# BIH-CEI/napkon-string-matching

Measured on AMD Instinct MI355X. Metric: pair-comparisons/sec (whole node), N x M all-pairs, higher is better.
Workload: dtype u64; 1 GPU; C3: 200000x200000 strings/GPU (len U[16,64], 37 symbols), fuzzy_match RAW, threshold 0.8; score_func=fuzzy_match, mode=RAW, hits_per_rank=2000, hits_all_ranks=2000, exact_prune=True, hit_ordering=second stream, overlapped with the next step's grid kernel (two hit buffers)

## Files before the change

### include/nsm_hip.h

```cpp
#ifndef NSM_HIP_H
#define NSM_HIP_H

#include <stdint.h>

#ifdef __cplusplus
extern "C" {
#endif

#define NSM_ABI_VERSION 5

#define NSM_E_BADARG 10001
#define NSM_E_UNSUPPORTED 10002

#define NSM_LEVELS_ID_LIMIT (1 << 26)

typedef struct nsm_hit {
  double score;
  int32_t i;
  int32_t j;
} nsm_hit;

typedef struct nsm_set_table {
  const int32_t* ids;
  const int32_t* cnt;
  const uint64_t* sig;
  const uint64_t* sig2;
  const int32_t* orig;
  const int32_t* size_start;
  const int32_t* nlev;
  const uint8_t* plen;
  const uint64_t* cat;
  const uint32_t* filt;
  const int32_t* seg;
  const int32_t* seg_start;
  int32_t n;
  int32_t width;
  int32_t max_levels;
  int32_t vocab;
  const uint64_t* post;
  const int32_t* post_start;
  uint64_t post_sq[5];
  int32_t post_row_bits;
  int32_t post_format;
} nsm_set_table;

typedef struct nsm_str_table {
  const uint8_t* codes;
  const int32_t* len;
  const int32_t* orig;
  const int32_t* len_start;
  const uint8_t* hist;
  int32_t n;
  int32_t stride;
  int32_t alphabet;
  const uint8_t* hist16;
} nsm_str_table;

typedef struct nsm_level_items {
  const int32_t* first;
  const int32_t* nlev;
  const int32_t* orig;
  const uint64_t* cat;
  const int32_t* seg;
  const int32_t* seg_start;
  int32_t n;
} nsm_level_items;

#define NSM_CAT_NONE 0
#define NSM_CAT_INTERSECT 1
#define NSM_CAT_INTERSECT_OR_BOTH_EMPTY 2

#define NSM_FLAG_PRUNE 1u
#define NSM_FLAG_INDEX 4u
#define NSM_FLAG_NO_INDEX 8u
#define NSM_FLAG_TILE_INDEX 64u
#define NSM_FLAG_PARK 16u
#define NSM_FLAG_SPLIT 128u
#define NSM_FLAG_TILE 256u
#define NSM_FLAG_PROBE 512u
#define NSM_FLAG_ONE_STAGE 1024u
#define NSM_FLAG_PACK 2048u
#define NSM_FLAG_NO_PACK 4096u
#define NSM_FLAG_WAVE_WIDE 2u

int nsm_abi_version(void);
const char* nsm_last_error(void);

int nsm_jaccard_raw_grid(const nsm_set_table* left, const nsm_set_table* right, double threshold,
                         uint32_t flags, nsm_hit* hits , uint64_t capacity,
                         unsigned long long* hit_count , void* stream);

int nsm_indel_raw_top_k(const nsm_str_table* left, const nsm_str_table* right, double threshold, int32_t k,
                        uint32_t flags, nsm_hit* out ,
                        unsigned long long* out_count , uint64_t* stats ,
                        void* stream);
int nsm_jaccard_raw_top_k(const nsm_set_table* left, const nsm_set_table* right, double threshold, int32_t k,
                          uint32_t flags, nsm_hit* out, unsigned long long* out_count, uint64_t* stats, void* stream);

int nsm_indel_raw_top_k_grouped(const nsm_str_table* left, const nsm_str_table* right,
                                const int32_t* right_group ,
                                double threshold, int32_t k, uint32_t flags,
                                nsm_hit* out , unsigned long long* out_count ,
                                uint64_t* stats , void* stream);
int nsm_jaccard_raw_top_k_grouped(const nsm_set_table* left, const nsm_set_table* right, const int32_t* right_group,
                                  double threshold, int32_t k, uint32_t flags,
                                  nsm_hit* out, unsigned long long* out_count, uint64_t* stats, void* stream);

int nsm_jaccard_levels_grid(const nsm_set_table* left, const nsm_set_table* right, double threshold,
                            int32_t category_mode, uint32_t flags, nsm_hit* hits, uint64_t capacity,
                            unsigned long long* hit_count, void* stream);

int nsm_indel_raw_grid(const nsm_str_table* left, const nsm_str_table* right, double threshold,
                       uint32_t flags, nsm_hit* hits, uint64_t capacity,
                       unsigned long long* hit_count, void* stream);

uint64_t nsm_indel_levels_workspace_bytes(const nsm_level_items* left, const nsm_str_table* left_strings,
                                          const nsm_level_items* right, const nsm_str_table* right_strings,
                                          double threshold, uint32_t flags, double expected_survivors);
int nsm_indel_levels_grid(const nsm_level_items* left, const nsm_str_table* left_strings,
                          const nsm_level_items* right, const nsm_str_table* right_strings,
                          double threshold, int32_t category_mode, uint32_t flags, nsm_hit* hits,
                          uint64_t capacity, unsigned long long* hit_count, void* workspace,
                          uint64_t workspace_bytes, double expected_survivors, void* stream);

int nsm_indel_levels_top_k(const nsm_level_items* left, const nsm_str_table* left_strings,
                           const nsm_level_items* right, const nsm_str_table* right_strings,
                           double threshold, int32_t k, int32_t category_mode, uint32_t flags,
                           const int32_t* banned_start , const int32_t* banned_j ,
                           nsm_hit* out , unsigned long long* out_count ,
                           uint64_t* stats , void* stream);
int nsm_jaccard_levels_top_k(const nsm_set_table* left, const nsm_set_table* right,
                             double threshold, int32_t k, int32_t category_mode, uint32_t flags,
                             const int32_t* banned_start, const int32_t* banned_j,
                             nsm_hit* out, unsigned long long* out_count, uint64_t* stats, void* stream);

int nsm_indel_raw_profile(const nsm_str_table* left, const nsm_str_table* right, const double* thresholds ,
                          int32_t n_thresholds, uint32_t flags, uint64_t* pairs ,
                          double* left_best ,
                          double* right_best , uint64_t* stats ,
                          void* stream);
int nsm_jaccard_raw_profile(const nsm_set_table* left, const nsm_set_table* right, const double* thresholds,
                            int32_t n_thresholds, uint32_t flags, uint64_t* pairs, double* left_best, double* right_best,
                            uint64_t* stats, void* stream);
int nsm_indel_levels_profile(const nsm_level_items* left, const nsm_str_table* left_strings,
                             const nsm_level_items* right, const nsm_str_table* right_strings,
                             const double* thresholds, int32_t n_thresholds, int32_t category_mode, uint32_t flags,
                             const int32_t* banned_start, const int32_t* banned_j, uint64_t* pairs, double* left_best,
                             double* right_best, uint64_t* stats, void* stream);
int nsm_jaccard_levels_profile(const nsm_set_table* left, const nsm_set_table* right, const double* thresholds,
                               int32_t n_thresholds, int32_t category_mode, uint32_t flags, const int32_t* banned_start,
                               const int32_t* banned_j, uint64_t* pairs, double* left_best, double* right_best,
                               uint64_t* stats, void* stream);

int nsm_indel_raw_floor_grid(const nsm_str_table* left, const nsm_str_table* right, double threshold,
                             const double* left_floor , const double* right_floor ,
                             uint32_t flags, nsm_hit* hits, uint64_t capacity,
                             unsigned long long* hit_count , uint64_t* stats ,
                             void* stream);
int nsm_jaccard_raw_floor_grid(const nsm_set_table* left, const nsm_set_table* right, double threshold,
                               const double* left_floor, const double* right_floor, uint32_t flags, nsm_hit* hits,
                               uint64_t capacity, unsigned long long* hit_count, uint64_t* stats, void* stream);
int nsm_indel_levels_floor_grid(const nsm_level_items* left, const nsm_str_table* left_strings,
                                const nsm_level_items* right, const nsm_str_table* right_strings, double threshold,
                                const double* left_floor, const double* right_floor, int32_t category_mode, uint32_t flags,
                                const int32_t* banned_start, const int32_t* banned_j, nsm_hit* hits, uint64_t capacity,
                                unsigned long long* hit_count, uint64_t* stats, void* stream);
int nsm_jaccard_levels_floor_grid(const nsm_set_table* left, const nsm_set_table* right, double threshold,
                                  const double* left_floor, const double* right_floor, int32_t category_mode, uint32_t flags,
                                  const int32_t* banned_start, const int32_t* banned_j, nsm_hit* hits, uint64_t capacity,
                                  unsigned long long* hit_count, uint64_t* stats, void* stream);

int nsm_indel_raw_pairs(const nsm_str_table* left, const nsm_str_table* right,
                        const int32_t* left_row , int32_t left_ids, const int32_t* right_row ,
                        int32_t right_ids, nsm_hit* pairs , uint64_t n_pairs, void* stream);
int nsm_jaccard_raw_pairs(const nsm_set_table* left, const nsm_set_table* right, const int32_t* left_row, int32_t left_ids,
                          const int32_t* right_row, int32_t right_ids, nsm_hit* pairs, uint64_t n_pairs, void* stream);
int nsm_indel_levels_pairs(const nsm_level_items* left, const nsm_str_table* left_strings,
                           const nsm_level_items* right, const nsm_str_table* right_strings,
                           const int32_t* left_row, int32_t left_ids, const int32_t* right_row, int32_t right_ids,
                           nsm_hit* pairs, uint64_t n_pairs, void* stream);
int nsm_jaccard_levels_pairs(const nsm_set_table* left, const nsm_set_table* right, const int32_t* left_row,
                             int32_t left_ids, const int32_t* right_row, int32_t right_ids, nsm_hit* pairs, uint64_t n_pairs,
                             void* stream);

int nsm_release(void* stream);
int nsm_release_all(void);

#define NSM_BUILD_PARTITION 1u
#define NSM_BUILD_VALIDATE 2u
#define NSM_BUILD_SORT 4u

int nsm_build_set_table(const int32_t* ids_in, int32_t n, int32_t width_in, int32_t side, const int32_t* nlev_in,
                        const uint8_t* plen_in, const uint64_t* cat_in, const int32_t* orig_in, int32_t category_mode,
                        uint32_t flags, nsm_set_table* out, void* stream);

int nsm_build_str_table(const uint8_t* codes_in, const int32_t* len_in, const int32_t* orig_in, int32_t n, uint32_t flags,
                        nsm_str_table* out, void* stream);

int nsm_build_level_items(const int32_t* first_in, const int32_t* nlev_in, const uint64_t* cat_in, const int32_t* orig_in,
                          int32_t n, int32_t category_mode, uint32_t flags, nsm_level_items* out, void* stream);

typedef struct nsm_any_strings {
  const uint16_t* codes;
  const int64_t* offset;
  int32_t n_rows;
  int32_t alphabet;
  int32_t max_len;
} nsm_any_strings;

typedef struct nsm_any_items {
  const int32_t* first;
  const int32_t* nlev;
  const int32_t* orig;
  const uint64_t* cat;
  int32_t n;
} nsm_any_items;

typedef struct nsm_any_sets {
  const int32_t* ids;
  const uint8_t* lv;
  const int64_t* offset;
  const int32_t* nlev;
  const int32_t* plen;
  const int32_t* orig;
  const uint64_t* cat;
  int32_t n;
  int32_t max_levels;
  int32_t max_ids;
  const int32_t* first;
} nsm_any_sets;

#define NSM_FLAG_RAW_SCORE 32u

int nsm_indel_any_grid(const nsm_any_items* left, const nsm_any_strings* left_strings, const nsm_any_items* right,
                       const nsm_any_strings* right_strings, double threshold, int32_t category_mode, uint32_t flags,
                       nsm_hit* hits, uint64_t capacity, unsigned long long* hit_count, void* stream);
int nsm_jaccard_any_grid(const nsm_any_sets* left, const nsm_any_sets* right, double threshold, int32_t category_mode,
                         uint32_t flags, nsm_hit* hits, uint64_t capacity, unsigned long long* hit_count, void* stream);

int nsm_sort_hits(nsm_hit* hits, nsm_hit* scratch, uint64_t capacity, const unsigned long long* hit_count,
                  uint64_t n_hint, uint32_t id_limit, void* stream);

#ifdef __cplusplus
}
#endif
#endif
```

### napkon-string-matching_amd/csrc/indel_raw.hip

```cpp
#include "nsm_common.hpp"
#include "indel_score.hpp"

#include <map>
#include <mutex>
#include <utility>

namespace nsm {

struct IndelRawParams {
  int32_t n_left;
  int32_t n_right;
  int32_t rows_per_chunk;
  int32_t pm_stride;
  int32_t zero_need;
  unsigned long long cap;
  uint8_t lcsmin[132];
};

static double indel_score_host(int la, int lb, int lcs) {
  if (la == 0 || lb == 0) return 0.0;
  const volatile double maximum = static_cast<double>(la + lb);
  const volatile double dist = static_cast<double>(la + lb - 2 * lcs);
  const volatile double q = dist / maximum;
  const volatile double norm_sim = 1.0 - q;
  const volatile double pct = norm_sim * 100.0;
  return pct / 100.0;
}

template <typename T>
__device__ __forceinline__ T lds_load(uint32_t addr) {
  return *reinterpret_cast<const __attribute__((address_space(3))) T*>(addr);
}

__device__ __forceinline__ unsigned long long add64(unsigned long long a, unsigned long long b) {
  unsigned long long d;
  asm("v_lshl_add_u64 %0, %1, 0, %2" : "=v"(d) : "v"(a), "v"(b));
  return d;
}

__device__ __forceinline__ void raw_build_masks(unsigned long long* pm, int pm_stride, const uint8_t* __restrict__ lcodes, int i,
                                                int la, bool wide, int lane) {
  for (int c = lane; c < pm_stride; c += kWave) pm[c] = 0ull;
  __builtin_amdgcn_fence(__ATOMIC_RELEASE, "wavefront");
  __builtin_amdgcn_wave_barrier();
  if (lane < la) {
    const unsigned c = lcodes[static_cast<size_t>(i) * 64 + lane];
    atomicOr(&pm[c], wide ? (1ull << lane) : ((1ull << lane) | (1ull << (32 + lane))));
  }
  __builtin_amdgcn_fence(__ATOMIC_ACQ_REL, "wavefront");
  __builtin_amdgcn_wave_barrier();
}

#ifndef NSM_LCS_STOP_EVERY
#define NSM_LCS_STOP_EVERY 1
#endif
__device__ __forceinline__ int raw_lcs_units(uint32_t lcode, int la, uint32_t rcode, int lb, int need, int lane) {
  const bool swap = la < lb;
  const int lp = swap ? lb : la, lt = swap ? la : lb;
  const uint32_t pat = lane < lp ? (swap ? rcode : lcode) : 0x100u;
  const uint32_t text = lane < lt ? (swap ? lcode : rcode) : 0x200u;
  const int lim = lt - need + 64;
  unsigned long long v = ~0ull;
  if (lt > 0) {
#pragma unroll
    for (int w = 0; w < 16; ++w) {
#pragma unroll
      for (int b = 0; b < 4; ++b) {
        const uint32_t c = static_cast<uint32_t>(__builtin_amdgcn_readlane(static_cast<int>(text), 4 * w + b));
        const unsigned long long m = __ballot(pat == c);
        const unsigned long long u = v & m;
        v = (v + u) | (v & ~m);
      }
      if (4 * (w + 1) >= lt) break;
      if (NSM_LCS_STOP_EVERY > 0 && (w + 1) % (NSM_LCS_STOP_EVERY > 0 ? NSM_LCS_STOP_EVERY : 1) == 0 && __popcll(v) + 4 * (w + 1) > lim)
        break;
    }
  }
  return __popcll(~v);
}

__device__ __forceinline__ int raw_lcs_pair(const uint8_t* __restrict__ lcodes, int row, int la, const uint8_t* __restrict__ rcodes,
                                            int j, int lb, int need, int lane) {
  return raw_lcs_units(lcodes[static_cast<size_t>(row) * 64 + lane], la, rcodes[static_cast<size_t>(j) * 64 + lane], lb, need, lane);
}

#ifndef NSM_C3_OCC
#define NSM_C3_OCC
#endif
#ifndef NSM_C3_TILES
#define NSM_C3_TILES 2
#endif
template <bool PRUNE>
constexpr int c3_tiles() { return PRUNE ? NSM_C3_TILES : 1; }

template <bool PRUNE>
__global__ __launch_bounds__(kBlock) NSM_C3_OCC void indel_raw_kernel(
    const uint8_t* __restrict__ lcodes, const int32_t* __restrict__ llen, const int32_t* __restrict__ lstart,
    const int32_t* __restrict__ lorig, const uint32_t* __restrict__ lhist, const uint8_t* __restrict__ rcodes,
    const int32_t* __restrict__ rlen, const int32_t* __restrict__ rorig, const uint32_t* __restrict__ rhist,
    nsm_hit* __restrict__ hits, unsigned long long* __restrict__ count, const IndelRawParams p) {
  constexpr int T = c3_tiles<PRUNE>();
  extern __shared__ __attribute__((aligned(16))) unsigned long long s_mem[];
  uint8_t* s_lcsmin = reinterpret_cast<uint8_t*>(s_mem + kWavesPerBlock * p.pm_stride);
  for (int t = threadIdx.x; t < 132; t += kBlock) s_lcsmin[t] = p.lcsmin[t];
  __syncthreads();

  const int lane = threadIdx.x & (kWave - 1);
  const int wave = threadIdx.x >> 6;
  const int tile0 = (blockIdx.x * kWavesPerBlock + wave) * T;
  if (tile0 * kWave >= p.n_right) return;
  bool valid[T];
  int jc[T], lbj[T];
#pragma unroll
  for (int t = 0; t < T; ++t) {
    const int j = (tile0 + t) * kWave + lane;
    valid[t] = j < p.n_right;
    jc[t] = valid[t] ? j : p.n_right - 1;
    lbj[t] = valid[t] ? rlen[jc[t]] : 0;
  }

  unsigned long long* pm = s_mem + wave * p.pm_stride;
  const uint32_t pm_base = static_cast<uint32_t>(wave * p.pm_stride * 8);

  uint32_t taddr[PRUNE ? 1 : 32];
  auto build_taddr = [&](bool narrow) {
    if constexpr (!PRUNE) {
      const uint4* tp = reinterpret_cast<const uint4*>(rcodes + static_cast<size_t>(jc[0]) * 64);
      const uint32_t hsel = narrow ? 4u : 0u;
#pragma unroll
      for (int q = 0; q < 4; ++q) {
        const uint4 v = tp[q];
        const uint32_t w[4] = {v.x, v.y, v.z, v.w};
#pragma unroll
        for (int e = 0; e < 4; ++e) {
          const uint32_t c0 = w[e] & 0xffu, c1 = (w[e] >> 8) & 0xffu, c2 = (w[e] >> 16) & 0xffu, c3 = w[e] >> 24;
          const uint32_t a0 = pm_base + 8 * c0 + (((c0 >> 4) & 1u) ? hsel : 0u), a1 = pm_base + 8 * c1 + (((c1 >> 4) & 1u) ? hsel : 0u);
          const uint32_t a2 = pm_base + 8 * c2 + (((c2 >> 4) & 1u) ? hsel : 0u), a3 = pm_base + 8 * c3 + (((c3 >> 4) & 1u) ? hsel : 0u);
          taddr[8 * q + 2 * e + 0] = a0 | (a1 << 16);
          taddr[8 * q + 2 * e + 1] = a2 | (a3 << 16);
        }
      }
    }
  };
  int taddr_narrow = -1;
  const int npairs = (wave_first(lbj[0]) + 1) >> 1;
  uint32_t hr[T][8];
  if (PRUNE) {
#pragma unroll
    for (int t = 0; t < T; ++t) {
      const uint4* hp = reinterpret_cast<const uint4*>(rhist + static_cast<size_t>(jc[t]) * 8);
      const uint4 h0 = hp[0], h1 = hp[1];
      hr[t][0] = h0.x; hr[t][1] = h0.y; hr[t][2] = h0.z; hr[t][3] = h0.w;
      hr[t][4] = h1.x; hr[t][5] = h1.y; hr[t][6] = h1.z; hr[t][7] = h1.w;
    }
  }
  uint32_t lowmask = 0xffffu;
  asm volatile("" : "+v"(lowmask));

  const int i0 = blockIdx.y * p.rows_per_chunk;
  const int i1 = min(p.n_left, i0 + p.rows_per_chunk);

  auto build_masks = [&](int i, int la, bool wide) { raw_build_masks(pm, p.pm_stride, lcodes, i, la, wide, lane); };

  auto lcs_row = [&](int i, int la, bool wide) -> int {
    if (taddr_narrow != static_cast<int>(!wide)) {
      build_taddr(!wide);
      taddr_narrow = static_cast<int>(!wide);
    }
    build_masks(i, la, wide);
    const int nchars = 2 * npairs;
    if (!wide) {
      uint32_t v = ~0u;
#pragma unroll
      for (int g = 0; g < 8; ++g) {
        if (g * 8 < nchars) {
          uint32_t m[8];
#pragma unroll
          for (int q = 0; q < 4; ++q) {
            m[2 * q] = lds_load<uint32_t>(taddr[(4 * g + q) % (PRUNE ? 1 : 32)] & lowmask);
            m[2 * q + 1] = lds_load<uint32_t>(taddr[(4 * g + q) % (PRUNE ? 1 : 32)] >> 16);
          }
#pragma unroll
          for (int q = 0; q < 8; ++q) v = lcs_step32(v, m[q]);
        }
      }
      return 32 - __popc(v);
    }
    unsigned long long v = ~0ull;
#pragma unroll
    for (int g = 0; g < 8; ++g) {
      if (g * 8 < nchars) {
        unsigned long long m[8];
#pragma unroll
        for (int q = 0; q < 4; ++q) {
          m[2 * q] = lds_load<unsigned long long>(taddr[(4 * g + q) % (PRUNE ? 1 : 32)] & lowmask);
          m[2 * q + 1] = lds_load<unsigned long long>(taddr[(4 * g + q) % (PRUNE ? 1 : 32)] >> 16);
        }
#pragma unroll
        for (int q = 0; q < 8; ++q) v = lcs_step64(v, m[q]);
      }
    }
    return 64 - __popcll(v);
  };

  const int c_first = 64 - llen[i0];
  const int c_last = 64 - llen[i1 - 1];
  for (int c = c_first; c <= c_last; ++c) {
    const int a = max(i0, lstart[c]);
    const int b = min(i1, lstart[c + 1]);
    if (a >= b) continue;
    const int la = 64 - c;
    int need[T];
#pragma unroll
    for (int t = 0; t < T; ++t) {
      if (la == 0 || lbj[t] == 0) need[t] = p.zero_need;
      else need[t] = s_lcsmin[la + lbj[t]];
      if (!valid[t]) need[t] = kNever;
    }
    const bool wide = la > 32;
    if constexpr (PRUNE) {
      bool fits[T], some = false;
#pragma unroll
      for (int t = 0; t < T; ++t) {
        fits[t] = min(la, lbj[t]) >= need[t];
        some = some || fits[t];
      }
      if (!__any(some)) continue;
      auto score_row = [&](int i, uint32_t who) {
#pragma unroll
        for (int t = 0; t < T; ++t) {
          for (unsigned long long todo = __ballot((who >> t) & 1u); todo; todo &= todo - 1ull) {
            const int leader = __builtin_ctzll(todo);
            const int j_s = __builtin_amdgcn_readlane(jc[t], leader);
            const int lb_s = __builtin_amdgcn_readlane(lbj[t], leader);
            const int need_s = __builtin_amdgcn_readlane(need[t], leader);
            const int lcs = raw_lcs_pair(lcodes, i, la, rcodes, j_s, lb_s, need_s, lane);
            if (lcs >= need_s && lane == 0) emit_hit(hits, p.cap, count, indel_score(la, lb_s, lcs), lorig[i], rorig[j_s]);
          }
        }
      };
      int limit[T];
      uint32_t seed[T];
#pragma unroll
      for (int t = 0; t < T; ++t) {
        limit[t] = fits[t] ? la + lbj[t] - 2 * need[t] : -1;
        seed[t] = static_cast<uint32_t>(-(limit[t] + 1));
      }
      const uint32_t* __restrict__ hp = lhist + static_cast<size_t>(a) * 8;
      int i = a;
#ifndef NSM_C3_BATCH
#define NSM_C3_BATCH 4
#endif
      constexpr int BATCH = NSM_C3_BATCH;
      for (; i + BATCH <= b; i += BATCH, hp += 8 * BATCH) {
        uint32_t h[8 * BATCH];
#pragma unroll
        for (int q = 0; q < 8 * BATCH; ++q) h[q] = hp[q];
        int margin[T][BATCH];
        int any_pass = 0;
#pragma unroll
        for (int r = 0; r < BATCH; ++r) {
#pragma unroll
          for (int t = 0; t < T; ++t) {
            uint32_t l1 = seed[t];
#pragma unroll
            for (int q = 0; q < 8; ++q) l1 = __builtin_amdgcn_sad_u8(h[8 * r + q], hr[t][q], l1);
            margin[t][r] = static_cast<int>(l1);
            any_pass |= margin[t][r];
          }
        }
        if (__any(any_pass < 0)) {
          uint32_t cand[T];
#pragma unroll
          for (int t = 0; t < T; ++t) {
            cand[t] = 0;
#pragma unroll
            for (int r = 0; r < BATCH; ++r) cand[t] |= margin[t][r] < 0 ? (1u << r) : 0u;
          }
          for (int r = 0; r < BATCH; ++r) {
            uint32_t who = 0;
#pragma unroll
            for (int t = 0; t < T; ++t) who |= ((cand[t] >> r) & 1u) << t;
            if (__any(who != 0u)) score_row(i + r, who);
          }
        }
      }
      for (; i < b; ++i, hp += 8) {
        uint32_t who = 0;
#pragma unroll
        for (int t = 0; t < T; ++t) {
          uint32_t l1 = 0;
#pragma unroll
          for (int q = 0; q < 8; ++q) l1 = __builtin_amdgcn_sad_u8(hp[q], hr[t][q], l1);
          who |= (static_cast<int>(l1) <= limit[t] ? 1u : 0u) << t;
        }
        if (__any(who != 0u)) score_row(i, who);
      }
    } else {
      for (int i = a; i < b; ++i) {
        const int lcs = lcs_row(i, la, wide);
        const bool hit = lcs >= need[0];
        if (__any(hit)) {
          if (hit) emit_hit(hits, p.cap, count, indel_score(la, lbj[0], lcs), lorig[i], rorig[jc[0]]);
        }
      }
    }
  }
}

}
#include "indel_raw_coarse.hpp"
namespace nsm {

static int pick_rows_per_chunk(int n_left, int n_tiles) {
#ifndef NSM_C3_WANT_WAVES
#define NSM_C3_WANT_WAVES (16ll * 256 * 32)
#endif
  const long long want_waves = NSM_C3_WANT_WAVES;
  long long chunks = (want_waves + n_tiles - 1) / (n_tiles > 0 ? n_tiles : 1);
  if (chunks < 1) chunks = 1;
  long long rows = (n_left + chunks - 1) / chunks;
  if (rows < 64) rows = 64;
#ifndef NSM_C3_CHUNK_MAX
#define NSM_C3_CHUNK_MAX 4096
#endif
  if (rows > NSM_C3_CHUNK_MAX) rows = NSM_C3_CHUNK_MAX;
  return static_cast<int>(rows);
}

struct PackScratch {
  void* rows = nullptr;
  size_t bytes = 0;
};
static std::mutex g_pack_mu;
static std::map<std::pair<int, void*>, PackScratch> g_pack;

static void* pack_scratch(hipStream_t stream, size_t bytes) {
  int dev = 0;
  if (hipGetDevice(&dev) != hipSuccess) return nullptr;
  std::lock_guard<std::mutex> lock(g_pack_mu);
  PackScratch& w = g_pack[std::make_pair(dev, static_cast<void*>(stream))];
  if (w.bytes >= bytes && w.rows) return w.rows;
  if (w.rows) (void)hipFree(w.rows);
  w.rows = nullptr;
  w.bytes = 0;
  if (hipMalloc(&w.rows, bytes) != hipSuccess) {
    (void)hipGetLastError();
    w.rows = nullptr;
    return nullptr;
  }
  w.bytes = bytes;
  return w.rows;
}

void release_pack_scratch(int dev, void* stream, bool all) {
  std::lock_guard<std::mutex> lock(g_pack_mu);
  for (auto it = g_pack.begin(); it != g_pack.end();) {
    if (all || it->first == std::make_pair(dev, stream)) {
      if (it->second.rows) (void)hipFree(it->second.rows);
      it = g_pack.erase(it);
    } else {
      ++it;
    }
  }
}

int indel_raw_wide(const nsm_str_table* left, const nsm_str_table* right, double threshold, uint32_t flags,
                   nsm_hit* hits, uint64_t capacity, unsigned long long* hit_count, hipStream_t stream);

}

extern "C" int nsm_indel_raw_grid(const nsm_str_table* left, const nsm_str_table* right,
                                  double threshold, uint32_t flags, nsm_hit* hits, uint64_t capacity,
                                  unsigned long long* hit_count, void* stream) {
  using namespace nsm;
  if (!left || !right || !hit_count || (!hits && capacity)) {
    set_error("nsm_indel_raw_grid: null argument");
    return NSM_E_BADARG;
  }
  if (left->stride != right->stride || (left->stride != 64 && left->stride != 128 && left->stride != 256 && left->stride != 512)) {
    set_error("nsm_indel_raw_grid: stride %d/%d unsupported (both sides 64, 128, 256 or 512 code units)",
              left->stride, right->stride);
    return NSM_E_UNSUPPORTED;
  }
  if (left->alphabet != right->alphabet || left->alphabet < 1 || left->alphabet > 255) {
    set_error("nsm_indel_raw_grid: alphabets differ or exceed 255 (%d, %d)", left->alphabet,
              right->alphabet);
    return NSM_E_BADARG;
  }
  if (left->n < 0 || right->n < 0) {
    set_error("nsm_indel_raw_grid: negative row count");
    return NSM_E_BADARG;
  }
  if (left->n == 0 || right->n == 0) return 0;
  if (!left->codes || !left->len || !left->orig || !left->len_start || !right->codes || !right->len ||
      !right->orig) {
    set_error("nsm_indel_raw_grid: table has a null column");
    return NSM_E_BADARG;
  }

  if (left->stride != 64)
    return indel_raw_wide(left, right, threshold, flags, hits, capacity, hit_count, static_cast<hipStream_t>(stream));

  IndelRawParams p;
  p.n_left = left->n; p.n_right = right->n;
  p.cap = capacity;
  p.pm_stride = ((left->alphabet + 1) + 63) / 64 * 64;
  p.zero_need = (0.0 >= threshold) ? 0 : kNever;
  for (int s = 0; s < 132; ++s) {
    p.lcsmin[s] = kNever;
    if (s < 2 || s > 128) continue;
    for (int lcs = 0; 2 * lcs <= s; ++lcs) {
      if (indel_score_host(1, s - 1, lcs) >= threshold) {
        p.lcsmin[s] = static_cast<uint8_t>(lcs);
        break;
      }
    }
  }
  const bool prune = (flags & NSM_FLAG_PRUNE) && left->hist && right->hist;
  if (prune && left->hist16 && right->hist16 && !(flags & NSM_FLAG_ONE_STAGE)) {
    if ((reinterpret_cast<uintptr_t>(left->hist16) | reinterpret_cast<uintptr_t>(right->hist16)) & 15u) {
      set_error("nsm_indel_raw_grid: hist16 must be 16-byte aligned (rows are read as one 128-bit word)");
      return NSM_E_BADARG;
    }
    if ((reinterpret_cast<uintptr_t>(left->hist) | reinterpret_cast<uintptr_t>(right->hist)) & 15u) {
      set_error("nsm_indel_raw_grid: hist must be 16-byte aligned (rows are read as 128-bit words)");
      return NSM_E_BADARG;
    }
    const int n_tiles = (right->n + kC3cRights - 1) / kC3cRights;
    p.rows_per_chunk = (pick_rows_per_chunk(left->n, n_tiles) + kC3cBlock - 1) / kC3cBlock * kC3cBlock;
    dim3 grid((n_tiles + kWavesPerBlock - 1) / kWavesPerBlock, (left->n + p.rows_per_chunk - 1) / p.rows_per_chunk);
    if (grid.y > 65535) {
      p.rows_per_chunk = ((left->n + 65534) / 65535 + kC3cBlock - 1) / kC3cBlock * kC3cBlock;
      grid.y = (left->n + p.rows_per_chunk - 1) / p.rows_per_chunk;
    }
    if (p.rows_per_chunk > (1 << 15)) {
      set_error("nsm_indel_raw_grid: %d left rows per chunk", p.rows_per_chunk);
      return NSM_E_UNSUPPORTED;
    }
    hipStream_t hs = static_cast<hipStream_t>(stream);
    const uint32_t* lh32 = reinterpret_cast<const uint32_t*>(left->hist);
    const uint32_t* rh32 = reinterpret_cast<const uint32_t*>(right->hist);
#if NSM_C3C_FP4
    bool pack = !(flags & NSM_FLAG_NO_PACK) &&
                ((flags & NSM_FLAG_PACK) || c3c_pack_pays(static_cast<long long>(left->n) * static_cast<long long>(right->n)));
    if (pack) {
      hipStreamCaptureStatus capture = hipStreamCaptureStatusNone;
      if (hipStreamIsCapturing(hs, &capture) != hipSuccess) capture = hipStreamCaptureStatusNone;
      pack = capture == hipStreamCaptureStatusNone;
    }
    void* packed = pack ? pack_scratch(hs, static_cast<size_t>(left->n) * kC3cPackedRow) : nullptr;
    if (packed) {
      const long long units = 2ll * left->n;
      hipLaunchKernelGGL(c3c_pack_left_kernel, dim3(static_cast<unsigned>((units + kBlock - 1) / kBlock)), dim3(kBlock), 0, hs,
                         lh32, static_cast<c3c_v4i*>(packed), left->n);
      hipLaunchKernelGGL((indel_raw_coarse_kernel<NSM_C3C_NT, NSM_C3C_CAP, true>), grid, dim3(kBlock), c3c_lds_bytes(), hs,
                         left->codes, left->len, left->len_start, left->orig, lh32, right->codes, right->len, right->orig,
                         rh32, hits, hit_count, p, static_cast<const char*>(packed));
      return hip_status(hipGetLastError(), "indel_raw_coarse_kernel launch (packed)");
    }
#endif
    hipLaunchKernelGGL((indel_raw_coarse_kernel<NSM_C3C_NT, NSM_C3C_CAP, false>), grid, dim3(kBlock), c3c_lds_bytes(), hs,
                       left->codes, left->len, left->len_start, left->orig, lh32, right->codes, right->len, right->orig,
                       rh32, hits, hit_count, p, static_cast<const char*>(nullptr));
    return hip_status(hipGetLastError(), "indel_raw_coarse_kernel launch");
  }
  const int tiles_per_wave = prune ? c3_tiles<true>() : 1;
  const int n_tiles = ((right->n + kWave - 1) / kWave + tiles_per_wave - 1) / tiles_per_wave;
  p.rows_per_chunk = pick_rows_per_chunk(left->n, n_tiles);
  dim3 grid((n_tiles + kWavesPerBlock - 1) / kWavesPerBlock,
            (left->n + p.rows_per_chunk - 1) / p.rows_per_chunk);
  if (grid.y > 65535) {
    p.rows_per_chunk = (left->n + 65534) / 65535;
    grid.y = (left->n + p.rows_per_chunk - 1) / p.rows_per_chunk;
  }
  const size_t lds = static_cast<size_t>(kWavesPerBlock) * p.pm_stride * 8 + 136;
  hipStream_t s = static_cast<hipStream_t>(stream);
  const uint32_t* lh = reinterpret_cast<const uint32_t*>(left->hist);
  const uint32_t* rh = reinterpret_cast<const uint32_t*>(right->hist);
  if (prune)
    hipLaunchKernelGGL((indel_raw_kernel<true>), grid, dim3(kBlock), lds, s, left->codes, left->len,
                       left->len_start, left->orig, lh, right->codes, right->len, right->orig, rh, hits, hit_count, p);
  else
    hipLaunchKernelGGL((indel_raw_kernel<false>), grid, dim3(kBlock), lds, s, left->codes, left->len,
                       left->len_start, left->orig, lh, right->codes, right->len, right->orig, rh, hits, hit_count, p);
  return hip_status(hipGetLastError(), "indel_raw_kernel launch");
}
```

### napkon-string-matching_amd/csrc/indel_raw_coarse.hpp

```cpp
#pragma once

namespace nsm {

#ifndef NSM_C3C_CAP
#define NSM_C3C_CAP 3
#endif
#ifndef NSM_C3C_FP4
#define NSM_C3C_FP4 1
#endif
#ifndef NSM_C3C_FP4_PERM
#define NSM_C3C_FP4_PERM 1
#endif
#ifndef NSM_C3C_FP4_SPLIT
#define NSM_C3C_FP4_SPLIT 4
#endif
#ifndef NSM_C3C_NT
#define NSM_C3C_NT 4
#endif
#ifndef NSM_C3C_ORFOLD
#define NSM_C3C_ORFOLD (NSM_C3C_FP4 && NSM_C3C_NT % 2 == 0)
#endif
#ifndef NSM_C3C_PIPE
#define NSM_C3C_PIPE (NSM_C3C_NT % (NSM_C3C_ORFOLD ? 4 : 2) == 0)
#endif
#ifndef NSM_C3C_OR_SPLIT
#define NSM_C3C_OR_SPLIT 2
#endif
#ifndef NSM_C3C_LCS_PREFETCH
#define NSM_C3C_LCS_PREFETCH 1
#endif
#ifndef NSM_C3C_EARLY_OUT
#define NSM_C3C_EARLY_OUT 1
#endif
constexpr int kC3cBlock = 32;
constexpr int kC3cRights = NSM_C3C_NT * kC3cBlock;
constexpr int kC3cPipeExtra = NSM_C3C_PIPE ? (NSM_C3C_ORFOLD ? 2 : 1) : 0;
constexpr int kC3cStack = (NSM_C3C_NT + 2 + kC3cPipeExtra) * kWave;
constexpr int kC3cDrainAt = 2 * kWave;
static_assert(NSM_C3C_NT >= 1 && NSM_C3C_NT <= 4, "an entry keeps its tile in 2 bits");
static_assert(NSM_C3C_CAP >= 2 && NSM_C3C_CAP <= 8, "code slots per bucket");

static inline size_t c3c_lds_bytes() {
  return static_cast<size_t>(kWavesPerBlock) * (kC3cStack * 8 + static_cast<size_t>(kC3cRights) * (8 * 4 + 1)) + 136;
}

typedef int c3c_v4i __attribute__((ext_vector_type(4)));
typedef int c3c_v16i __attribute__((ext_vector_type(16)));
typedef int c3c_v8i __attribute__((ext_vector_type(8)));
typedef float c3c_v16f __attribute__((ext_vector_type(16)));

__device__ __forceinline__ uint32_t c3c_ge64(uint32_t w, int k) {
  return (w + static_cast<uint32_t>(0x40 - k) * 0x01010101u) & 0x40404040u;
}


__device__ __forceinline__ int c3c_fp4_scale(const uint4& f0, const uint4& f1) {
  const uint32_t ws[8] = {f0.x, f0.y, f0.z, f0.w, f1.x, f1.y, f1.z, f1.w};
  uint32_t any = 0u;
#pragma unroll
  for (int q = 0; q < 8; ++q) any |= ws[q];
  if ((any & 0xf0f0f0f0u) == 0u) return 0;
  uint32_t top = 0u;
#pragma unroll
  for (int q = 0; q < 8; ++q)
#pragma unroll
    for (int b = 0; b < 4; ++b) top = max(top, (ws[q] >> (8 * b)) & 0xffu);
  return top <= 27u ? 1 : top <= 51u ? 2 : 3;
}
__device__ __forceinline__ void c3c_fp4_right_k0(uint32_t fw, int& m1, int& m2) {
  const uint32_t sel = fw & 0x07070707u;
  const uint32_t big = ((fw >> 3) & 0x01010101u) * 0xffu;
  const uint32_t lo1 = __builtin_amdgcn_perm(0x11111111u, 0x11110100u, sel);
  const uint32_t lo2 = __builtin_amdgcn_perm(0x41312111u, 0x01000000u, sel), hi2 = __builtin_amdgcn_perm(0x71717171u, 0x61615151u, sel);
  m1 = static_cast<int>((big & 0x11111111u) | (~big & lo1));
  m2 = static_cast<int>((big & hi2) | (~big & lo2));
}
__device__ __forceinline__ void c3c_fp4_right_scaled(uint32_t fw, int k, int& m1, int& m2) {
  m1 = static_cast<int>((c3c_ge64(fw, 1) >> 6) | (c3c_ge64(fw, 2) >> 2));
  uint32_t w2 = c3c_ge64(fw, 3) >> 6;
  const uint32_t round_up = (1u << k) - 1u;
#pragma unroll
  for (int b = 0; b < 4; ++b) {
    const uint32_t r = (fw >> (8 * b)) & 0xffu;
    const uint32_t q = (max(r, 3u) - 3u + round_up) >> k;
    w2 |= (static_cast<uint32_t>(0x7777665543210ull >> (4u * q)) & 0xfu) << (8 * b + 4);
  }
  m2 = static_cast<int>(w2);
}
__device__ __forceinline__ void c3c_fp4_left(uint32_t w, int& m1, int& m2) {
#if NSM_C3C_FP4_PERM
  const uint32_t sel = (w + 0x3c3c3c3cu) & 0x43434343u;
  m1 = static_cast<int>(__builtin_amdgcn_perm(0u, 0x44440400u, sel) & 0x44444444u);
  m2 = static_cast<int>(__builtin_amdgcn_perm(0u, 0x04000000u, sel) & 0x44444444u);
#else
  m1 = static_cast<int>(((c3c_ge64(w, 1) >> 4)) | c3c_ge64(w, 2));
  m2 = static_cast<int>(((c3c_ge64(w, 3) >> 4)) | c3c_ge64(w, 4));
#endif
}
__device__ __forceinline__ c3c_v16f c3c_fp4_mfma1(const c3c_v4i& a, const c3c_v4i& b) {
  const c3c_v8i a8 = {a.x, a.y, a.z, a.w, 0, 0, 0, 0}, b8 = {b.x, b.y, b.z, b.w, 0, 0, 0, 0};
  const c3c_v16f zero = {0, 0, 0, 0, 0, 0, 0, 0, 0, 0, 0, 0, 0, 0, 0, 0};
  return __builtin_amdgcn_mfma_scale_f32_32x32x64_f8f6f4(a8, b8, zero, 4, 4, 0, 0, 0, 0);
}
__device__ __forceinline__ c3c_v16f c3c_fp4_mfma2(const c3c_v4i& a, const c3c_v4i& b, const c3c_v16f& acc, int scales, int t) {
  const c3c_v8i a8 = {a.x, a.y, a.z, a.w, 0, 0, 0, 0}, b8 = {b.x, b.y, b.z, b.w, 0, 0, 0, 0};
  switch (t) {
    case 0: return __builtin_amdgcn_mfma_scale_f32_32x32x64_f8f6f4(a8, b8, acc, 4, 4, 0, 0x7f7f7f7f, 0, scales);
    case 1: return __builtin_amdgcn_mfma_scale_f32_32x32x64_f8f6f4(a8, b8, acc, 4, 4, 0, 0x7f7f7f7f, 1, scales);
    case 2: return __builtin_amdgcn_mfma_scale_f32_32x32x64_f8f6f4(a8, b8, acc, 4, 4, 0, 0x7f7f7f7f, 2, scales);
    default: return __builtin_amdgcn_mfma_scale_f32_32x32x64_f8f6f4(a8, b8, acc, 4, 4, 0, 0x7f7f7f7f, 3, scales);
  }
}

constexpr int kC3cPackedRow = 64;
#ifndef NSM_C3C_PACK_MIN_PAIRS
#define NSM_C3C_PACK_MIN_PAIRS 10000000000ll
#endif
static inline bool c3c_pack_pays(long long pairs) { return pairs >= static_cast<long long>(NSM_C3C_PACK_MIN_PAIRS); }
struct c3c_packed_rows {
  c3c_v4i m1, m2;
};
template <bool PACKED>
struct c3c_rows {
  typedef uint4 type;
};
template <>
struct c3c_rows<true> {
  typedef c3c_packed_rows type;
};

__global__ __launch_bounds__(kBlock) void c3c_pack_left_kernel(const uint32_t* __restrict__ lhist, c3c_v4i* __restrict__ packed,
                                                               int n_left) {
  const int u = blockIdx.x * kBlock + threadIdx.x;
  if (u >= 2 * n_left) return;
  const uint4 w = reinterpret_cast<const uint4*>(lhist)[u];
  const uint32_t ws[4] = {w.x, w.y, w.z, w.w};
  c3c_v4i m1, m2;
#pragma unroll
  for (int q = 0; q < 4; ++q) {
    int a1, a2;
    c3c_fp4_left(ws[q], a1, a2);
    m1[q] = a1;
    m2[q] = a2;
  }
  packed[2 * static_cast<size_t>(u)] = m1;
  packed[2 * static_cast<size_t>(u) + 1] = m2;
}

#ifndef NSM_C3C_OCC
#define NSM_C3C_OCC __attribute__((amdgpu_waves_per_eu((NSM_C3C_ORFOLD && PACKED) ? 4 : 2)))
#endif
template <int NT, int CAP, bool PACKED>
__global__ __launch_bounds__(kBlock) NSM_C3C_OCC void indel_raw_coarse_kernel(
    const uint8_t* __restrict__ lcodes, const int32_t* __restrict__ llen, const int32_t* __restrict__ lstart,
    const int32_t* __restrict__ lorig, const uint32_t* __restrict__ lhist, const uint8_t* __restrict__ rcodes,
    const int32_t* __restrict__ rlen, const int32_t* __restrict__ rorig, const uint32_t* __restrict__ rhist,
    nsm_hit* __restrict__ hits, unsigned long long* __restrict__ count, const IndelRawParams p,
    const char* __restrict__ lpacked) {
  static_assert(!PACKED || NSM_C3C_FP4, "only the FP4 scan has packed left rows");
  constexpr int kRights = NT * kC3cBlock;
  static_assert(kC3cDrainAt >= kWave && kC3cDrainAt + (NT + kC3cPipeExtra) * kWave <= kC3cStack,
                "the drain is triggered above kC3cDrainAt entries and runs full passes");
  constexpr bool kOrFold = NSM_C3C_ORFOLD && PACKED;
  constexpr int kFlagHi = 1 << 17, kFlagLo = 1 << 8;
  static_assert(!kOrFold || (NSM_C3C_FP4 && NT % 2 == 0), "the OR fold puts tiles 2 p and 2 p + 1 of the FP4 scan on one accumulator");
  extern __shared__ __attribute__((aligned(16))) unsigned long long s_mem[];
  unsigned long long* s_stack = s_mem;
  uint32_t* s_rh = reinterpret_cast<uint32_t*>(s_stack + kWavesPerBlock * kC3cStack);
  uint8_t* s_rl = reinterpret_cast<uint8_t*>(s_rh + kWavesPerBlock * 8 * kRights);
  uint8_t* s_lcsmin = s_rl + kWavesPerBlock * kRights;
  for (int t = threadIdx.x; t < 132; t += kBlock) s_lcsmin[t] = p.lcsmin[t];
  __syncthreads();

  const int lane = threadIdx.x & (kWave - 1);
  const int wave = threadIdx.x >> 6;
  const int col = lane & (kC3cBlock - 1);
  const int half = lane >> 5;
  const int j0 = (blockIdx.x * kWavesPerBlock + wave) * kRights;
  if (j0 >= p.n_right) return;
  auto lane_again = [&]() -> int {
    int l = lane;
    asm volatile("" : "+v"(l));
    return l;
  };
#if NSM_C3C_EARLY_OUT
  if (p.zero_need != 0) {
    const int ie = blockIdx.y * p.rows_per_chunk;
    const int la_hi = llen[ie], la_lo = llen[min(p.n_left, ie + p.rows_per_chunk) - 1];
    bool fits = false;
#pragma unroll
    for (int k = 0; k < (kRights + kWave - 1) / kWave; ++k) {
      const int j = j0 + k * kWave + lane;
      if (k * kWave + lane < kRights && j < p.n_right) {
        const int lb = rlen[j];
        const int la = min(max(lb, la_lo), la_hi);
        const int nd = (la == 0 || lb == 0) ? p.zero_need : static_cast<int>(s_lcsmin[la + lb]);
        fits = fits || min(la, lb) >= nd;
      }
    }
    if (!__any(fits)) return;
  }
#endif
  unsigned long long* stack = s_stack + wave * kC3cStack;
  uint32_t* rh_lds = s_rh + wave * 8 * kRights;
  uint8_t* rl_lds = s_rl + wave * kRights;

#pragma unroll
  for (int k = 0; k < (kRights + kWave - 1) / kWave; ++k) {
    const int rl = k * kWave + lane;
    if (rl < kRights) {
      const int j = j0 + rl;
      const int jcl = j < p.n_right ? j : p.n_right - 1;
      const uint4* fp = reinterpret_cast<const uint4*>(rhist + static_cast<size_t>(jcl) * 8);
      const uint4 f0 = fp[0], f1 = fp[1];
      uint32_t* dst = rh_lds + rl;
      dst[0 * kRights] = f0.x; dst[1 * kRights] = f0.y; dst[2 * kRights] = f0.z; dst[3 * kRights] = f0.w;
      dst[4 * kRights] = f1.x; dst[5 * kRights] = f1.y; dst[6 * kRights] = f1.z; dst[7 * kRights] = f1.w;
      rl_lds[rl] = static_cast<uint8_t>(j < p.n_right ? rlen[jcl] : 0);
    }
  }
  bool valid[NT];
#if NSM_C3C_FP4
  c3c_v4i bfrag[NT][2];
  uint32_t bscales = 0u;
  auto scale_base = [](int t) -> uint32_t { return (kOrFold && t % 2 == 0) ? 0x7fu + 9u : 0x7fu; };
  uint32_t bscales1 = 0u;
  if constexpr (kOrFold) {
#pragma unroll
    for (int t = 0; t < NT; ++t) bscales1 |= scale_base(t) << (8 * t);
    asm volatile("" : "+v"(bscales1));
  }
  auto code_tile = [&](int t, const uint4& f, int k) __attribute__((always_inline)) {
    const uint32_t ws[4] = {f.x, f.y, f.z, f.w};
    if (k == 0) {
#pragma unroll
      for (int q = 0; q < 4; ++q) {
        int m1, m2;
        c3c_fp4_right_k0(ws[q], m1, m2);
        bfrag[t][0][q] = m1;
        bfrag[t][1][q] = m2;
      }
    } else {
#pragma unroll
      for (int q = 0; q < 4; ++q) {
        int m1, m2;
        c3c_fp4_right_scaled(ws[q], k, m1, m2);
        bfrag[t][0][q] = m1;
        bfrag[t][1][q] = m2;
      }
    }
  };
#pragma unroll
  for (int t = 0; t < NT; ++t) {
    const int j = j0 + t * kC3cBlock + col;
    valid[t] = j < p.n_right;
    const int jcl = valid[t] ? j : p.n_right - 1;
    const uint4* fp = reinterpret_cast<const uint4*>(rhist + static_cast<size_t>(jcl) * 8);
    const uint4 f0 = fp[0], f1 = fp[1];
    const int k = c3c_fp4_scale(f0, f1);
    bscales |= (scale_base(t) + static_cast<uint32_t>(k)) << (8 * t);
    uint4 f = half ? f1 : f0;
    if (!valid[t]) f = make_uint4(0u, 0u, 0u, 0u);
    code_tile(t, f, k);
  }
  auto make_bfrag = [&]() __attribute__((always_inline)) {
    const int l = lane_again();
    const uint32_t* rp0 = rh_lds + (4 * (l >> 5)) * kRights + (l & (kC3cBlock - 1));
#pragma unroll
    for (int t = 0; t < NT; ++t) {
      const uint32_t* rp = rp0 + t * kC3cBlock;
      const int k = static_cast<int>(((bscales >> (8 * t)) & 0xffu) - scale_base(t));
      uint4 f = make_uint4(rp[0], rp[kRights], rp[2 * kRights], rp[3 * kRights]);
      if (!valid[t]) f = make_uint4(0u, 0u, 0u, 0u);
      code_tile(t, f, k);
    }
  };
  __builtin_amdgcn_fence(__ATOMIC_ACQ_REL, "wavefront");
  __builtin_amdgcn_wave_barrier();
#else
  c3c_v4i bfrag[NT][CAP];
  auto code_b = [&](int t, int q, uint32_t fw) {
    const uint32_t full = c3c_ge64(fw, CAP);
#pragma unroll
    for (int s = 0; s < CAP - 1; ++s)
      bfrag[t][s][q] = static_cast<int>((c3c_ge64(fw, s + 1) ^ full) >> 6);
    bfrag[t][CAP - 1][q] = static_cast<int>(full);
  };
#pragma unroll
  for (int t = 0; t < NT; ++t) {
    const int j = j0 + t * kC3cBlock + col;
    valid[t] = j < p.n_right;
    const int jcl = valid[t] ? j : p.n_right - 1;
    uint4 f = reinterpret_cast<const uint4*>(rhist + static_cast<size_t>(jcl) * 8)[half];
    if (!valid[t]) f = make_uint4(0u, 0u, 0u, 0u);
    code_b(t, 0, f.x); code_b(t, 1, f.y); code_b(t, 2, f.z); code_b(t, 3, f.w);
  }
  auto make_bfrag = [&]() {
#pragma unroll
    for (int t = 0; t < NT; ++t) {
      const uint32_t* rp = rh_lds + (4 * half) * kRights + t * kC3cBlock + col;
#pragma unroll
      for (int q = 0; q < 4; ++q) code_b(t, q, valid[t] ? rp[q * kRights] : 0u);
    }
  };
  __builtin_amdgcn_fence(__ATOMIC_ACQ_REL, "wavefront");
  __builtin_amdgcn_wave_barrier();
#endif
  const int i0 = blockIdx.y * p.rows_per_chunk;
  const int i1 = min(p.n_left, i0 + p.rows_per_chunk);
  int q_cnt = 0;

  auto need_of = [&](int la, int lb) -> int { return (la == 0 || lb == 0) ? p.zero_need : static_cast<int>(s_lcsmin[la + lb]); };

  const char* chunk = reinterpret_cast<const char*>(lhist + static_cast<size_t>(i0) * 8);
  const char* pchunk = PACKED ? lpacked + static_cast<size_t>(i0) * kC3cPackedRow : nullptr;

  auto drain_pass = [&]() __attribute__((always_inline)) {
    __builtin_amdgcn_fence(__ATOMIC_ACQ_REL, "wavefront");
    __builtin_amdgcn_wave_barrier();
    const int n = min(q_cnt, kWave);
    const int base = q_cnt - n;
    q_cnt = base;
#ifdef NSM_C3C_X_NODRAIN
    return;
#endif
    const int m = lane & 3;
    uint32_t mask = 0;
#pragma nounroll
    for (int s = (n - 1) >> 4; s >= 0; --s) {
      const int e = 16 * s + (lane >> 2);
      const bool active = e < n;
      const unsigned long long ent = stack[base + (active ? e : 0)];
      const int n_rows = active ? static_cast<int>(static_cast<uint32_t>(ent)) : 0;
      const uint32_t ehi = static_cast<uint32_t>(ent >> 32);
      const uint32_t ib_rel = active ? ehi >> 15 : 0u;
      const int r0 = 4 * static_cast<int>((ehi >> 5) & 1u) + m;
      const uint32_t last_r = static_cast<uint32_t>(max(n_rows, 1) - 1);
      uint4 w0[4], w1[4];
#pragma unroll
      for (int g = 0; g < 4; ++g) {
        const uint4* lp = reinterpret_cast<const uint4*>(chunk + (ib_rel + min(static_cast<uint32_t>(r0 + 8 * g), last_r)) * 32u);
        w0[g] = lp[0];
        w1[g] = lp[1];
      }
      const int la = static_cast<int>((ehi >> 8) & 127u);
      const int tl = static_cast<int>((ehi >> 6) & 3u) * kC3cBlock + static_cast<int>(ehi & 31u);
      const int lb = rl_lds[tl];
      uint32_t rq[8];
      {
        const uint32_t* rp = rh_lds + tl;
#pragma unroll
        for (int q = 0; q < 8; ++q) rq[q] = rp[q * kRights];
      }
      const int nd = need_of(la, lb);
      const int budget = (active && min(la, lb) >= nd) ? la + lb - 2 * nd : -1;
      const uint32_t sad0 = ~static_cast<uint32_t>(budget);
#pragma unroll
      for (int g = 3; g >= 0; --g) {
        uint32_t l1 = sad0;
        l1 = __builtin_amdgcn_sad_u8(w0[g].x, rq[0], l1);
        l1 = __builtin_amdgcn_sad_u8(w0[g].y, rq[1], l1);
        l1 = __builtin_amdgcn_sad_u8(w0[g].z, rq[2], l1);
        l1 = __builtin_amdgcn_sad_u8(w0[g].w, rq[3], l1);
        l1 = __builtin_amdgcn_sad_u8(w1[g].x, rq[4], l1);
        l1 = __builtin_amdgcn_sad_u8(w1[g].y, rq[5], l1);
        l1 = __builtin_amdgcn_sad_u8(w1[g].z, rq[6], l1);
        l1 = __builtin_amdgcn_sad_u8(w1[g].w, rq[7], l1);
        if (r0 + 8 * g >= n_rows) l1 = 0u;
        mask = __builtin_amdgcn_alignbit(mask, l1, 31);
      }
    }
#ifdef NSM_C3C_X_NOLCS
    mask = 0u;
#endif
#ifdef NSM_C3C_X_FINEONLY
    mask = p.n_left < 0 ? mask : 0u;
#endif
    unsigned long long todo = __ballot(mask != 0u);
    uint32_t cur = 0u;
    int leader = 0, row_s = 0, j_n = 0, la_n = 0, lb_n = 0;
    auto next_pair = [&]() -> bool {
      if (cur == 0u) {
        if (todo == 0ull) return false;
        leader = __builtin_ctzll(todo);
        todo &= todo - 1ull;
        cur = static_cast<uint32_t>(__builtin_amdgcn_readlane(static_cast<int>(mask), leader));
      }
      const int pos = 31 - __builtin_clz(cur);
      cur &= ~(1u << pos);
      const uint32_t ehi = static_cast<uint32_t>(
          __builtin_amdgcn_readfirstlane(static_cast<int>(stack[base + 16 * (pos >> 2) + (leader >> 2)] >> 32)));
      const int tl = static_cast<int>((ehi >> 6) & 3u) * kC3cBlock + static_cast<int>(ehi & 31u);
      row_s = i0 + static_cast<int>(ehi >> 15) + 8 * (pos & 3) + 4 * static_cast<int>((ehi >> 5) & 1u) + (leader & 3);
      j_n = j0 + tl;
      la_n = static_cast<int>((ehi >> 8) & 127u);
      lb_n = __builtin_amdgcn_readfirstlane(static_cast<int>(rl_lds[tl]));
      return true;
    };
    auto row_units = [&](uint32_t& lc, uint32_t& rc) {
      lc = lcodes[static_cast<size_t>(row_s) * 64 + lane];
      rc = rcodes[static_cast<size_t>(j_n) * 64 + lane];
    };
    uint32_t lc_next = 0, rc_next = 0;
    bool have = next_pair();
    if (NSM_C3C_LCS_PREFETCH && have) row_units(lc_next, rc_next);
    while (have) {
      const int row_c = row_s, j_s = j_n, la_s = la_n, lb_s = lb_n;
      const int need_s = need_of(la_s, lb_s);
      uint32_t lc = lc_next, rc = rc_next;
      if (!NSM_C3C_LCS_PREFETCH) row_units(lc, rc);
      have = next_pair();
      if (NSM_C3C_LCS_PREFETCH && have) row_units(lc_next, rc_next);
      const int lcs = raw_lcs_units(lc, la_s, rc, lb_s, need_s, lane);
#ifdef NSM_C3C_X_COUNTLCS
      if (lane == 0)
#else
      if (lcs >= need_s && lane == 0)
#endif
        emit_hit(hits, p.cap, count, indel_score(la_s, lb_s, lcs), lorig[row_c], rorig[j_s]);
    }
  };
  auto drain_full = [&]() __attribute__((always_inline)) {
    while (q_cnt >= kWave) drain_pass();
    make_bfrag();
  };

  const int c_first = 64 - llen[i0];
  const int c_last = 64 - llen[i1 - 1];
  const uint32_t lane_off = static_cast<uint32_t>(col * 32 + half * 16);
  for (int c = c_first; c <= c_last; ++c) {
    const int a = max(i0, lstart[c]);
    const int b = min(i1, lstart[c + 1]);
    if (a >= b) continue;
    const int la = 64 - c;
    int need2[2] = {static_cast<int>(kNever), static_cast<int>(kNever)};
    int nm1[NT];
    bool some = false;
    const int l_c = lane_again();
#pragma unroll
    for (int t = 0; t < NT; ++t) {
      const int lb = rl_lds[t * kC3cBlock + (l_c & (kC3cBlock - 1))];
      const int nd = valid[t] ? need_of(la, lb) : static_cast<int>(kNever);
      const bool fits = min(la, lb) >= nd;
      some = some || fits;
#if NSM_C3C_FP4
      if constexpr (kOrFold)
        need2[t & 1] = min(need2[t & 1], fits ? nd : static_cast<int>(kNever));
      else
        nm1[t] = __float_as_int(static_cast<float>(fits ? nd : static_cast<int>(kNever)) - 0.5f);
#else
      nm1[t] = 64 * (fits ? nd : static_cast<int>(kNever)) - 1;
#endif
    }
    if (!__any(some)) continue;
    c3c_v16f bias;
    const float bias1 = __int_as_float(0x4b000000 | ((256 - need2[0]) << 9) | (256 - need2[1]));
    auto make_bias = [&]() {
#pragma unroll
      for (int k = 0; k < 16; ++k) {
        float x;
        asm volatile("v_mov_b32 %0, %1" : "=v"(x) : "v"(bias1));
        bias[k] = x;
      }
    };

    typedef typename c3c_rows<PACKED>::type rows_t;
    const uint32_t last_off = static_cast<uint32_t>(b - 1 - i0) * (PACKED ? 64u : 32u) + static_cast<uint32_t>((l_c >> 5) * (PACKED ? 32 : 16));
    auto load_rows = [&](int i) -> rows_t {
      if constexpr (PACKED) {
        const uint32_t off = min(static_cast<uint32_t>(i - i0) * 64u + 2u * lane_off, last_off);
        const c3c_v4i* pp = reinterpret_cast<const c3c_v4i*>(pchunk + off);
        return c3c_packed_rows{pp[0], pp[1]};
      } else {
        const uint32_t off = min(static_cast<uint32_t>(i - i0) * 32u + lane_off, last_off);
        return *reinterpret_cast<const uint4*>(chunk + off);
      }
    };
#if NSM_C3C_FP4
    typedef c3c_v16f acc_t;
    c3c_v4i afrag[2];
    auto make_afrag = [&](const rows_t& w) {
      if constexpr (!PACKED) {
        const uint32_t ws[4] = {w.x, w.y, w.z, w.w};
#pragma unroll
        for (int q = 0; q < 4; ++q) {
          int m1, m2;
          c3c_fp4_left(ws[q], m1, m2);
          afrag[0][q] = m1;
          afrag[1][q] = m2;
        }
      }
    };
    constexpr int NU = kOrFold ? NT / 2 : NT;
    auto chain = [&](int u, const rows_t& w) -> acc_t {
      if constexpr (kOrFold) {
        acc_t acc = c3c_fp4_mfma2(w.m1, bfrag[2 * u][0], bias, static_cast<int>(bscales1), 2 * u);
        acc = c3c_fp4_mfma2(w.m2, bfrag[2 * u][1], acc, static_cast<int>(bscales), 2 * u);
        acc = c3c_fp4_mfma2(w.m1, bfrag[2 * u + 1][0], acc, static_cast<int>(bscales1), 2 * u + 1);
        return c3c_fp4_mfma2(w.m2, bfrag[2 * u + 1][1], acc, static_cast<int>(bscales), 2 * u + 1);
      } else if constexpr (PACKED) {
        return c3c_fp4_mfma2(w.m2, bfrag[u][1], c3c_fp4_mfma1(w.m1, bfrag[u][0]), static_cast<int>(bscales), u);
      } else {
        return c3c_fp4_mfma2(afrag[1], bfrag[u][1], c3c_fp4_mfma1(afrag[0], bfrag[u][0]), static_cast<int>(bscales), u);
      }
    };
    auto fold = [&](const acc_t& acc) -> int {
      const c3c_v16i bits = __builtin_bit_cast(c3c_v16i, acc);
      if constexpr (kOrFold) {
        int top = bits[0] | bits[1] | bits[2];
#pragma unroll
        for (int k = 3; k < 15; k += 2) top = top | bits[k] | bits[k + 1];
        return (top | bits[15]) & (kFlagHi | kFlagLo);
      } else {
        int top = max(max(bits[0], bits[1]), bits[2]);
#pragma unroll
        for (int k = 3; k < 15; k += 2) top = max(max(top, bits[k]), bits[k + 1]);
        return max(top, bits[15]);
      }
    };
#else
    typedef c3c_v16i acc_t;
    constexpr int NU = NT;
    c3c_v4i afrag[CAP - 1];
    auto make_afrag = [&](const uint4& w) {
#pragma unroll
      for (int s = 0; s < CAP - 1; ++s) {
        afrag[s].x = static_cast<int>(c3c_ge64(w.x, s + 1)); afrag[s].y = static_cast<int>(c3c_ge64(w.y, s + 1));
        afrag[s].z = static_cast<int>(c3c_ge64(w.z, s + 1)); afrag[s].w = static_cast<int>(c3c_ge64(w.w, s + 1));
      }
    };
    auto chain = [&](int t, const uint4& w) -> c3c_v16i {
      c3c_v16i acc = {0, 0, 0, 0, 0, 0, 0, 0, 0, 0, 0, 0, 0, 0, 0, 0};
#pragma unroll
      for (int s = 0; s < CAP - 1; ++s) acc = __builtin_amdgcn_mfma_i32_32x32x32_i8(afrag[s], bfrag[t][s], acc, 0, 0, 0);
      const c3c_v4i last = {static_cast<int>(w.x), static_cast<int>(w.y), static_cast<int>(w.z), static_cast<int>(w.w)};
      return __builtin_amdgcn_mfma_i32_32x32x32_i8(last, bfrag[t][CAP - 1], acc, 0, 0, 0);
    };
    auto fold = [&](const c3c_v16i& acc) -> int {
      int top = max(max(acc[0], acc[1]), acc[2]);
#pragma unroll
      for (int k = 3; k < 15; k += 2) top = max(max(top, acc[k]), acc[k + 1]);
      return max(top, acc[15]);
    };
#endif
    auto push = [&](bool ps, unsigned long long m, int t, int i) {
      if (m == 0ull) return;
#ifdef NSM_C3C_X_COUNTPUSH
      if (lane == 0) atomicAdd(count, static_cast<unsigned long long>(__popcll(m)));
#endif
      if (ps) {
        const int slot = __builtin_amdgcn_mbcnt_hi(static_cast<uint32_t>(m >> 32), __builtin_amdgcn_mbcnt_lo(static_cast<uint32_t>(m), static_cast<uint32_t>(q_cnt)));
        const uint32_t hi = (static_cast<uint32_t>(i - i0) << 15) | (static_cast<uint32_t>(la) << 8) | (static_cast<uint32_t>(t) << 6);
        uint32_t el = static_cast<uint32_t>(lane);
        asm volatile("" : "+v"(el));
        const uint32_t n_rows = static_cast<uint32_t>(min(kC3cBlock, b - i));
        stack[slot] = (static_cast<unsigned long long>(hi | el) << 32) | n_rows;
      }
      q_cnt += __popcll(m);
    };
    auto finish = [&](int top, int u, int i) {
      if constexpr (kOrFold) {
        if (__ballot(top != 0) == 0ull) return;
        const bool hi = (top & kFlagHi) != 0 && valid[2 * u], lo = (top & kFlagLo) != 0 && valid[2 * u + 1];
        push(hi, __ballot(hi), 2 * u, i);
        push(lo, __ballot(lo), 2 * u + 1, i);
      } else {
        const bool ps = top > nm1[u];
        push(ps, __ballot(ps), u, i);
      }
    };
#if NSM_C3C_PIPE
    static_assert(NU % 2 == 0, "unit 0 of the next block takes the accumulator of unit NU: NU must be even (or NSM_C3C_PIPE=0)");
    acc_t acc[2];
    auto block = [&](int i, rows_t& wc, rows_t& wn) __attribute__((always_inline)) -> bool {
      const bool more = i + kC3cBlock < b;
      bool flush = false;
#pragma unroll
      for (int t = 0; t < NU; ++t) {
        if (t + 1 < NU) {
          acc[(t + 1) & 1] = chain(t + 1, wc);
        } else {
          flush = q_cnt > kC3cDrainAt;
          if (kOrFold || (more && !flush)) {
            make_afrag(wn);
            if constexpr (PACKED) asm volatile("" : "+v"(wn.m1), "+v"(wn.m2));
            if (i + 2 * kC3cBlock < b) wc = load_rows(i + 2 * kC3cBlock);
            acc[0] = chain(0, wn);
          }
        }
        const int top = fold(acc[t & 1]);
#if NSM_C3C_FP4
        if constexpr (kOrFold) {
          __builtin_amdgcn_sched_group_barrier(0x008, 1, 0);
          __builtin_amdgcn_sched_group_barrier(0x002, NSM_C3C_OR_SPLIT, 0);
          __builtin_amdgcn_sched_group_barrier(0x008, 1, 0);
          __builtin_amdgcn_sched_group_barrier(0x002, NSM_C3C_OR_SPLIT, 0);
          __builtin_amdgcn_sched_group_barrier(0x008, 1, 0);
          __builtin_amdgcn_sched_group_barrier(0x002, NSM_C3C_OR_SPLIT, 0);
          __builtin_amdgcn_sched_group_barrier(0x008, 1, 0);
          __builtin_amdgcn_sched_group_barrier(0x002, 8 - 3 * NSM_C3C_OR_SPLIT, 0);
        } else {
          __builtin_amdgcn_sched_group_barrier(0x008, 1, 0);
          __builtin_amdgcn_sched_group_barrier(0x002, NSM_C3C_FP4_SPLIT, 0);
          __builtin_amdgcn_sched_group_barrier(0x008, 1, 0);
          __builtin_amdgcn_sched_group_barrier(0x002, 8 - NSM_C3C_FP4_SPLIT, 0);
        }
        if (t + 1 < NU || kOrFold || (more && !flush)) asm volatile("" : "+v"(acc[(t + 1) & 1]));
#else
        __builtin_amdgcn_sched_group_barrier(0x008, 1, 0);
        __builtin_amdgcn_sched_group_barrier(0x002, 4, 0);
        __builtin_amdgcn_sched_group_barrier(0x008, 1, 0);
        __builtin_amdgcn_sched_group_barrier(0x002, 4, 0);
        __builtin_amdgcn_sched_group_barrier(0x008, 1, 0);
#endif
        finish(top, t, i);
      }
      return flush;
    };
    for (int i = a; i < b;) {
      if (q_cnt > kC3cDrainAt)
        drain_full();
      if constexpr (kOrFold) make_bias();
      rows_t w0 = load_rows(i);
      make_afrag(w0);
      rows_t w1;
      if constexpr (PACKED) {
        w1 = load_rows(i + kC3cBlock);
      } else {
        w1 = w0;
        if (i + kC3cBlock < b) w1 = load_rows(i + kC3cBlock);
      }
      acc[0] = chain(0, w0);
      for (;;) {
        const bool f0 = block(i, w0, w1);
        if ((i += kC3cBlock) >= b || f0) break;
        const bool f1 = block(i, w1, w0);
        if ((i += kC3cBlock) >= b || f1) break;
      }
    }
#else
    if constexpr (kOrFold) make_bias();
    rows_t w_next = load_rows(a);
    for (int i = a; i < b; i += kC3cBlock) {
      const rows_t w = w_next;
      if (i + kC3cBlock < b) w_next = load_rows(i + kC3cBlock);
      if (q_cnt > kC3cDrainAt)
        drain_full();
      make_afrag(w);
#pragma unroll
      for (int t = 0; t < NU; ++t) {
        const acc_t acc = chain(t, w);
        finish(fold(acc), t, i);
      }
    }
#endif
  }
  while (q_cnt > 0) drain_pass();
}

}
```

### napkon-string-matching_amd/napkon_string_matching_amd/_lib.py

```python
import ctypes
import os
from pathlib import Path

_HERE = Path(__file__).resolve().parent
LIB_PATH = Path(os.environ.get("NSM_HIP_LIBRARY", _HERE.parent / "csrc" / "libnsm_hip.so"))

ABI_VERSION = 5
FLAG_PRUNE = 1
FLAG_WAVE_WIDE = 2
FLAG_INDEX, FLAG_NO_INDEX = 4, 8
FLAG_TILE_INDEX = 64
FLAG_RAW_SCORE = 32
FLAG_ONE_STAGE = 1024
FLAG_PACK, FLAG_NO_PACK = 2048, 4096
FLAG_SPLIT, FLAG_TILE, FLAG_PROBE = 128, 256, 512
FLAG_PARK = 16
BUILD_PARTITION, BUILD_VALIDATE, BUILD_SORT = 1, 2, 4
ASSIGN_ROUNDS_ONLY, ASSIGN_STREAM_ONLY = 1, 2
GROUP_CONTINUE = 1
SPAN_NO_COMPACT = 1
CAT_NONE, CAT_INTERSECT, CAT_INTERSECT_OR_BOTH_EMPTY = 0, 1, 2

c_i32p = ctypes.c_void_p
c_u64 = ctypes.c_uint64


class NsmHit(ctypes.Structure):
    _fields_ = [("score", ctypes.c_double), ("i", ctypes.c_int32), ("j", ctypes.c_int32)]


class NsmHitList(ctypes.Structure):
    _fields_ = [("hits", ctypes.c_void_p), ("n", ctypes.c_uint64), ("left_base", ctypes.c_int32), ("left_ids", ctypes.c_int32),
                ("right_base", ctypes.c_int32), ("right_ids", ctypes.c_int32)]


class NsmSetTable(ctypes.Structure):
    _fields_ = [
        ("ids", ctypes.c_void_p),
        ("cnt", ctypes.c_void_p),
        ("sig", ctypes.c_void_p),
        ("sig2", ctypes.c_void_p),
        ("orig", ctypes.c_void_p),
        ("size_start", ctypes.c_void_p),
        ("nlev", ctypes.c_void_p),
        ("plen", ctypes.c_void_p),
        ("cat", ctypes.c_void_p),
        ("filt", ctypes.c_void_p),
        ("seg", ctypes.c_void_p),
        ("seg_start", ctypes.c_void_p),
        ("n", ctypes.c_int32),
        ("width", ctypes.c_int32),
        ("max_levels", ctypes.c_int32),
        ("vocab", ctypes.c_int32),
        ("post", ctypes.c_void_p),
        ("post_start", ctypes.c_void_p),
        ("post_sq", ctypes.c_uint64 * 5),
        ("post_row_bits", ctypes.c_int32),
        ("post_format", ctypes.c_int32),
    ]


class NsmStrTable(ctypes.Structure):
    _fields_ = [
        ("codes", ctypes.c_void_p),
        ("len", ctypes.c_void_p),
        ("orig", ctypes.c_void_p),
        ("len_start", ctypes.c_void_p),
        ("hist", ctypes.c_void_p),
        ("n", ctypes.c_int32),
        ("stride", ctypes.c_int32),
        ("alphabet", ctypes.c_int32),
        ("hist16", ctypes.c_void_p),
    ]


class NsmAnyStrings(ctypes.Structure):
    _fields_ = [("codes", ctypes.c_void_p), ("offset", ctypes.c_void_p), ("n_rows", ctypes.c_int32),
                ("alphabet", ctypes.c_int32), ("max_len", ctypes.c_int32)]


class NsmAnyItems(ctypes.Structure):
    _fields_ = [("first", ctypes.c_void_p), ("nlev", ctypes.c_void_p), ("orig", ctypes.c_void_p), ("cat", ctypes.c_void_p),
                ("n", ctypes.c_int32)]


class NsmAnySets(ctypes.Structure):
    _fields_ = [("ids", ctypes.c_void_p), ("lv", ctypes.c_void_p), ("offset", ctypes.c_void_p), ("nlev", ctypes.c_void_p),
                ("plen", ctypes.c_void_p), ("orig", ctypes.c_void_p), ("cat", ctypes.c_void_p), ("n", ctypes.c_int32),
                ("max_levels", ctypes.c_int32), ("max_ids", ctypes.c_int32), ("first", ctypes.c_void_p)]


class NsmLevelItems(ctypes.Structure):
    _fields_ = [
        ("first", ctypes.c_void_p),
        ("nlev", ctypes.c_void_p),
        ("orig", ctypes.c_void_p),
        ("cat", ctypes.c_void_p),
        ("seg", ctypes.c_void_p),
        ("seg_start", ctypes.c_void_p),
        ("n", ctypes.c_int32),
    ]


EXPORTS = (
    "nsm_abi_version",
    "nsm_last_error",
    "nsm_jaccard_raw_grid",
    "nsm_jaccard_levels_grid",
    "nsm_indel_raw_grid",
    "nsm_indel_levels_grid",
    "nsm_indel_levels_workspace_bytes",
    "nsm_release",
    "nsm_release_all",
    "nsm_sort_hits",
    "nsm_build_set_table",
    "nsm_build_str_table",
    "nsm_build_level_items",
    "nsm_indel_any_grid",
    "nsm_jaccard_any_grid",
    "nsm_indel_raw_top_k",
    "nsm_jaccard_raw_top_k",
    "nsm_indel_levels_top_k",
    "nsm_jaccard_levels_top_k",
    "nsm_indel_raw_top_k_grouped",
    "nsm_jaccard_raw_top_k_grouped",
    "nsm_indel_raw_profile",
    "nsm_jaccard_raw_profile",
    "nsm_indel_levels_profile",
    "nsm_jaccard_levels_profile",
    "nsm_indel_raw_pairs",
    "nsm_jaccard_raw_pairs",
    "nsm_indel_levels_pairs",
    "nsm_jaccard_levels_pairs",
    "nsm_indel_raw_floor_grid",
    "nsm_jaccard_raw_floor_grid",
    "nsm_indel_levels_floor_grid",
    "nsm_jaccard_levels_floor_grid",
)

ASSIGN_EXPORTS = ("nsm_assign_hits",)
GROUP_EXPORTS = ("nsm_group_hits",)

SPAN_EXPORTS = ("nsm_span_hits",)

_lib = None


class NsmLibraryError(RuntimeError):
    pass


def load() -> ctypes.CDLL:
    global _lib
    if _lib is not None:
        return _lib
    if not LIB_PATH.exists():
        raise NsmLibraryError(
            f"{LIB_PATH} is missing: build it with `python -c 'import __graft_entry__ as g; g.build()'` "
            "(hipcc --offload-arch=gfx950).  There is no CPU fallback for the match loop."
        )
    lib = ctypes.CDLL(str(LIB_PATH))
    lib.nsm_abi_version.restype = ctypes.c_int
    lib.nsm_last_error.restype = ctypes.c_char_p
    if lib.nsm_abi_version() != ABI_VERSION:
        raise NsmLibraryError(f"{LIB_PATH}: ABI {lib.nsm_abi_version()} != expected {ABI_VERSION}")
    P = ctypes.POINTER
    grid_tail = [ctypes.c_void_p, c_u64, ctypes.c_void_p, ctypes.c_void_p]
    lib.nsm_jaccard_raw_grid.argtypes = [P(NsmSetTable), P(NsmSetTable), ctypes.c_double, ctypes.c_uint32] + grid_tail
    lib.nsm_jaccard_levels_grid.argtypes = [
        P(NsmSetTable), P(NsmSetTable), ctypes.c_double, ctypes.c_int32, ctypes.c_uint32] + grid_tail
    lib.nsm_indel_raw_grid.argtypes = [P(NsmStrTable), P(NsmStrTable), ctypes.c_double, ctypes.c_uint32] + grid_tail
    lib.nsm_indel_levels_grid.argtypes = [
        P(NsmLevelItems), P(NsmStrTable), P(NsmLevelItems), P(NsmStrTable),
        ctypes.c_double, ctypes.c_int32, ctypes.c_uint32, ctypes.c_void_p, c_u64, ctypes.c_void_p, ctypes.c_void_p, c_u64,
        ctypes.c_double, ctypes.c_void_p]
    lib.nsm_indel_levels_workspace_bytes.argtypes = [
        P(NsmLevelItems), P(NsmStrTable), P(NsmLevelItems), P(NsmStrTable), ctypes.c_double, ctypes.c_uint32, ctypes.c_double]
    lib.nsm_release.argtypes = [ctypes.c_void_p]
    lib.nsm_release_all.argtypes = []
    lib.nsm_indel_any_grid.argtypes = [
        P(NsmAnyItems), P(NsmAnyStrings), P(NsmAnyItems), P(NsmAnyStrings), ctypes.c_double, ctypes.c_int32,
        ctypes.c_uint32] + grid_tail
    lib.nsm_jaccard_any_grid.argtypes = [P(NsmAnySets), P(NsmAnySets), ctypes.c_double, ctypes.c_int32, ctypes.c_uint32] + grid_tail
    top_k_tail = [ctypes.c_double, ctypes.c_int32, ctypes.c_uint32, ctypes.c_void_p, ctypes.c_void_p, ctypes.c_void_p,
                  ctypes.c_void_p]
    lib.nsm_indel_raw_top_k.argtypes = [P(NsmStrTable), P(NsmStrTable)] + top_k_tail
    lib.nsm_jaccard_raw_top_k.argtypes = [P(NsmSetTable), P(NsmSetTable)] + top_k_tail
    lib.nsm_indel_raw_top_k_grouped.argtypes = [P(NsmStrTable), P(NsmStrTable), ctypes.c_void_p] + top_k_tail
    lib.nsm_jaccard_raw_top_k_grouped.argtypes = [P(NsmSetTable), P(NsmSetTable), ctypes.c_void_p] + top_k_tail
    levels_top_k_tail = [ctypes.c_double, ctypes.c_int32, ctypes.c_int32, ctypes.c_uint32, ctypes.c_void_p, ctypes.c_void_p,
                         ctypes.c_void_p, ctypes.c_void_p, ctypes.c_void_p, ctypes.c_void_p]
    lib.nsm_indel_levels_top_k.argtypes = [P(NsmLevelItems), P(NsmStrTable), P(NsmLevelItems), P(NsmStrTable)] + levels_top_k_tail
    lib.nsm_jaccard_levels_top_k.argtypes = [P(NsmSetTable), P(NsmSetTable)] + levels_top_k_tail
    profile_tail = [ctypes.c_void_p, ctypes.c_int32, ctypes.c_uint32, ctypes.c_void_p, ctypes.c_void_p, ctypes.c_void_p,
                    ctypes.c_void_p, ctypes.c_void_p]
    lib.nsm_indel_raw_profile.argtypes = [P(NsmStrTable), P(NsmStrTable)] + profile_tail
    lib.nsm_jaccard_raw_profile.argtypes = [P(NsmSetTable), P(NsmSetTable)] + profile_tail
    levels_profile_tail = [ctypes.c_void_p, ctypes.c_int32, ctypes.c_int32, ctypes.c_uint32, ctypes.c_void_p, ctypes.c_void_p,
                           ctypes.c_void_p, ctypes.c_void_p, ctypes.c_void_p, ctypes.c_void_p, ctypes.c_void_p]
    lib.nsm_indel_levels_profile.argtypes = [P(NsmLevelItems), P(NsmStrTable), P(NsmLevelItems), P(NsmStrTable)] + levels_profile_tail
    lib.nsm_jaccard_levels_profile.argtypes = [P(NsmSetTable), P(NsmSetTable)] + levels_profile_tail
    pairs_tail = [ctypes.c_void_p, ctypes.c_int32, ctypes.c_void_p, ctypes.c_int32, ctypes.c_void_p, c_u64, ctypes.c_void_p]
    lib.nsm_indel_raw_pairs.argtypes = [P(NsmStrTable), P(NsmStrTable)] + pairs_tail
    lib.nsm_jaccard_raw_pairs.argtypes = [P(NsmSetTable), P(NsmSetTable)] + pairs_tail
    lib.nsm_indel_levels_pairs.argtypes = [P(NsmLevelItems), P(NsmStrTable), P(NsmLevelItems), P(NsmStrTable)] + pairs_tail
    lib.nsm_jaccard_levels_pairs.argtypes = [P(NsmSetTable), P(NsmSetTable)] + pairs_tail
    floor_tail = [ctypes.c_double, ctypes.c_void_p, ctypes.c_void_p, ctypes.c_uint32, ctypes.c_void_p, c_u64, ctypes.c_void_p,
                  ctypes.c_void_p, ctypes.c_void_p]
    lib.nsm_indel_raw_floor_grid.argtypes = [P(NsmStrTable), P(NsmStrTable)] + floor_tail
    lib.nsm_jaccard_raw_floor_grid.argtypes = [P(NsmSetTable), P(NsmSetTable)] + floor_tail
    levels_floor_tail = [ctypes.c_double, ctypes.c_void_p, ctypes.c_void_p, ctypes.c_int32, ctypes.c_uint32, ctypes.c_void_p,
                         ctypes.c_void_p, ctypes.c_void_p, c_u64, ctypes.c_void_p, ctypes.c_void_p, ctypes.c_void_p]
    lib.nsm_indel_levels_floor_grid.argtypes = [P(NsmLevelItems), P(NsmStrTable), P(NsmLevelItems), P(NsmStrTable)] + levels_floor_tail
    lib.nsm_jaccard_levels_floor_grid.argtypes = [P(NsmSetTable), P(NsmSetTable)] + levels_floor_tail
    lib.nsm_sort_hits.argtypes = [ctypes.c_void_p, ctypes.c_void_p, c_u64, ctypes.c_void_p, c_u64, ctypes.c_uint32,
                                  ctypes.c_void_p]
    vp, i32, u32 = ctypes.c_void_p, ctypes.c_int32, ctypes.c_uint32
    lib.nsm_build_set_table.argtypes = [vp, i32, i32, i32, vp, vp, vp, vp, i32, u32, P(NsmSetTable), vp]
    lib.nsm_build_str_table.argtypes = [vp, vp, vp, i32, u32, P(NsmStrTable), vp]
    lib.nsm_build_level_items.argtypes = [vp, vp, vp, vp, i32, i32, u32, P(NsmLevelItems), vp]
    for name in EXPORTS:
        fn = getattr(lib, name)
        if name not in ("nsm_last_error", "nsm_indel_levels_workspace_bytes"):
            fn.restype = ctypes.c_int
    lib.nsm_indel_levels_workspace_bytes.restype = c_u64
    lib.nsm_last_error.restype = ctypes.c_char_p
    assign_args = {"nsm_assign_hits": [vp, c_u64, i32, i32, u32, vp, vp, vp, vp]}
    group_args = {"nsm_group_hits": [P(NsmHitList), i32, i32, ctypes.c_double, u32, vp, vp, vp]}
    span_args = {"nsm_span_hits": [P(NsmHitList), i32, i32, ctypes.c_double, u32, vp, vp, vp, vp, vp]}
    for names, args in ((ASSIGN_EXPORTS, assign_args), (GROUP_EXPORTS, group_args), (SPAN_EXPORTS, span_args)):
        for name in names:
            try:
                fn = getattr(lib, name)
            except AttributeError:
                continue
            fn.argtypes, fn.restype = args[name], ctypes.c_int
    _lib = lib
    return lib


def entry(name: str):
    try:
        return getattr(load(), name)
    except AttributeError:
        raise NsmLibraryError(f"{LIB_PATH} has no {name}: rebuild it (python -c 'import __graft_entry__ as g; g.build()')") from None


def check(status: int, what: str) -> None:
    if status != 0:
        msg = load().nsm_last_error().decode("utf-8", "replace")
        if status == 10002:
            raise NotImplementedError(f"{what}: {msg}")
        raise NsmLibraryError(f"{what} failed with status {status}: {msg}")
```

### napkon-string-matching_amd/napkon_string_matching_amd/grid.py

```python
from __future__ import annotations

from dataclasses import dataclass
from typing import Callable, Optional

import numpy as np
import torch

from . import _lib
from .tables import LevelItems, SetTable, StrTable

HIT_BYTES = 16
DEFAULT_CAPACITY = 1 << 20


@dataclass
class Hits:

    score: np.ndarray
    i: np.ndarray
    j: np.ndarray

    def __len__(self) -> int:
        return int(self.score.shape[0])

    def as_tuples(self):
        return list(zip(self.score.tolist(), self.i.tolist(), self.j.tolist()))


def _require_gpu(device) -> torch.device:
    dev = torch.device(device)
    if dev.type != "cuda" or not torch.cuda.is_available():
        raise _lib.NsmLibraryError(
            "the match loop only runs on an MI355X (HIP device); there is no CPU fallback"
        )
    return dev


class HitBuffer:

    def __init__(self, capacity: int, device) -> None:
        self.capacity = int(capacity)
        rows = max(1, self.capacity)
        self.storage = torch.zeros((rows + 1, 2), dtype=torch.float64, device=device)
        self.records = self.storage[:rows]
        self.count = self.storage[rows:].view(torch.int64).view(-1)[:1]
        self.scratch: Optional[torch.Tensor] = None

    def reset(self) -> None:
        self.count.zero_()

    def views(self, n: int):
        score = self.records[:n, 0]
        ij = self.records.view(torch.int32).view(-1, 4)[:n, 2:4]
        return score, ij[:, 0], ij[:, 1]


SMALL_SORT_MAX = 8192


def sort_hits_device(buf: HitBuffer, n: int, id_limit: int = 0) -> Hits:
    if n == 0:
        return Hits(np.zeros(0, np.float64), np.zeros(0, np.int32), np.zeros(0, np.int32))
    lib = _lib.load()
    scratch_ptr = 0
    if n > SMALL_SORT_MAX:
        if buf.scratch is None or buf.scratch.shape[0] < n:
            buf.scratch = torch.empty((n, 2), dtype=torch.float64, device=buf.records.device)
        scratch_ptr = buf.scratch.data_ptr()
    stream = torch.cuda.current_stream(buf.records.device).cuda_stream
    _lib.check(
        lib.nsm_sort_hits(buf.records.data_ptr(), scratch_ptr, buf.capacity, buf.count.data_ptr(), n,
                          max(0, min(int(id_limit), 0x7FFFFFFF)), stream),
        "nsm_sort_hits",
    )
    host = buf.records[:n].cpu().numpy()
    ij = host.view(np.int32).reshape(n, 4)
    return Hits(host[:, 0].copy(), ij[:, 2].copy(), ij[:, 3].copy())


class PendingHits:

    def __init__(self, buf: HitBuffer, n: int, id_limit: int) -> None:
        self.buf, self.n, self.id_limit = buf, int(n), int(id_limit)

    def finish(self) -> Hits:
        return sort_hits_device(self.buf, self.n, self.id_limit)

    def storage(self, capacity: int) -> torch.Tensor:
        out = torch.zeros((int(capacity) + 1, 2), dtype=torch.float64, device=self.buf.records.device)
        out[: self.n] = self.buf.records[: self.n]
        out[int(capacity):].view(torch.int64).view(-1)[0] = self.n
        return out


def run_grid(launch: Callable[[HitBuffer, int], int], device, capacity: Optional[int], what: str,
             id_limit: int = 0, defer: bool = False):
    dev = _require_gpu(device)
    buf = HitBuffer(capacity or DEFAULT_CAPACITY, dev)
    stream = torch.cuda.current_stream(dev).cuda_stream
    for _attempt in range(2):
        buf.reset()
        _lib.check(launch(buf, stream), what)
        n = int(buf.count.item())
        if n <= buf.capacity:
            return PendingHits(buf, n, id_limit) if defer else sort_hits_device(buf, n, id_limit)
        buf = HitBuffer(n, dev)
    raise _lib.NsmLibraryError(f"{what}: hit count changed between two identical launches")


def jaccard_raw_grid(
    left: SetTable, right: SetTable, threshold: float, prune: bool = True, capacity: Optional[int] = None,
    index: Optional[bool] = None, defer: bool = False,
) -> Hits:
    if left.side != "left" or right.side != "right":
        raise ValueError("tables must be encoded with side='left' and side='right' (distinct padding)")
    if left.has_empty and right.has_empty:
        raise ZeroDivisionError("division by zero")
    lib = _lib.load()
    ls, rs = left.struct(), right.struct()
    flags = (_lib.FLAG_PRUNE if prune else 0) | (0 if index is None else (_lib.FLAG_INDEX if index else _lib.FLAG_NO_INDEX))
    if index == "tile":
        flags |= _lib.FLAG_TILE_INDEX

    def launch(buf: HitBuffer, stream: int) -> int:
        return lib.nsm_jaccard_raw_grid(
            ls, rs, float(threshold), flags, buf.records.data_ptr(), buf.capacity, buf.count.data_ptr(), stream
        )

    id_limit = max(left.id_limit, right.id_limit) if left.id_limit and right.id_limit else 0
    return run_grid(launch, left.ids.device, capacity, "nsm_jaccard_raw_grid", id_limit=id_limit, defer=defer)


def indel_raw_grid(
    left: StrTable, right: StrTable, threshold: float, prune: bool = True, capacity: Optional[int] = None,
    two_stage: bool = True, pack: Optional[bool] = None, defer: bool = False,
) -> Hits:
    lib = _lib.load()
    ls, rs = left.struct(), right.struct()
    flags = ((_lib.FLAG_PRUNE if prune else 0) | (0 if two_stage else _lib.FLAG_ONE_STAGE)
             | (0 if pack is None else (_lib.FLAG_PACK if pack else _lib.FLAG_NO_PACK)))

    def launch(buf: HitBuffer, stream: int) -> int:
        return lib.nsm_indel_raw_grid(
            ls, rs, float(threshold), flags, buf.records.data_ptr(), buf.capacity, buf.count.data_ptr(), stream
        )

    return run_grid(launch, left.codes.device, capacity, "nsm_indel_raw_grid", defer=defer)


TOP_K_MAX = 4096


def check_k(k) -> int:
    if isinstance(k, bool) or not isinstance(k, (int, np.integer)) or int(k) < 1:
        raise ValueError(f"k must be an int >= 1, got {k!r}")
    return int(k)


def select_top_k(hits: Hits, k: int, groups=None) -> Hits:
    if len(hits) == 0:
        return hits
    by_row = np.lexsort((hits.j, -hits.score, hits.i))
    if groups is not None:
        g = np.asarray(groups)[hits.j]
        by_group = np.lexsort((hits.j, -hits.score, g, hits.i))
        gi, gg = hits.i[by_group], g[by_group]
        reps = by_group[np.r_[True, (gi[1:] != gi[:-1]) | (gg[1:] != gg[:-1])]]
        by_row = reps[np.lexsort((hits.j[reps], -hits.score[reps], hits.i[reps]))]
    i_sorted = hits.i[by_row]
    start = np.r_[0, np.flatnonzero(i_sorted[1:] != i_sorted[:-1]) + 1]
    rank = np.arange(len(by_row)) - np.repeat(start, np.diff(np.r_[start, len(by_row)]))
    keep = by_row[rank < k]
    order = keep[np.lexsort((hits.j[keep], hits.i[keep], -hits.score[keep]))]
    return Hits(hits.score[order], hits.i[order], hits.j[order])


def _device_groups(groups, n_right: int, orig: torch.Tensor, device, what: str) -> torch.Tensor:
    if isinstance(groups, torch.Tensor):
        if groups.dim() != 1 or groups.dtype != torch.int32:
            raise ValueError(f"{what}: groups must be a one-dimensional int32 tensor")
        n = int(groups.shape[0])
    else:
        groups = np.ascontiguousarray(groups)
        if groups.ndim != 1 or not np.issubdtype(groups.dtype, np.integer):
            raise ValueError(f"{what}: groups must be a one-dimensional integer array")
        n = int(groups.shape[0])
    if n != n_right:
        raise ValueError(f"{what}: {n} group ids for {n_right} right items")
    dev = _require_gpu(device)
    if not isinstance(groups, torch.Tensor):
        if groups.size and (groups.min() < -(1 << 31) or groups.max() >= (1 << 31)):
            raise ValueError(f"{what}: group ids must fit int32")
        groups = torch.from_numpy(groups.astype(np.int32))
    groups = groups.to(dev).contiguous()
    if n_right and int(orig.max().item()) >= n:
        raise ValueError(f"{what}: the right table reports ids up to {int(orig.max().item())}, beyond the {n} group ids")
    return groups


def _top_k(launch: Callable, n_left: int, n_right: int, k: int, device, what: str, stats: Optional[list] = None,
           id_limit: int = 0) -> Hits:
    dev = _require_gpu(device)
    k_eff = min(k, max(n_right, 1))
    if k_eff > TOP_K_MAX:
        raise NotImplementedError(f"{what}: k = {k_eff} (after clamping to the right side's {n_right} rows) exceeds the "
                                  f"supported {TOP_K_MAX}")
    buf = HitBuffer(max(1, n_left * k_eff), dev)
    st = torch.zeros(4, dtype=torch.int64, device=dev)
    buf.reset()
    if n_left and n_right:
        _lib.check(launch(buf.records, buf.count, st, k_eff, torch.cuda.current_stream(dev).cuda_stream), what)
    n = int(buf.count.item())
    if stats is not None:
        stats[:] = [int(v) for v in st.tolist()]
    return sort_hits_device(buf, n, id_limit)


def _raw_top_k(entry: str, left, right, device, k: int, threshold: float, prune: bool, stats: Optional[list], groups,
               id_limit: int = 0) -> Hits:
    what = entry if groups is None else entry + "_grouped"
    gcol = None if groups is None else _device_groups(groups, right.n, right.orig, device, what)
    fn = getattr(_lib.load(), what)
    ls, rs = left.struct(), right.struct()
    flags = _lib.FLAG_PRUNE if prune else 0
    group_arg = () if gcol is None else (gcol.data_ptr(),)
    return _top_k(lambda out, cnt, st, kk, stream: fn(
        ls, rs, *group_arg, float(threshold), kk, flags, out.data_ptr(), cnt.data_ptr(), st.data_ptr(), stream),
        left.n, right.n, k, device, what, stats, id_limit)


def indel_raw_top_k(left: StrTable, right: StrTable, k: int, threshold: float, prune: bool = True,
                    stats: Optional[list] = None, groups=None) -> Hits:
    k = check_k(k)
    return _raw_top_k("nsm_indel_raw_top_k", left, right, left.codes.device, k, threshold, prune, stats, groups)


def jaccard_raw_top_k(left: SetTable, right: SetTable, k: int, threshold: float, prune: bool = True,
                      stats: Optional[list] = None, groups=None) -> Hits:
    k = check_k(k)
    if left.side != "left" or right.side != "right":
        raise ValueError("tables must be encoded with side='left' and side='right' (distinct padding)")
    if groups is not None and len(groups) != right.n:
        raise ValueError(f"nsm_jaccard_raw_top_k_grouped: {len(groups)} group ids for {right.n} right items")
    if left.has_empty and right.has_empty:
        raise ZeroDivisionError("division by zero")
    id_limit = max(left.id_limit, right.id_limit) if left.id_limit and right.id_limit else 0
    return _raw_top_k("nsm_jaccard_raw_top_k", left, right, left.ids.device, k, threshold, prune, stats, groups, id_limit)


def banned_csr(banned, n_ids: int, device):
    if banned is None:
        return None, None
    bi = np.asarray(banned[0], dtype=np.int64).reshape(-1)
    bj = np.asarray(banned[1], dtype=np.int64).reshape(-1)
    if bi.shape != bj.shape:
        raise ValueError("banned: the left and right id arrays differ in length")
    if len(bi) == 0:
        return None, None
    if int(bi.min()) < 0 or int(bj.min()) < 0:
        raise ValueError("banned: caller ids must be >= 0")
    n = max(int(n_ids), int(bi.max()) + 1)
    order = np.lexsort((bj, bi))
    start = np.zeros(n + 1, dtype=np.int32)
    start[1:] = np.cumsum(np.bincount(bi, minlength=n))
    to_dev = lambda a: torch.from_numpy(np.ascontiguousarray(a, dtype=np.int32)).to(device)
    return to_dev(start), to_dev(bj[order])


def _left_id_limit(orig: torch.Tensor, n: int) -> int:
    if not n:
        return 0
    lo, hi = torch.stack(torch.aminmax(orig[:n])).tolist()
    return 0 if lo < 0 else int(hi) + 1


def _id_count(orig: torch.Tensor, n: int, what: str) -> int:
    ids = _left_id_limit(orig, n)
    if n and not ids:
        raise ValueError(f"{what}: caller ids must be >= 0")
    return ids


def _levels_top_k(entry: str, tables: tuple, left, right, device, k: int, threshold: float, category_mode: int, prune: bool,
                  banned, stats: Optional[list]) -> Hits:
    fn = getattr(_lib.load(), entry)
    if left.category_mode is not None:
        category_mode = left.category_mode
    structs = [t.struct() for t in tables]
    flags = _lib.FLAG_PRUNE if prune else 0
    bs, bj = banned_csr(banned, _id_count(left.orig, left.n, "banned") if banned is not None else 0, device)
    ptr = lambda t: 0 if t is None else t.data_ptr()
    return _top_k(lambda out, cnt, st, kk, stream: fn(
        *structs, float(threshold), kk, int(category_mode), flags, ptr(bs), ptr(bj), out.data_ptr(), cnt.data_ptr(),
        st.data_ptr(), stream), left.n, right.n, k, device, entry, stats)


def indel_levels_top_k(left: LevelItems, left_strings: StrTable, right: LevelItems, right_strings: StrTable, k: int,
                       threshold: float, category_mode: int = _lib.CAT_NONE, prune: bool = True, banned=None,
                       stats: Optional[list] = None) -> Hits:
    k = check_k(k)
    return _levels_top_k("nsm_indel_levels_top_k", (left, left_strings, right, right_strings), left, right, left.first.device,
                         k, threshold, category_mode, prune, banned, stats)


def jaccard_levels_top_k(left: SetTable, right: SetTable, k: int, threshold: float, category_mode: int = _lib.CAT_NONE,
                         prune: bool = True, banned=None, stats: Optional[list] = None) -> Hits:
    k = check_k(k)
    if left.nlev is None or right.nlev is None:
        raise ValueError("levels top-k needs tables built with SetTable.from_levels")
    if left.side != "left" or right.side != "right":
        raise ValueError("tables must be encoded with side='left' and side='right' (distinct padding)")
    return _levels_top_k("nsm_jaccard_levels_top_k", (left, right), left, right, left.ids.device, k, threshold,
                         category_mode, prune, banned, stats)


PROFILE_MAX_THRESHOLDS = 64


def check_thresholds(thresholds) -> np.ndarray:
    t = np.array(list(thresholds), dtype=np.float64).reshape(-1)
    if not 1 <= len(t) <= PROFILE_MAX_THRESHOLDS:
        raise ValueError(f"a profile takes 1 .. {PROFILE_MAX_THRESHOLDS} thresholds, got {len(t)}")
    if np.isnan(t).any():
        raise ValueError("thresholds must not be NaN")
    if (np.diff(t) <= 0).any():
        raise ValueError("thresholds must be strictly ascending")
    return t


@dataclass
class ThresholdProfile:

    thresholds: np.ndarray
    pairs: np.ndarray
    left_best: np.ndarray
    right_best: np.ndarray

    def matched_left(self) -> np.ndarray:
        return (self.left_best[None, :] >= self.thresholds[:, None]).sum(axis=1).astype(np.int64)

    def matched_right(self) -> np.ndarray:
        return (self.right_best[None, :] >= self.thresholds[:, None]).sum(axis=1).astype(np.int64)


def profile_of_hits(hits: Hits, thresholds, n_left: int, n_right: int) -> ThresholdProfile:
    t = check_thresholds(thresholds)
    keep = hits.score >= t[0]
    score, i, j = hits.score[keep], hits.i[keep], hits.j[keep]
    pairs = (len(score) - np.searchsorted(np.sort(score), t, side="left")).astype(np.uint64)
    left_best, right_best = np.full(int(n_left), -1.0), np.full(int(n_right), -1.0)
    np.maximum.at(left_best, i, score)
    np.maximum.at(right_best, j, score)
    return ThresholdProfile(t, pairs, left_best, right_best)


def merge_profiles(parts, thresholds, n_left: int, n_right: int) -> ThresholdProfile:
    t = check_thresholds(thresholds)
    out = ThresholdProfile(t, np.zeros(len(t), np.uint64), np.full(int(n_left), -1.0), np.full(int(n_right), -1.0))
    for prof, li, ri in parts:
        if not np.array_equal(prof.thresholds, t):
            raise ValueError("profiles of different ladders cannot be merged")
        out.pairs += prof.pairs
        np.maximum.at(out.left_best, np.asarray(li, dtype=np.int64), prof.left_best)
        np.maximum.at(out.right_best, np.asarray(ri, dtype=np.int64), prof.right_best)
    return out


def _profile(launch: Callable, t: np.ndarray, left_orig: torch.Tensor, n_left: int, right_orig: torch.Tensor, n_right: int,
             device, what: str, stats: Optional[list]) -> ThresholdProfile:
    import ctypes

    dev = _require_gpu(device)
    ids_l, ids_r = _id_count(left_orig, n_left, what), _id_count(right_orig, n_right, what)
    pairs = torch.zeros(len(t), dtype=torch.int64, device=dev)
    left_best = torch.full((max(1, ids_l),), -1.0, dtype=torch.float64, device=dev)
    right_best = torch.full((max(1, ids_r),), -1.0, dtype=torch.float64, device=dev)
    st = torch.zeros(4, dtype=torch.int64, device=dev)
    ladder = (ctypes.c_double * len(t))(*t.tolist())
    _lib.check(launch(ladder, len(t), pairs.data_ptr(), left_best.data_ptr(), right_best.data_ptr(), st.data_ptr(),
                      torch.cuda.current_stream(dev).cuda_stream), what)
    if stats is not None:
        stats[:] = [int(v) for v in st.tolist()]
    return ThresholdProfile(t, pairs.cpu().numpy().view(np.uint64), left_best[:ids_l].cpu().numpy(),
                            right_best[:ids_r].cpu().numpy())


def indel_raw_profile(left: StrTable, right: StrTable, thresholds, prune: bool = True,
                      stats: Optional[list] = None) -> ThresholdProfile:
    t = check_thresholds(thresholds)
    lib = _lib.load()
    ls, rs = left.struct(), right.struct()
    flags = _lib.FLAG_PRUNE if prune else 0
    return _profile(lambda lad, n, pairs, lb, rb, st, stream: lib.nsm_indel_raw_profile(ls, rs, lad, n, flags, pairs, lb, rb, st, stream),
                    t, left.orig, left.n, right.orig, right.n, left.codes.device, "nsm_indel_raw_profile", stats)


def jaccard_raw_profile(left: SetTable, right: SetTable, thresholds, prune: bool = True,
                        stats: Optional[list] = None) -> ThresholdProfile:
    t = check_thresholds(thresholds)
    if left.side != "left" or right.side != "right":
        raise ValueError("tables must be encoded with side='left' and side='right' (distinct padding)")
    if left.has_empty and right.has_empty:
        raise ZeroDivisionError("division by zero")
    lib = _lib.load()
    ls, rs = left.struct(), right.struct()
    flags = _lib.FLAG_PRUNE if prune else 0
    return _profile(lambda lad, n, pairs, lb, rb, st, stream: lib.nsm_jaccard_raw_profile(ls, rs, lad, n, flags, pairs, lb, rb, st, stream),
                    t, left.orig, left.n, right.orig, right.n, left.ids.device, "nsm_jaccard_raw_profile", stats)


def _levels_profile(entry: str, tables: tuple, left, right, device, t: np.ndarray, category_mode: int, prune: bool, banned,
                    stats: Optional[list]) -> ThresholdProfile:
    fn = getattr(_lib.load(), entry)
    if left.category_mode is not None:
        category_mode = left.category_mode
    structs = [tab.struct() for tab in tables]
    flags = _lib.FLAG_PRUNE if prune else 0
    bs, bj = banned_csr(banned, _id_count(left.orig, left.n, "banned") if banned is not None else 0, device)
    ptr = lambda x: 0 if x is None else x.data_ptr()
    return _profile(lambda lad, n, pairs, lb, rb, st, stream: fn(*structs, lad, n, int(category_mode), flags, ptr(bs), ptr(bj),
                                                                 pairs, lb, rb, st, stream),
                    t, left.orig, left.n, right.orig, right.n, device, entry, stats)


def indel_levels_profile(left: LevelItems, left_strings: StrTable, right: LevelItems, right_strings: StrTable, thresholds,
                         category_mode: int = _lib.CAT_NONE, prune: bool = True, banned=None,
                         stats: Optional[list] = None) -> ThresholdProfile:
    t = check_thresholds(thresholds)
    return _levels_profile("nsm_indel_levels_profile", (left, left_strings, right, right_strings), left, right,
                           left.first.device, t, category_mode, prune, banned, stats)


def jaccard_levels_profile(left: SetTable, right: SetTable, thresholds, category_mode: int = _lib.CAT_NONE, prune: bool = True,
                           banned=None, stats: Optional[list] = None) -> ThresholdProfile:
    t = check_thresholds(thresholds)
    if left.nlev is None or right.nlev is None:
        raise ValueError("levels profile needs tables built with SetTable.from_levels")
    if left.side != "left" or right.side != "right":
        raise ValueError("tables must be encoded with side='left' and side='right' (distinct padding)")
    return _levels_profile("nsm_jaccard_levels_profile", (left, right), left, right, left.ids.device, t, category_mode, prune,
                           banned, stats)


def check_margin(margin) -> float:
    if isinstance(margin, bool) or not isinstance(margin, (int, float, np.integer, np.floating)):
        raise ValueError(f"margin must be a finite number >= 0, got {margin!r}")
    m = float(margin)
    if not np.isfinite(m) or m < 0.0:
        raise ValueError(f"margin must be a finite number >= 0, got {margin!r}")
    return m


def _best_scores(hits: Hits, n_left: Optional[int], n_right: Optional[int]):
    nl = max(int(n_left or 0), int(hits.i.max()) + 1 if len(hits) else 0)
    nr = max(int(n_right or 0), int(hits.j.max()) + 1 if len(hits) else 0)
    lb, rb = np.full(nl, -np.inf), np.full(nr, -np.inf)
    np.maximum.at(lb, hits.i, hits.score)
    np.maximum.at(rb, hits.j, hits.score)
    return lb, rb


def _canonical(score: np.ndarray, i: np.ndarray, j: np.ndarray) -> Hits:
    order = np.lexsort((j, i, -score))
    return Hits(score[order], i[order], j[order])


def filter_by_floors(hits: Hits, left_floor=None, right_floor=None) -> Hits:
    keep = np.ones(len(hits), dtype=bool)
    if left_floor is not None:
        keep &= hits.score >= np.asarray(left_floor, dtype=np.float64)[hits.i]
    if right_floor is not None:
        keep &= hits.score >= np.asarray(right_floor, dtype=np.float64)[hits.j]
    return _canonical(hits.score[keep], hits.i[keep], hits.j[keep])


def best_of_hits(hits: Hits, margin: float = 0.0, mutual: bool = False, n_left: Optional[int] = None,
                 n_right: Optional[int] = None) -> Hits:
    m = check_margin(margin)
    lb, rb = _best_scores(hits, n_left, n_right)
    return filter_by_floors(hits, lb - m, rb - m if mutual else None)


def _floor_column(floor, ids: int, device, what: str) -> Optional[torch.Tensor]:
    if floor is None:
        return None
    if isinstance(floor, torch.Tensor):
        if floor.dim() != 1 or floor.dtype != torch.float64:
            raise ValueError(f"{what}: floors must be a one-dimensional float64 tensor")
        col = floor.to(device).contiguous()
    else:
        arr = np.ascontiguousarray(floor, dtype=np.float64)
        if arr.ndim != 1:
            raise ValueError(f"{what}: floors must be a one-dimensional float64 array")
        col = torch.from_numpy(arr).to(device)
    if int(col.shape[0]) < ids:
        raise ValueError(f"{what}: {int(col.shape[0])} floors for caller ids up to {ids - 1}")
    return col


def _floor_grid(entry: str, structs: list, middle: tuple, left, right, device, threshold: float, left_floor, right_floor,
                stats: Optional[list], capacity: Optional[int]) -> Hits:
    dev = _require_gpu(device)
    fn = getattr(_lib.load(), entry)
    ids_l, ids_r = _left_id_limit(left.orig, left.n), _left_id_limit(right.orig, right.n)
    if left_floor is not None:
        _id_count(left.orig, left.n, entry + ": left_floor")
    if right_floor is not None:
        _id_count(right.orig, right.n, entry + ": right_floor")
    lf = _floor_column(left_floor, ids_l, dev, entry + ": left_floor")
    rf = _floor_column(right_floor, ids_r, dev, entry + ": right_floor")
    st = torch.zeros(4, dtype=torch.int64, device=dev)
    ptr = lambda t: 0 if t is None or t.numel() == 0 else t.data_ptr()

    def launch(buf: HitBuffer, stream: int) -> int:
        st.zero_()
        return fn(*structs, float(threshold), ptr(lf), ptr(rf), *middle, buf.records.data_ptr(), buf.capacity,
                  buf.count.data_ptr(), st.data_ptr(), stream)

    hits = run_grid(launch, dev, capacity, entry, id_limit=max(ids_l, ids_r) if ids_l and ids_r else 0)
    if stats is not None:
        stats[:] = [int(v) for v in st.tolist()]
    return hits


def indel_raw_floor_grid(left: StrTable, right: StrTable, threshold: float, left_floor=None, right_floor=None,
                         prune: bool = True, stats: Optional[list] = None, capacity: Optional[int] = None) -> Hits:
    flags = _lib.FLAG_PRUNE if prune else 0
    return _floor_grid("nsm_indel_raw_floor_grid", [left.struct(), right.struct()], (flags,), left, right, left.codes.device,
                       threshold, left_floor, right_floor, stats, capacity)


def jaccard_raw_floor_grid(left: SetTable, right: SetTable, threshold: float, left_floor=None, right_floor=None,
                           prune: bool = True, stats: Optional[list] = None, capacity: Optional[int] = None) -> Hits:
    if left.side != "left" or right.side != "right":
        raise ValueError("tables must be encoded with side='left' and side='right' (distinct padding)")
    if left.has_empty and right.has_empty:
        raise ZeroDivisionError("division by zero")
    flags = _lib.FLAG_PRUNE if prune else 0
    return _floor_grid("nsm_jaccard_raw_floor_grid", [left.struct(), right.struct()], (flags,), left, right, left.ids.device,
                       threshold, left_floor, right_floor, stats, capacity)


def _levels_floor_grid(entry: str, tables: tuple, left, right, device, threshold: float, left_floor, right_floor,
                       category_mode: int, prune: bool, banned, stats: Optional[list], capacity: Optional[int]) -> Hits:
    if left.category_mode is not None:
        category_mode = left.category_mode
    bs, bj = banned_csr(banned, _id_count(left.orig, left.n, "banned") if banned is not None else 0, device)
    ptr = lambda t: 0 if t is None else t.data_ptr()
    middle = (int(category_mode), _lib.FLAG_PRUNE if prune else 0, ptr(bs), ptr(bj))
    return _floor_grid(entry, [t.struct() for t in tables], middle, left, right, device, threshold, left_floor, right_floor,
                       stats, capacity)


def indel_levels_floor_grid(left: LevelItems, left_strings: StrTable, right: LevelItems, right_strings: StrTable,
                            threshold: float, left_floor=None, right_floor=None, category_mode: int = _lib.CAT_NONE,
                            prune: bool = True, banned=None, stats: Optional[list] = None,
                            capacity: Optional[int] = None) -> Hits:
    return _levels_floor_grid("nsm_indel_levels_floor_grid", (left, left_strings, right, right_strings), left, right,
                              left.first.device, threshold, left_floor, right_floor, category_mode, prune, banned, stats, capacity)


def jaccard_levels_floor_grid(left: SetTable, right: SetTable, threshold: float, left_floor=None, right_floor=None,
                              category_mode: int = _lib.CAT_NONE, prune: bool = True, banned=None,
                              stats: Optional[list] = None, capacity: Optional[int] = None) -> Hits:
    if left.nlev is None or right.nlev is None:
        raise ValueError("levels floor grid needs tables built with SetTable.from_levels")
    if left.side != "left" or right.side != "right":
        raise ValueError("tables must be encoded with side='left' and side='right' (distinct padding)")
    return _levels_floor_grid("nsm_jaccard_levels_floor_grid", (left, right), left, right, left.ids.device, threshold,
                              left_floor, right_floor, category_mode, prune, banned, stats, capacity)


def floors_of_profile(prof: ThresholdProfile, margin: float, mutual: bool):
    m = check_margin(margin)
    return prof.left_best - m, (prof.right_best - m if mutual else None)


def _best(profile: Callable, floor_grid: Callable, margin: float, threshold: float, mutual: bool, stats: Optional[list]) -> Hits:
    m = check_margin(margin)
    t = check_thresholds([threshold])
    st1, st2 = [], []
    lf, rf = floors_of_profile(profile(t, st1), m, mutual)
    hits = floor_grid(lf, rf, st2)
    if stats is not None:
        stats[:] = [st1, st2]
    return hits


def indel_raw_best(left: StrTable, right: StrTable, margin: float = 0.0, threshold: float = 0.0, mutual: bool = False,
                   prune: bool = True, stats: Optional[list] = None) -> Hits:
    return _best(lambda t, st: indel_raw_profile(left, right, t, prune=prune, stats=st),
                 lambda lf, rf, st: indel_raw_floor_grid(left, right, threshold, lf, rf, prune=prune, stats=st),
                 margin, threshold, mutual, stats)


def jaccard_raw_best(left: SetTable, right: SetTable, margin: float = 0.0, threshold: float = 0.0, mutual: bool = False,
                     prune: bool = True, stats: Optional[list] = None) -> Hits:
    return _best(lambda t, st: jaccard_raw_profile(left, right, t, prune=prune, stats=st),
                 lambda lf, rf, st: jaccard_raw_floor_grid(left, right, threshold, lf, rf, prune=prune, stats=st),
                 margin, threshold, mutual, stats)


def indel_levels_best(left: LevelItems, left_strings: StrTable, right: LevelItems, right_strings: StrTable,
                      margin: float = 0.0, threshold: float = 0.0, mutual: bool = False, category_mode: int = _lib.CAT_NONE,
                      prune: bool = True, banned=None, stats: Optional[list] = None) -> Hits:
    tabs = (left, left_strings, right, right_strings)
    return _best(lambda t, st: indel_levels_profile(*tabs, t, category_mode=category_mode, prune=prune, banned=banned, stats=st),
                 lambda lf, rf, st: indel_levels_floor_grid(*tabs, threshold, lf, rf, category_mode=category_mode, prune=prune,
                                                            banned=banned, stats=st),
                 margin, threshold, mutual, stats)


def jaccard_levels_best(left: SetTable, right: SetTable, margin: float = 0.0, threshold: float = 0.0, mutual: bool = False,
                        category_mode: int = _lib.CAT_NONE, prune: bool = True, banned=None,
                        stats: Optional[list] = None) -> Hits:
    return _best(lambda t, st: jaccard_levels_profile(left, right, t, category_mode=category_mode, prune=prune, banned=banned, stats=st),
                 lambda lf, rf, st: jaccard_levels_floor_grid(left, right, threshold, lf, rf, category_mode=category_mode,
                                                              prune=prune, banned=banned, stats=st),
                 margin, threshold, mutual, stats)


NO_SCORE = -1.0


def check_pair_ids(i, j):
    i, j = np.asarray(i), np.asarray(j)
    for name, a in (("i", i), ("j", j)):
        if a.ndim != 1 or not (np.issubdtype(a.dtype, np.integer) or a.size == 0):
            raise ValueError(f"pairs: {name} must be a one-dimensional integer array")
    if i.shape != j.shape:
        raise ValueError(f"pairs: {len(i)} left ids for {len(j)} right ids")
    return i.astype(np.int64), j.astype(np.int64)


def _pair_keys(i: np.ndarray, j: np.ndarray) -> np.ndarray:
    return (i.astype(np.int64) << 32) | (j.astype(np.int64) & 0xFFFFFFFF)


def lookup_pairs(hits, i, j) -> np.ndarray:
    i, j = check_pair_ids(i, j)
    if not isinstance(hits, Hits):
        rec = list(hits)
        hits = Hits(np.array([r[0] for r in rec], dtype=np.float64), np.array([r[1] for r in rec], dtype=np.int32),
                    np.array([r[2] for r in rec], dtype=np.int32))
    out = np.full(len(i), NO_SCORE, dtype=np.float64)
    if len(hits) == 0 or len(i) == 0:
        return out
    keys = _pair_keys(hits.i, hits.j)
    order = np.argsort(keys, kind="stable")
    keys = keys[order]
    int32 = lambda a: (a >= -(1 << 31)) & (a < (1 << 31))
    fits = int32(i) & int32(j)
    want = _pair_keys(np.where(fits, i, 0), np.where(fits, j, 0))
    at = np.minimum(np.searchsorted(keys, want), len(keys) - 1)
    found = fits & (keys[at] == want)
    out[found] = hits.score[order[at[found]]]
    return out


def _row_map(orig: torch.Tensor, n: int, device) -> torch.Tensor:
    ids = _id_count(orig, n, "pairs")
    rows = torch.full((max(1, ids),), -1, dtype=torch.int32, device=device)
    if n:
        rows[orig[:n].long()] = torch.arange(n, dtype=torch.int32, device=device)
    return rows[:ids] if ids else rows[:0]


def _pairs(entry: str, tables: tuple, left, right, device, i, j) -> np.ndarray:
    i, j = check_pair_ids(i, j)
    dev = _require_gpu(device)
    fn = getattr(_lib.load(), entry)
    n = len(i)
    if n == 0:
        return np.zeros(0, dtype=np.float64)
    fits = lambda a: np.where((a >= 0) & (a < (1 << 31)), a, -1).astype(np.int32)
    host = np.zeros((n, 2), dtype=np.float64)
    ij = host.view(np.int32).reshape(n, 4)
    ij[:, 2], ij[:, 3] = fits(i), fits(j)
    records = torch.from_numpy(host).to(dev)
    lmap, rmap = _row_map(left.orig, left.n, dev), _row_map(right.orig, right.n, dev)
    structs = [t.struct() for t in tables]
    ptr = lambda t: t.data_ptr() if t.numel() else 0
    _lib.check(fn(*structs, ptr(lmap), int(lmap.numel()), ptr(rmap), int(rmap.numel()), records.data_ptr(), n,
                  torch.cuda.current_stream(dev).cuda_stream), entry)
    return records[:, 0].cpu().numpy()


def indel_raw_pairs(left: StrTable, right: StrTable, i, j) -> np.ndarray:
    i, j = check_pair_ids(i, j)
    return _pairs("nsm_indel_raw_pairs", (left, right), left, right, left.codes.device, i, j)


def jaccard_raw_pairs(left: SetTable, right: SetTable, i, j) -> np.ndarray:
    i, j = check_pair_ids(i, j)
    if left.side != "left" or right.side != "right":
        raise ValueError("tables must be encoded with side='left' and side='right' (distinct padding)")
    return _pairs("nsm_jaccard_raw_pairs", (left, right), left, right, left.ids.device, i, j)


def indel_levels_pairs(left: LevelItems, left_strings: StrTable, right: LevelItems, right_strings: StrTable, i, j) -> np.ndarray:
    i, j = check_pair_ids(i, j)
    return _pairs("nsm_indel_levels_pairs", (left, left_strings, right, right_strings), left, right, left.first.device, i, j)


def jaccard_levels_pairs(left: SetTable, right: SetTable, i, j) -> np.ndarray:
    i, j = check_pair_ids(i, j)
    if left.nlev is None or right.nlev is None:
        raise ValueError("levels pairs need tables built with SetTable.from_levels")
    if left.side != "left" or right.side != "right":
        raise ValueError("tables must be encoded with side='left' and side='right' (distinct padding)")
    return _pairs("nsm_jaccard_levels_pairs", (left, right), left, right, left.ids.device, i, j)


def jaccard_levels_grid(
    left: SetTable, right: SetTable, threshold: float, category_mode: int = _lib.CAT_NONE, prune: bool = True,
    capacity: Optional[int] = None, index: Optional[bool] = None, defer: bool = False,
) -> Hits:
    if left.nlev is None or right.nlev is None:
        raise ValueError("levels grid needs tables built with SetTable.from_levels")
    lib = _lib.load()
    ls, rs = left.struct(), right.struct()
    flags = (_lib.FLAG_PRUNE if prune else 0) | (0 if index is None else (_lib.FLAG_INDEX if index else _lib.FLAG_NO_INDEX))
    if index == "tile":
        flags |= _lib.FLAG_TILE_INDEX
    if (left.seg is None) != (right.seg is None) or left.category_mode != right.category_mode:
        raise ValueError("both sides must be encoded alike: same category_mode and partition (tables.partition_allowed)")
    if left.category_mode is not None:
        category_mode = left.category_mode

    def launch(buf: HitBuffer, stream: int) -> int:
        return lib.nsm_jaccard_levels_grid(
            ls, rs, float(threshold), int(category_mode), flags, buf.records.data_ptr(), buf.capacity,
            buf.count.data_ptr(), stream,
        )

    return run_grid(launch, left.ids.device, capacity, "nsm_jaccard_levels_grid", defer=defer)


PROBE_MIN_PAIRS = 1 << 27
PROBE_LEFT_ROWS = 8192
SPLIT_MAX_SURVIVAL = 0.10


def _visited_pairs(left: LevelItems, right: LevelItems) -> float:
    if left.seg_start is None or right.seg_start is None:
        return float(left.n) * float(right.n)
    a = left.seg_start.cpu().numpy().astype(np.float64)
    b = right.seg_start.cpu().numpy().astype(np.float64)
    return float(((a[1:] - a[:-1]) * (b[1:] - b[:-1])).sum())


def probe_survival(left: LevelItems, left_strings: StrTable, right: LevelItems, right_strings: StrTable, threshold: float,
                   category_mode: int):
    lib = _lib.load()
    dev = left.first.device
    k = max(1, left.n // PROBE_LEFT_ROWS)
    idx = torch.arange(0, left.n, k, device=dev)
    seg = seg_start = None
    if left.seg is not None:
        seg = left.seg[idx].contiguous()
        seg_start = torch.zeros(65, dtype=torch.int32, device=dev)
        seg_start[1:] = torch.cumsum(torch.bincount(seg, minlength=64)[:64], 0).to(torch.int32)
    sample = LevelItems(first=left.first[idx].contiguous(), nlev=left.nlev[idx].contiguous(), orig=left.orig[idx].contiguous(),
                        cat=None if left.cat is None else left.cat[idx].contiguous(), n=int(idx.numel()), seg=seg,
                        seg_start=seg_start, category_mode=left.category_mode)
    flags = _lib.FLAG_PRUNE | _lib.FLAG_SPLIT | _lib.FLAG_PROBE
    si, ls, ri, rs = sample.struct(), left_strings.struct(), right.struct(), right_strings.struct()
    if int(lib.nsm_indel_levels_workspace_bytes(si, ls, ri, rs, float(threshold), flags, 0.0)) == 0:
        return None
    ws = torch.zeros(64 + 2 * (1 << 16), dtype=torch.int64, device=dev)
    count = torch.zeros(1, dtype=torch.int64, device=dev)
    stream = torch.cuda.current_stream(dev).cuda_stream
    _lib.check(lib.nsm_indel_levels_grid(si, ls, ri, rs, float(threshold), int(category_mode), flags, 0, 0, count.data_ptr(),
                                         ws.data_ptr(), ws.numel() * 8, 1.0, stream), "nsm_indel_levels_grid (probe)")
    survivors = float(ws[2:64].sum().item())
    visited_sample = _visited_pairs(sample, right)
    visited = _visited_pairs(left, right)
    if visited_sample <= 0:
        return 0.0, visited
    return survivors / visited_sample * visited, visited


def route_one_word(left: LevelItems, left_strings: StrTable, right: LevelItems, right_strings: StrTable, threshold: float,
                   category_mode: int):
    got = probe_survival(left, left_strings, right, right_strings, threshold, category_mode)
    if got is None:
        return 0, 0.0, None
    expected, visited = got
    rate = expected / visited if visited > 0 else 0.0
    if rate <= SPLIT_MAX_SURVIVAL:
        return _lib.FLAG_SPLIT, max(1.0, 1.25 * expected), {"survival_rate": rate, "path": "split", "pairs_visited": visited}
    return _lib.FLAG_TILE, 0.0, {"survival_rate": rate, "path": "tile", "pairs_visited": visited}


def indel_levels_grid(
    left: LevelItems, left_strings: StrTable, right: LevelItems, right_strings: StrTable, threshold: float,
    category_mode: int = _lib.CAT_NONE, prune: bool = True, capacity: Optional[int] = None, wave_wide: bool = False,
    park: bool = False, workspace: Optional[int] = None, return_overflow: Optional[list] = None, defer: bool = False,
    probe: Optional[bool] = None, route: Optional[list] = None,
) -> Hits:
    lib = _lib.load()
    li, ls, ri, rs = left.struct(), left_strings.struct(), right.struct(), right_strings.struct()
    flags = (_lib.FLAG_PRUNE if prune else 0) | (_lib.FLAG_WAVE_WIDE if wave_wide else 0) | (_lib.FLAG_PARK if park else 0)
    if (left.seg is None) != (right.seg is None) or left.category_mode != right.category_mode:
        raise ValueError("both sides must be encoded alike: same category_mode and partition (tables.partition_allowed)")
    if left.category_mode is not None:
        category_mode = left.category_mode

    dev = left.first.device
    expected = 0.0
    if probe is None:
        probe = (workspace is None and prune and not wave_wide and not park and left_strings.stride == 64 and threshold > 0 and
                 float(left.n) * float(right.n) >= PROBE_MIN_PAIRS)
    if probe:
        extra, expected, measured = route_one_word(left, left_strings, right, right_strings, threshold, category_mode)
        flags |= extra
        if route is not None and measured is not None:
            route.append(dict(measured, expected_survivors=expected))
    want = int(lib.nsm_indel_levels_workspace_bytes(li, ls, ri, rs, float(threshold), flags, float(expected))) if workspace is None \
        else int(workspace)
    ws = split_workspace(want, dev) if want > 0 else None

    def launch(buf: HitBuffer, stream: int) -> int:
        return lib.nsm_indel_levels_grid(
            li, ls, ri, rs, float(threshold), int(category_mode), flags, buf.records.data_ptr(), buf.capacity,
            buf.count.data_ptr(), ws.data_ptr() if ws is not None else 0, ws.numel() * 8 if ws is not None else 0, float(expected),
            stream,
        )

    hits = run_grid(launch, dev, capacity, "nsm_indel_levels_grid", defer=defer)
    if ws is not None and return_overflow is not None:
        return_overflow.append(int(ws[1].item()) & 0xFFFFFFFF)
    return hits


def split_workspace(nbytes: int, device) -> Optional[torch.Tensor]:
    words = int(nbytes) // 8
    try:
        free, _total = torch.cuda.mem_get_info(device)
        words = min(words, int(free * 0.5) // 8)
    except RuntimeError:
        pass
    if words < 128:
        return None
    try:
        return torch.empty(words, dtype=torch.int64, device=device)
    except torch.cuda.OutOfMemoryError:
        return None


ASSIGN_ROUTES = {None: 0, "rounds": _lib.ASSIGN_ROUNDS_ONLY, "stream": _lib.ASSIGN_STREAM_ONLY}


def assign_of_hits(hits: Hits) -> Hits:
    h = _canonical(np.asarray(hits.score, np.float64), np.asarray(hits.i, np.int32), np.asarray(hits.j, np.int32))
    left, right, keep = set(), set(), []
    for r, (a, b) in enumerate(zip(h.i.tolist(), h.j.tolist())):
        if a not in left and b not in right:
            left.add(a)
            right.add(b)
            keep.append(r)
    keep = np.asarray(keep, dtype=np.int64)
    return Hits(h.score[keep], h.i[keep], h.j[keep])


def _assign_flags(route) -> int:
    if route not in ASSIGN_ROUTES:
        raise ValueError(f"route must be None, 'rounds' or 'stream', got {route!r}")
    return ASSIGN_ROUTES[route]


def assign_hits_device(buf: HitBuffer, n: int, n_left: int, n_right: int, id_limit: int = 0, route=None,
                       stats: Optional[list] = None) -> Hits:
    flags = _assign_flags(route)
    if n == 0:
        if stats is not None:
            stats[:] = [0, 0, 0, 0]
        return Hits(np.zeros(0, np.float64), np.zeros(0, np.int32), np.zeros(0, np.int32))
    fn = _lib.entry("nsm_assign_hits")
    lib = _lib.load()
    dev = buf.records.device
    stream = torch.cuda.current_stream(dev).cuda_stream
    limit = max(0, min(int(id_limit), 0x7FFFFFFF))
    scratch_ptr = 0
    if n > SMALL_SORT_MAX:
        if buf.scratch is None or buf.scratch.shape[0] < n:
            buf.scratch = torch.empty((n, 2), dtype=torch.float64, device=dev)
        scratch_ptr = buf.scratch.data_ptr()
    _lib.check(lib.nsm_sort_hits(buf.records.data_ptr(), scratch_ptr, buf.capacity, buf.count.data_ptr(), n, limit, stream),
               "nsm_sort_hits")
    out = HitBuffer(max(1, min(n, int(n_left), int(n_right))), dev)
    st = torch.zeros(4, dtype=torch.int64, device=dev)
    _lib.check(fn(buf.records.data_ptr(), n, int(n_left), int(n_right), flags, out.records.data_ptr(), out.count.data_ptr(),
                  st.data_ptr(), stream), "nsm_assign_hits")
    if stats is not None:
        stats[:] = [int(v) for v in st.tolist()]
    return sort_hits_device(out, int(out.count.item()), limit)


def assign_hits(hits: Hits, n_left: Optional[int] = None, n_right: Optional[int] = None, device=None, route=None,
                stats: Optional[list] = None) -> Hits:
    _assign_flags(route)
    dev = _require_gpu("cuda" if device is None else device)
    if dev.index is None:
        dev = torch.device("cuda", torch.cuda.current_device())
    h = _canonical(np.asarray(hits.score, np.float64), np.asarray(hits.i, np.int32), np.asarray(hits.j, np.int32))
    n = len(h)
    nl = max(int(n_left or 0), int(h.i.max()) + 1 if n else 0)
    nr = max(int(n_right or 0), int(h.j.max()) + 1 if n else 0)
    if n and (int(h.i.min()) < 0 or int(h.j.min()) < 0):
        raise ValueError("assign_hits: ids must be >= 0")
    buf = HitBuffer(n, dev)
    if n:
        host = np.empty((n, 2), dtype=np.float64)
        host[:, 0] = h.score
        ij = host.view(np.int32).reshape(n, 4)
        ij[:, 2], ij[:, 3] = h.i, h.j
        buf.records[:n] = torch.from_numpy(host).to(dev)
        buf.count.fill_(n)
    return assign_hits_device(buf, n, nl, nr, max(nl, nr), route, stats)


def _assign_pending(pending: PendingHits, left, right, route, stats: Optional[list]) -> Hits:
    ids_l, ids_r = _id_count(left.orig, left.n, "assign"), _id_count(right.orig, right.n, "assign")
    return assign_hits_device(pending.buf, pending.n, ids_l, ids_r, max(ids_l, ids_r) if ids_l and ids_r else 0, route, stats)


def indel_raw_assign(left: StrTable, right: StrTable, threshold: float, prune: bool = True, capacity: Optional[int] = None,
                     two_stage: bool = True, pack: Optional[bool] = None, route=None, stats: Optional[list] = None) -> Hits:
    pending = indel_raw_grid(left, right, threshold, prune=prune, capacity=capacity, two_stage=two_stage, pack=pack, defer=True)
    return _assign_pending(pending, left, right, route, stats)


def jaccard_raw_assign(left: SetTable, right: SetTable, threshold: float, prune: bool = True, capacity: Optional[int] = None,
                       index: Optional[bool] = None, route=None, stats: Optional[list] = None) -> Hits:
    pending = jaccard_raw_grid(left, right, threshold, prune=prune, capacity=capacity, index=index, defer=True)
    return _assign_pending(pending, left, right, route, stats)


def indel_levels_assign(left: LevelItems, left_strings: StrTable, right: LevelItems, right_strings: StrTable, threshold: float,
                        category_mode: int = _lib.CAT_NONE, prune: bool = True, capacity: Optional[int] = None, route=None,
                        stats: Optional[list] = None, **grid_options) -> Hits:
    pending = indel_levels_grid(left, left_strings, right, right_strings, threshold, category_mode=category_mode, prune=prune,
                                capacity=capacity, defer=True, **grid_options)
    return _assign_pending(pending, left, right, route, stats)


def jaccard_levels_assign(left: SetTable, right: SetTable, threshold: float, category_mode: int = _lib.CAT_NONE,
                          prune: bool = True, capacity: Optional[int] = None, index: Optional[bool] = None, route=None,
                          stats: Optional[list] = None) -> Hits:
    pending = jaccard_levels_grid(left, right, threshold, category_mode=category_mode, prune=prune, capacity=capacity,
                                  index=index, defer=True)
    return _assign_pending(pending, left, right, route, stats)


def _check_forest(start, nodes: int) -> np.ndarray:
    forest = np.asarray(start)
    if forest.shape != (nodes,) or not np.issubdtype(forest.dtype, np.integer):
        raise ValueError(f"start must be an integer array of {nodes} labels")
    if nodes and ((forest < 0).any() or (forest > np.arange(nodes)).any()):
        raise ValueError("start: every label[v] must lie in [0, v]")
    return forest.astype(np.int32)


def _list_nodes(hits: Hits, left_base: int, right_base: int, nodes: int, what: str):
    i, j = np.asarray(hits.i, dtype=np.int64), np.asarray(hits.j, dtype=np.int64)
    left_base, right_base = int(left_base), int(right_base)
    if left_base < 0 or right_base < 0 or left_base > nodes or right_base > nodes:
        raise ValueError(f"{what}: a list's bases must lie in [0, nodes]")
    if len(i) and (int(i.min()) < 0 or int(j.min()) < 0):
        raise ValueError(f"{what}: ids must be >= 0")
    if len(i) and (int(i.max()) + left_base >= nodes or int(j.max()) + right_base >= nodes):
        raise ValueError(f"{what}: a record reaches beyond the {nodes} nodes")
    return i + left_base, j + right_base


def groups_of_hits(lists, nodes: int, min_score: float = 0.0, start=None) -> np.ndarray:
    nodes = int(nodes)
    if nodes < 0:
        raise ValueError("groups_of_hits: nodes must be >= 0")
    parent = list(range(nodes)) if start is None else _check_forest(start, nodes).tolist()

    def find(v: int) -> int:
        while parent[v] != v:
            parent[v] = parent[parent[v]]
            v = parent[v]
        return v

    for hits, left_base, right_base in lists:
        u, v = _list_nodes(hits, left_base, right_base, nodes, "groups_of_hits")
        keep = np.asarray(hits.score, dtype=np.float64) >= min_score
        for a, b in zip(u[keep].tolist(), v[keep].tolist()):
            a, b = find(a), find(b)
            if a != b:
                parent[max(a, b)] = min(a, b)
    return np.fromiter((find(v) for v in range(nodes)), dtype=np.int32, count=nodes)


def _records_to_device(hits: Hits, dev) -> Optional[torch.Tensor]:
    n = len(hits)
    if n == 0:
        return None
    host = np.empty((n, 2), dtype=np.float64)
    host[:, 0] = hits.score
    ij = host.view(np.int32).reshape(n, 4)
    ij[:, 2], ij[:, 3] = hits.i, hits.j
    return torch.from_numpy(host).to(dev)


def group_lists_device(entries, nodes: int, min_score: float, dev, start=None, stats: Optional[list] = None) -> np.ndarray:
    fn = _lib.entry("nsm_group_hits")
    nodes = int(nodes)
    if nodes == 0:
        if stats is not None:
            stats[:] = [0, 0]
        return np.zeros(0, dtype=np.int32)
    flags = 0
    if start is None:
        label = torch.empty(nodes, dtype=torch.int32, device=dev)
    else:
        label = torch.from_numpy(_check_forest(start, nodes)).to(dev)
        flags = _lib.GROUP_CONTINUE
    lists = (_lib.NsmHitList * max(1, len(entries)))()
    for slot, (ptr, n, left_base, left_ids, right_base, right_ids) in zip(lists, entries):
        slot.hits, slot.n = (ptr if n else None), int(n)
        slot.left_base, slot.left_ids, slot.right_base, slot.right_ids = int(left_base), int(left_ids), int(right_base), int(right_ids)
    st = torch.zeros(2, dtype=torch.int64, device=dev) if stats is not None else None
    status = fn(lists, len(entries), nodes, float(min_score), flags, label.data_ptr(), st.data_ptr() if st is not None else None,
                torch.cuda.current_stream(dev).cuda_stream)
    if status == 10001:
        raise ValueError("nsm_group_hits: " + _lib.load().nsm_last_error().decode("utf-8", "replace"))
    _lib.check(status, "nsm_group_hits")
    if stats is not None:
        stats[:] = [int(v) for v in st.tolist()]
    return label.cpu().numpy()


def group_hits(lists, nodes: int, min_score: float = 0.0, start=None, device=None, stats: Optional[list] = None) -> np.ndarray:
    dev = _require_gpu("cuda" if device is None else device)
    if dev.index is None:
        dev = torch.device("cuda", torch.cuda.current_device())
    nodes = int(nodes)
    if nodes < 0:
        raise ValueError("group_hits: nodes must be >= 0")
    entries, keep = [], []
    for hits, left_base, right_base in lists:
        _list_nodes(hits, left_base, right_base, nodes, "group_hits")
        recs = _records_to_device(hits, dev)
        keep.append(recs)
        entries.append((recs.data_ptr() if recs is not None else 0, len(hits), int(left_base), nodes - int(left_base),
                        int(right_base), nodes - int(right_base)))
    return group_lists_device(entries, nodes, min_score, dev, start, stats)


@dataclass
class MatchGroups:

    label: np.ndarray
    bases: tuple
    cohort_sizes: tuple

    def of(self, c: int) -> np.ndarray:
        return self.label[self.bases[c]: self.bases[c] + self.cohort_sizes[c]]

    def sizes(self) -> np.ndarray:
        return np.bincount(self.label, minlength=len(self.label))

    def members(self, min_size: int = 2):
        order = np.argsort(self.label, kind="stable")
        sorted_label = self.label[order]
        starts = np.r_[0, np.flatnonzero(sorted_label[1:] != sorted_label[:-1]) + 1, len(order)] if len(order) else np.zeros(1, int)
        out = []
        for a, b in zip(starts[:-1].tolist(), starts[1:].tolist()):
            if b - a < min_size:
                continue
            nodes = order[a:b]
            out.append(tuple((nodes[(nodes >= base) & (nodes < base + size)] - base).astype(np.int64)
                             for base, size in zip(self.bases, self.cohort_sizes)))
        return out


def _groups_pending(pending: PendingHits, left, right, same: bool, min_score, stats: Optional[list]) -> MatchGroups:
    ids_l, ids_r = _id_count(left.orig, left.n, "groups"), _id_count(right.orig, right.n, "groups")
    if same:
        nodes, bases, sizes = max(ids_l, ids_r), (0,), (max(ids_l, ids_r),)
    else:
        nodes, bases, sizes = ids_l + ids_r, (0, ids_l), (ids_l, ids_r)
    floor = float("-inf") if min_score is None else float(min_score)
    label = group_lists_device([(pending.buf.records.data_ptr(), pending.n, 0, ids_l, bases[-1], ids_r)], nodes, floor,
                               pending.buf.records.device, None, stats)
    return MatchGroups(label, bases, sizes)


def indel_raw_groups(left: StrTable, right: StrTable, threshold: float, prune: bool = True, capacity: Optional[int] = None,
                     two_stage: bool = True, pack: Optional[bool] = None, same: bool = False, min_score: Optional[float] = None,
                     stats: Optional[list] = None) -> MatchGroups:
    pending = indel_raw_grid(left, right, threshold, prune=prune, capacity=capacity, two_stage=two_stage, pack=pack, defer=True)
    return _groups_pending(pending, left, right, same, min_score, stats)


def jaccard_raw_groups(left: SetTable, right: SetTable, threshold: float, prune: bool = True, capacity: Optional[int] = None,
                       index: Optional[bool] = None, same: bool = False, min_score: Optional[float] = None,
                       stats: Optional[list] = None) -> MatchGroups:
    pending = jaccard_raw_grid(left, right, threshold, prune=prune, capacity=capacity, index=index, defer=True)
    return _groups_pending(pending, left, right, same, min_score, stats)


def indel_levels_groups(left: LevelItems, left_strings: StrTable, right: LevelItems, right_strings: StrTable, threshold: float,
                        category_mode: int = _lib.CAT_NONE, prune: bool = True, capacity: Optional[int] = None, same: bool = False,
                        min_score: Optional[float] = None, stats: Optional[list] = None, **grid_options) -> MatchGroups:
    pending = indel_levels_grid(left, left_strings, right, right_strings, threshold, category_mode=category_mode, prune=prune,
                                capacity=capacity, defer=True, **grid_options)
    return _groups_pending(pending, left, right, same, min_score, stats)


def jaccard_levels_groups(left: SetTable, right: SetTable, threshold: float, category_mode: int = _lib.CAT_NONE,
                          prune: bool = True, capacity: Optional[int] = None, index: Optional[bool] = None, same: bool = False,
                          min_score: Optional[float] = None, stats: Optional[list] = None) -> MatchGroups:
    pending = jaccard_levels_grid(left, right, threshold, category_mode=category_mode, prune=prune, capacity=capacity,
                                  index=index, defer=True)
    return _groups_pending(pending, left, right, same, min_score, stats)


def _score_key(score: np.ndarray) -> np.ndarray:
    bits = np.ascontiguousarray(score, dtype=np.float64).view(np.uint64)
    flip = np.where(bits >> np.uint64(63), np.uint64(0xFFFFFFFFFFFFFFFF), np.uint64(1) << np.uint64(63))
    return ~(bits ^ flip)


def _check_cut(threshold, min_score: float, what: str) -> float:
    t = float(threshold)
    if not t >= min_score:
        raise ValueError(f"{what}: threshold {threshold!r} is not >= the forest's min_score {min_score!r}; "
                         "the forest does not know what links below it")
    return t


@dataclass
class MergeForest:

    score: np.ndarray
    u: np.ndarray
    v: np.ndarray
    nodes: int
    bases: tuple
    cohort_sizes: tuple
    min_score: float

    def __len__(self) -> int:
        return int(self.score.shape[0])

    def as_tuples(self):
        return list(zip(self.score.tolist(), self.u.tolist(), self.v.tolist()))

    def hits(self) -> Hits:
        return Hits(self.score, self.u, self.v)

    def cut(self, threshold: float) -> MatchGroups:
        t = _check_cut(threshold, self.min_score, "MergeForest.cut")
        return MatchGroups(groups_of_hits([(self.hits(), 0, 0)], self.nodes, t), self.bases, self.cohort_sizes)

    def ladder(self, thresholds) -> dict:
        ts = np.asarray([_check_cut(t, self.min_score, "MergeForest.ladder") for t in np.asarray(thresholds, dtype=np.float64).ravel()])
        out = {name: np.zeros(len(ts), dtype=np.int64) for name in ("components", "groups", "grouped", "largest")}
        parent, size = list(range(self.nodes)), [1] * self.nodes

        def find(x: int) -> int:
            while parent[x] != x:
                parent[x] = parent[parent[x]]
                x = parent[x]
            return x

        score, u, v = self.score.tolist(), self.u.tolist(), self.v.tolist()
        k, groups, grouped, largest = 0, 0, 0, min(self.nodes, 1)
        for slot in np.argsort(-ts, kind="stable").tolist():
            while k < len(score) and score[k] >= ts[slot]:
                a, b = find(u[k]), find(v[k])
                sa, sb = size[a], size[b]
                groups += 1 - (sa >= 2) - (sb >= 2)
                grouped += (sa if sa < 2 else 0) + (sb if sb < 2 else 0)
                parent[b], size[a] = a, sa + sb
                largest = max(largest, sa + sb)
                k += 1
            out["components"][slot], out["groups"][slot] = self.nodes - k, groups
            out["grouped"][slot], out["largest"][slot] = grouped, largest
        return out

    def merge_score(self, a, b) -> np.ndarray:
        a, b = np.asarray(a, dtype=np.int64).ravel(), np.asarray(b, dtype=np.int64).ravel()
        if a.shape != b.shape:
            raise ValueError("merge_score: a and b must have the same length")
        if len(a) and (min(int(a.min()), int(b.min())) < 0 or max(int(a.max()), int(b.max())) >= self.nodes):
            raise ValueError(f"merge_score: nodes must lie in [0, {self.nodes})")
        out = np.full(len(a), -1.0)
        out[a == b] = np.inf
        parent = list(range(self.nodes))
        open_at: dict = {}
        for q, (x, y) in enumerate(zip(a.tolist(), b.tolist())):
            if x != y:
                open_at.setdefault(x, set()).add(q)
                open_at.setdefault(y, set()).add(q)

        def find(x: int) -> int:
            while parent[x] != x:
                parent[x] = parent[parent[x]]
                x = parent[x]
            return x

        for s, x, y in zip(self.score.tolist(), self.u.tolist(), self.v.tolist()):
            x, y = find(x), find(y)
            qx, qy = open_at.pop(x, set()), open_at.pop(y, set())
            if len(qx) < len(qy):
                qx, qy = qy, qx
            for q in qy:
                if q in qx:
                    qx.discard(q)
                    out[q] = s
                else:
                    qx.add(q)
            parent[y] = x
            if qx:
                open_at[x] = qx
        return out


def _forest_layout(nodes: int, bases, cohort_sizes):
    return ((0,), (nodes,)) if bases is None else (tuple(bases), tuple(cohort_sizes))


def forest_of_hits(lists, nodes: int, min_score: float = 0.0, bases=None, cohort_sizes=None) -> MergeForest:
    nodes = int(nodes)
    if nodes < 0:
        raise ValueError("forest_of_hits: nodes must be >= 0")
    min_score = float(min_score)
    parts = []
    for hits, left_base, right_base in lists:
        a, b = _list_nodes(hits, left_base, right_base, nodes, "forest_of_hits")
        s = np.asarray(hits.score, dtype=np.float64)
        keep = (s >= min_score) & (a != b)
        parts.append((s[keep], np.minimum(a, b)[keep], np.maximum(a, b)[keep]))
    score = np.concatenate([p[0] for p in parts]) if parts else np.zeros(0, np.float64)
    lo = np.concatenate([p[1] for p in parts]) if parts else np.zeros(0, np.int64)
    hi = np.concatenate([p[2] for p in parts]) if parts else np.zeros(0, np.int64)
    order = np.lexsort((hi, lo, _score_key(score)))
    parent = list(range(nodes))

    def find(x: int) -> int:
        while parent[x] != x:
            parent[x] = parent[parent[x]]
            x = parent[x]
        return x

    taken = []
    for r, a, b in zip(order.tolist(), lo[order].tolist(), hi[order].tolist()):
        a, b = find(a), find(b)
        if a != b:
            parent[max(a, b)] = min(a, b)
            taken.append(r)
    taken = np.asarray(taken, dtype=np.int64)
    return MergeForest(score[taken], lo[taken].astype(np.int32), hi[taken].astype(np.int32), nodes,
                       *_forest_layout(nodes, bases, cohort_sizes), min_score)


def span_lists_device(entries, nodes: int, min_score: float, dev, stats: Optional[list] = None, bases=None,
                      cohort_sizes=None) -> MergeForest:
    fn = _lib.entry("nsm_span_hits")
    nodes = int(nodes)
    layout = _forest_layout(nodes, bases, cohort_sizes)
    if nodes == 0:
        if stats is not None:
            stats[:] = [0, 0, 0, 0]
        return MergeForest(np.zeros(0, np.float64), np.zeros(0, np.int32), np.zeros(0, np.int32), 0, *layout, float(min_score))
    lists = (_lib.NsmHitList * max(1, len(entries)))()
    for slot, (ptr, n, left_base, left_ids, right_base, right_ids) in zip(lists, entries):
        slot.hits, slot.n = (ptr if n else None), int(n)
        slot.left_base, slot.left_ids, slot.right_base, slot.right_ids = int(left_base), int(left_ids), int(right_base), int(right_ids)
    out = HitBuffer(max(1, nodes - 1), dev)
    st = torch.zeros(4, dtype=torch.int64, device=dev) if stats is not None else None
    status = fn(lists, len(entries), nodes, float(min_score), 0, out.records.data_ptr(),
                out.count.data_ptr(), None, st.data_ptr() if st is not None else None, torch.cuda.current_stream(dev).cuda_stream)
    if status == 10001:
        raise ValueError("nsm_span_hits: " + _lib.load().nsm_last_error().decode("utf-8", "replace"))
    _lib.check(status, "nsm_span_hits")
    if stats is not None:
        stats[:] = [int(v) for v in st.tolist()]
    taken = sort_hits_device(out, int(out.count.item()), nodes)
    return MergeForest(taken.score, taken.i, taken.j, nodes, *layout, float(min_score))


def span_hits(lists, nodes: int, min_score: float = 0.0, device=None, stats: Optional[list] = None, bases=None,
              cohort_sizes=None) -> MergeForest:
    dev = _require_gpu("cuda" if device is None else device)
    if dev.index is None:
        dev = torch.device("cuda", torch.cuda.current_device())
    nodes = int(nodes)
    if nodes < 0:
        raise ValueError("span_hits: nodes must be >= 0")
    entries, keep = [], []
    for hits, left_base, right_base in lists:
        _list_nodes(hits, left_base, right_base, nodes, "span_hits")
        recs = _records_to_device(hits, dev)
        keep.append(recs)
        entries.append((recs.data_ptr() if recs is not None else 0, len(hits), int(left_base), nodes - int(left_base),
                        int(right_base), nodes - int(right_base)))
    return span_lists_device(entries, nodes, min_score, dev, stats, bases, cohort_sizes)


def _forest_pending(pending: PendingHits, left, right, threshold: float, same: bool, min_score,
                    stats: Optional[list]) -> MergeForest:
    ids_l, ids_r = _id_count(left.orig, left.n, "forest"), _id_count(right.orig, right.n, "forest")
    if same:
        nodes, bases, sizes = max(ids_l, ids_r), (0,), (max(ids_l, ids_r),)
    else:
        nodes, bases, sizes = ids_l + ids_r, (0, ids_l), (ids_l, ids_r)
    floor = float("-inf") if min_score is None else float(min_score)
    forest = span_lists_device([(pending.buf.records.data_ptr(), pending.n, 0, ids_l, bases[-1], ids_r)], nodes, floor,
                               pending.buf.records.device, stats, bases, sizes)
    forest.min_score = max(floor, float(threshold))
    return forest


def indel_raw_forest(left: StrTable, right: StrTable, threshold: float, prune: bool = True, capacity: Optional[int] = None,
                     two_stage: bool = True, pack: Optional[bool] = None, same: bool = False, min_score: Optional[float] = None,
                     stats: Optional[list] = None) -> MergeForest:
    pending = indel_raw_grid(left, right, threshold, prune=prune, capacity=capacity, two_stage=two_stage, pack=pack, defer=True)
    return _forest_pending(pending, left, right, threshold, same, min_score, stats)


def jaccard_raw_forest(left: SetTable, right: SetTable, threshold: float, prune: bool = True, capacity: Optional[int] = None,
                       index: Optional[bool] = None, same: bool = False, min_score: Optional[float] = None,
                       stats: Optional[list] = None) -> MergeForest:
    pending = jaccard_raw_grid(left, right, threshold, prune=prune, capacity=capacity, index=index, defer=True)
    return _forest_pending(pending, left, right, threshold, same, min_score, stats)


def indel_levels_forest(left: LevelItems, left_strings: StrTable, right: LevelItems, right_strings: StrTable, threshold: float,
                        category_mode: int = _lib.CAT_NONE, prune: bool = True, capacity: Optional[int] = None, same: bool = False,
                        min_score: Optional[float] = None, stats: Optional[list] = None, **grid_options) -> MergeForest:
    pending = indel_levels_grid(left, left_strings, right, right_strings, threshold, category_mode=category_mode, prune=prune,
                                capacity=capacity, defer=True, **grid_options)
    return _forest_pending(pending, left, right, threshold, same, min_score, stats)


def jaccard_levels_forest(left: SetTable, right: SetTable, threshold: float, category_mode: int = _lib.CAT_NONE,
                          prune: bool = True, capacity: Optional[int] = None, index: Optional[bool] = None, same: bool = False,
                          min_score: Optional[float] = None, stats: Optional[list] = None) -> MergeForest:
    pending = jaccard_levels_grid(left, right, threshold, category_mode=category_mode, prune=prune, capacity=capacity,
                                  index=index, defer=True)
    return _forest_pending(pending, left, right, threshold, same, min_score, stats)
```

Baseline: 43390 billion pair-comparisons/s.

## Add opt-in persistent work-queue coarse kernel and enlarge packed row chunks

Adds a prepass that packs left rows and builds a per-tile work-item list from length-feasible row intervals. An optional persistent coarse kernel then pulls items from an atomic queue with adaptive grain, keeping right-tile fragments and hit stacks across items of the same tile. The persistent path is gated behind a compile macro or a new ONE_GROUP flag. Separately, the default packed launch now picks larger row chunks (half the target waves, cap 8192) to amortize per-block right-tile setup and drains, at the cost of coarser load balance.

```diff
diff --git a/include/nsm_hip.h b/include/nsm_hip.h
--- a/include/nsm_hip.h
+++ b/include/nsm_hip.h
@@ -81,6 +81,7 @@
 #define NSM_FLAG_ONE_STAGE 1024u
 #define NSM_FLAG_PACK 2048u
 #define NSM_FLAG_NO_PACK 4096u
+#define NSM_FLAG_ONE_GROUP 8192u
 #define NSM_FLAG_WAVE_WIDE 2u
 
 int nsm_abi_version(void);
diff --git a/napkon-string-matching_amd/csrc/indel_raw.hip b/napkon-string-matching_amd/csrc/indel_raw.hip
--- a/napkon-string-matching_amd/csrc/indel_raw.hip
+++ b/napkon-string-matching_amd/csrc/indel_raw.hip
@@ -1,6 +1,7 @@
 #include "nsm_common.hpp"
 #include "indel_score.hpp"
 
+#include <algorithm>
 #include <map>
 #include <mutex>
 #include <utility>
@@ -312,19 +313,24 @@
 #include "indel_raw_coarse.hpp"
 namespace nsm {
 
-static int pick_rows_per_chunk(int n_left, int n_tiles) {
 #ifndef NSM_C3_WANT_WAVES
 #define NSM_C3_WANT_WAVES (16ll * 256 * 32)
 #endif
-  const long long want_waves = NSM_C3_WANT_WAVES;
+#ifndef NSM_C3_CHUNK_MAX
+#define NSM_C3_CHUNK_MAX 4096
+#endif
+#ifndef NSM_C3C_PACK_WANT_WAVES
+#define NSM_C3C_PACK_WANT_WAVES (NSM_C3_WANT_WAVES / 2)
+#endif
+#ifndef NSM_C3C_PACK_CHUNK_MAX
+#define NSM_C3C_PACK_CHUNK_MAX 8192
+#endif
+static int pick_rows_per_chunk(int n_left, int n_tiles, long long want_waves = NSM_C3_WANT_WAVES, int chunk_max = NSM_C3_CHUNK_MAX) {
   long long chunks = (want_waves + n_tiles - 1) / (n_tiles > 0 ? n_tiles : 1);
   if (chunks < 1) chunks = 1;
   long long rows = (n_left + chunks - 1) / chunks;
   if (rows < 64) rows = 64;
-#ifndef NSM_C3_CHUNK_MAX
-#define NSM_C3_CHUNK_MAX 4096
-#endif
-  if (rows > NSM_C3_CHUNK_MAX) rows = NSM_C3_CHUNK_MAX;
+  if (rows > chunk_max) rows = chunk_max;
   return static_cast<int>(rows);
 }
 
@@ -353,6 +359,23 @@
   return w.rows;
 }
 
+static int device_cus() {
+  static std::mutex mu;
+  static std::map<int, int> cus;
+  int dev = 0;
+  if (hipGetDevice(&dev) != hipSuccess) return 256;
+  std::lock_guard<std::mutex> lock(mu);
+  auto it = cus.find(dev);
+  if (it != cus.end()) return it->second;
+  int n = 0;
+  if (hipDeviceGetAttribute(&n, hipDeviceAttributeMultiprocessorCount, dev) != hipSuccess || n < 1) {
+    (void)hipGetLastError();
+    n = 256;
+  }
+  cus[dev] = n;
+  return n;
+}
+
 void release_pack_scratch(int dev, void* stream, bool all) {
   std::lock_guard<std::mutex> lock(g_pack_mu);
   for (auto it = g_pack.begin(); it != g_pack.end();) {
@@ -449,8 +472,49 @@
       if (hipStreamIsCapturing(hs, &capture) != hipSuccess) capture = hipStreamCaptureStatusNone;
       pack = capture == hipStreamCaptureStatusNone;
     }
+    if (pack && (NSM_C3C_PERSIST || (flags & NSM_FLAG_ONE_GROUP))) {
+      C3pItemParams ip;
+      ip.n_left = left->n; ip.n_right = right->n; ip.n_tiles = n_tiles;
+      ip.item_rows = NSM_C3P_ITEM_ROWS > 0 ? (NSM_C3P_ITEM_ROWS + kC3cBlock - 1) / kC3cBlock * kC3cBlock : p.rows_per_chunk;
+      if (ip.item_rows > kC3pWindow) ip.item_rows = kC3pWindow;
+      ip.every_row = p.zero_need == 0;
+      for (int lb = 0; lb <= 64; ++lb) {
+        ip.la_lo[lb] = 65;
+        ip.la_hi[lb] = 0;
+        for (int la = 1; la <= 64 && lb > 0; ++la) {
+          if (std::min(la, lb) < static_cast<int>(p.lcsmin[la + lb])) continue;
+          if (ip.la_lo[lb] == 65) ip.la_lo[lb] = static_cast<uint8_t>(la);
+          ip.la_hi[lb] = static_cast<uint8_t>(la);
+        }
+      }
+      const long long item_cap = static_cast<long long>(n_tiles) * c3p_items_of(left->n, ip.item_rows);
+      const size_t rows_bytes = static_cast<size_t>(left->n) * kC3cPackedRow;
+      const size_t list_bytes = (static_cast<size_t>(item_cap) * sizeof(int4) + 63) / 64 * 64;
+      if (item_cap >= (1ll << 31)) pack = false;
+      ip.cap = static_cast<unsigned int>(item_cap);
+      char* kept = pack ? static_cast<char*>(pack_scratch(hs, list_bytes + kC3pQueueBytes + rows_bytes)) : nullptr;
+      if (kept) {
+        char* packed = kept + list_bytes + kC3pQueueBytes;
+        const long long units = 2ll * left->n;
+        const int item_blocks = (n_tiles + kBlock - 1) / kBlock;
+        hipLaunchKernelGGL(c3p_prepass_kernel, dim3(static_cast<unsigned>(item_blocks + (units + kBlock - 1) / kBlock)), dim3(kBlock), 0, hs,
+                           lh32, reinterpret_cast<c3c_v4i*>(packed), right->len, left->len_start, c3p_queue(packed), ip, item_blocks);
+        long long groups = std::min<long long>((item_cap + kWavesPerBlock - 1) / kWavesPerBlock, 4ll * device_cus());
+        if (groups < 1 || (flags & NSM_FLAG_ONE_GROUP)) groups = 1;
+        hipLaunchKernelGGL((indel_raw_coarse_kernel<NSM_C3C_NT, NSM_C3C_CAP, true, true>), dim3(static_cast<unsigned>(groups)), dim3(kBlock),
+                           c3c_lds_bytes(), hs, left->codes, left->len, left->len_start, left->orig, lh32, right->codes, right->len,
+                           right->orig, rh32, hits, hit_count, p, static_cast<const char*>(packed));
+        return hip_status(hipGetLastError(), "indel_raw_coarse_kernel launch (persistent)");
+      }
+    }
     void* packed = pack ? pack_scratch(hs, static_cast<size_t>(left->n) * kC3cPackedRow) : nullptr;
     if (packed) {
+      const int rows_packed =
+          (pick_rows_per_chunk(left->n, n_tiles, NSM_C3C_PACK_WANT_WAVES, NSM_C3C_PACK_CHUNK_MAX) + kC3cBlock - 1) / kC3cBlock * kC3cBlock;
+      if (rows_packed <= (1 << 15) && (left->n + rows_packed - 1) / rows_packed <= 65535) {
+        p.rows_per_chunk = rows_packed;
+        grid.y = (left->n + rows_packed - 1) / rows_packed;
+      }
       const long long units = 2ll * left->n;
       hipLaunchKernelGGL(c3c_pack_left_kernel, dim3(static_cast<unsigned>((units + kBlock - 1) / kBlock)), dim3(kBlock), 0, hs,
                          lh32, static_cast<c3c_v4i*>(packed), left->n);
diff --git a/napkon-string-matching_amd/csrc/indel_raw_coarse.hpp b/napkon-string-matching_amd/csrc/indel_raw_coarse.hpp
--- a/napkon-string-matching_amd/csrc/indel_raw_coarse.hpp
+++ b/napkon-string-matching_amd/csrc/indel_raw_coarse.hpp
@@ -31,6 +31,12 @@
 #endif
 #ifndef NSM_C3C_EARLY_OUT
 #define NSM_C3C_EARLY_OUT 1
+#endif
+#ifndef NSM_C3C_PERSIST
+#define NSM_C3C_PERSIST 0
+#endif
+#ifndef NSM_C3P_ITEM_ROWS
+#define NSM_C3P_ITEM_ROWS 0
 #endif
 constexpr int kC3cBlock = 32;
 constexpr int kC3cRights = NSM_C3C_NT * kC3cBlock;
@@ -129,9 +135,8 @@
   typedef c3c_packed_rows type;
 };
 
-__global__ __launch_bounds__(kBlock) void c3c_pack_left_kernel(const uint32_t* __restrict__ lhist, c3c_v4i* __restrict__ packed,
-                                                               int n_left) {
-  const int u = blockIdx.x * kBlock + threadIdx.x;
+__device__ __forceinline__ void c3c_pack_left_unit(const uint32_t* __restrict__ lhist, c3c_v4i* __restrict__ packed, int n_left,
+                                                   int u) {
   if (u >= 2 * n_left) return;
   const uint4 w = reinterpret_cast<const uint4*>(lhist)[u];
   const uint32_t ws[4] = {w.x, w.y, w.z, w.w};
@@ -146,11 +151,91 @@
   packed[2 * static_cast<size_t>(u)] = m1;
   packed[2 * static_cast<size_t>(u) + 1] = m2;
 }
+__global__ __launch_bounds__(kBlock) void c3c_pack_left_kernel(const uint32_t* __restrict__ lhist, c3c_v4i* __restrict__ packed,
+                                                               int n_left) {
+  c3c_pack_left_unit(lhist, packed, n_left, blockIdx.x * kBlock + threadIdx.x);
+}
+
+constexpr int kC3pWindow = 1 << 15;
+struct C3pItemParams {
+  int n_left, n_right, n_tiles, item_rows, every_row;
+  unsigned int cap;
+  uint8_t la_lo[65], la_hi[65];
+};
+__host__ __device__ static inline int c3p_items_of(int rows, int item_rows) {
+  const int per_window = (kC3pWindow + item_rows - 1) / item_rows;
+  return (rows >> 15) * per_window + ((rows & (kC3pWindow - 1)) + item_rows - 1) / item_rows;
+}
+constexpr int kC3pQueueBytes = 64;
+__host__ __device__ static inline unsigned int* c3p_queue(const char* lpacked) {
+  return reinterpret_cast<unsigned int*>(const_cast<char*>(lpacked) - kC3pQueueBytes);
+}
+__host__ __device__ static inline int4* c3p_item(unsigned int* queue, unsigned int k) {
+  return reinterpret_cast<int4*>(queue) - 1 - k;
+}
+__global__ __launch_bounds__(kBlock) void c3p_prepass_kernel(const uint32_t* __restrict__ lhist, c3c_v4i* __restrict__ packed,
+                                                             const int32_t* __restrict__ rlen, const int32_t* __restrict__ lstart,
+                                                             unsigned int* __restrict__ queue,
+                                                             const C3pItemParams ip, int item_blocks) {
+  if (static_cast<int>(blockIdx.x) >= item_blocks) {
+    c3c_pack_left_unit(lhist, packed, ip.n_left, (static_cast<int>(blockIdx.x) - item_blocks) * kBlock + static_cast<int>(threadIdx.x));
+    return;
+  }
+  __shared__ unsigned long long s_scan[kBlock];
+  const int tid = threadIdx.x;
+  auto interval = [&](int t, int& r0) -> int {
+    r0 = 0;
+    if (ip.every_row) return ip.n_left;
+    const int j_a = t * kC3cRights, j_b = min(j_a + kC3cRights, ip.n_right) - 1;
+    const int lb_a = min(max(rlen[j_a], 0), 64), lb_b = min(max(rlen[j_b], 0), 64);
+    int lo = 65, hi = 0;
+    for (int lb = min(lb_a, lb_b); lb <= max(lb_a, lb_b); ++lb) {
+      lo = min(lo, static_cast<int>(ip.la_lo[lb]));
+      hi = max(hi, static_cast<int>(ip.la_hi[lb]));
+    }
+    if (hi < lo) return 0;
+    r0 = lstart[64 - hi];
+    return lstart[64 - lo + 1] - r0;
+  };
+  unsigned int before = 0u;
+  for (int t = tid; t < static_cast<int>(blockIdx.x) * kBlock; t += kBlock) {
+    int r0;
+    before += static_cast<unsigned int>(c3p_items_of(interval(t, r0), ip.item_rows));
+  }
+  const int tile = static_cast<int>(blockIdx.x) * kBlock + tid;
+  int r0 = 0, rows = 0;
+  if (tile < ip.n_tiles) rows = interval(tile, r0);
+  const unsigned int own = static_cast<unsigned int>(c3p_items_of(rows, ip.item_rows));
+  unsigned long long v = (static_cast<unsigned long long>(before) << 32) | own;
+  s_scan[tid] = v;
+  __syncthreads();
+  for (int d = 1; d < kBlock; d <<= 1) {
+    const unsigned long long add = tid >= d ? s_scan[tid - d] : 0ull;
+    __syncthreads();
+    v += add;
+    s_scan[tid] = v;
+    __syncthreads();
+  }
+  const unsigned long long total = s_scan[kBlock - 1];
+  const unsigned int carry = static_cast<unsigned int>(total >> 32);
+  unsigned int at = carry + static_cast<unsigned int>(v) - own;
+  const int per_window = (kC3pWindow + ip.item_rows - 1) / ip.item_rows;
+  for (unsigned int k = 0; k < own; ++k, ++at) {
+    const int base = r0 + (static_cast<int>(k) / per_window) * kC3pWindow;
+    const int first = base + (static_cast<int>(k) % per_window) * ip.item_rows;
+    const int end = min(first + ip.item_rows, min(base + kC3pWindow, r0 + rows));
+    if (at < ip.cap) *c3p_item(queue, at) = make_int4(tile, first, end, base);
+  }
+  if (static_cast<int>(blockIdx.x) == item_blocks - 1 && tid == 0) {
+    queue[0] = 0u;
+    queue[1] = min(carry + static_cast<unsigned int>(total), ip.cap);
+  }
+}
 
 #ifndef NSM_C3C_OCC
 #define NSM_C3C_OCC __attribute__((amdgpu_waves_per_eu((NSM_C3C_ORFOLD && PACKED) ? 4 : 2)))
 #endif
-template <int NT, int CAP, bool PACKED>
+template <int NT, int CAP, bool PACKED, bool PERSIST = false>
 __global__ __launch_bounds__(kBlock) NSM_C3C_OCC void indel_raw_coarse_kernel(
     const uint8_t* __restrict__ lcodes, const int32_t* __restrict__ llen, const int32_t* __restrict__ lstart,
     const int32_t* __restrict__ lorig, const uint32_t* __restrict__ lhist, const uint8_t* __restrict__ rcodes,
@@ -158,6 +243,7 @@
     nsm_hit* __restrict__ hits, unsigned long long* __restrict__ count, const IndelRawParams p,
     const char* __restrict__ lpacked) {
   static_assert(!PACKED || NSM_C3C_FP4, "only the FP4 scan has packed left rows");
+  static_assert(!PERSIST || PACKED, "the persistent launch is the packed scan's");
   constexpr int kRights = NT * kC3cBlock;
   static_assert(kC3cDrainAt >= kWave && kC3cDrainAt + (NT + kC3cPipeExtra) * kWave <= kC3cStack,
                 "the drain is triggered above kC3cDrainAt entries and runs full passes");
@@ -176,15 +262,15 @@
   const int wave = threadIdx.x >> 6;
   const int col = lane & (kC3cBlock - 1);
   const int half = lane >> 5;
-  const int j0 = (blockIdx.x * kWavesPerBlock + wave) * kRights;
-  if (j0 >= p.n_right) return;
+  int j0 = (blockIdx.x * kWavesPerBlock + wave) * kRights;
+  if (!PERSIST && j0 >= p.n_right) return;
   auto lane_again = [&]() -> int {
     int l = lane;
     asm volatile("" : "+v"(l));
     return l;
   };
 #if NSM_C3C_EARLY_OUT
-  if (p.zero_need != 0) {
+  if (!PERSIST && p.zero_need != 0) {
     const int ie = blockIdx.y * p.rows_per_chunk;
     const int la_hi = llen[ie], la_lo = llen[min(p.n_left, ie + p.rows_per_chunk) - 1];
     bool fits = false;
@@ -205,457 +291,515 @@
   uint32_t* rh_lds = s_rh + wave * 8 * kRights;
   uint8_t* rl_lds = s_rl + wave * kRights;
 
-#pragma unroll
-  for (int k = 0; k < (kRights + kWave - 1) / kWave; ++k) {
-    const int rl = k * kWave + lane;
-    if (rl < kRights) {
-      const int j = j0 + rl;
-      const int jcl = j < p.n_right ? j : p.n_right - 1;
-      const uint4* fp = reinterpret_cast<const uint4*>(rhist + static_cast<size_t>(jcl) * 8);
-      const uint4 f0 = fp[0], f1 = fp[1];
-      uint32_t* dst = rh_lds + rl;
-      dst[0 * kRights] = f0.x; dst[1 * kRights] = f0.y; dst[2 * kRights] = f0.z; dst[3 * kRights] = f0.w;
-      dst[4 * kRights] = f1.x; dst[5 * kRights] = f1.y; dst[6 * kRights] = f1.z; dst[7 * kRights] = f1.w;
-      rl_lds[rl] = static_cast<uint8_t>(j < p.n_right ? rlen[jcl] : 0);
-    }
-  }
   bool valid[NT];
+  c3c_v4i bfrag[NT][NSM_C3C_FP4 ? 2 : CAP];
+  uint32_t bscales = 0u;
+  int q_cnt = 0;
+  int i0 = 0, ifirst = 0, i1 = 0;
+  int it_cur = 0, it_end = 0;
+  bool other_tile = true;
+  if constexpr (PERSIST) j0 = -1;
+  do {
+    if constexpr (PERSIST) {
+      unsigned int* queue = c3p_queue(lpacked);
+      if (it_cur >= it_end) {
+        const unsigned int n_items = static_cast<unsigned int>(__builtin_amdgcn_readfirstlane(static_cast<int>(queue[1])));
+        unsigned int start = 0u, grain = 0u;
+        if (lane == 0) {
+          const unsigned int seen = *reinterpret_cast<volatile unsigned int*>(queue);
+          const unsigned int left = seen < n_items ? n_items - seen : 0u;
+          grain = max(1u, left / (2u * gridDim.x * kWavesPerBlock));
+          start = atomicAdd(queue, grain);
+        }
+        const unsigned int s = static_cast<unsigned int>(__builtin_amdgcn_readfirstlane(static_cast<int>(start)));
+        const unsigned int g = static_cast<unsigned int>(__builtin_amdgcn_readfirstlane(static_cast<int>(grain)));
+        if (s >= n_items) return;
+        it_cur = static_cast<int>(s);
+        it_end = static_cast<int>(min(s + g, n_items));
+      }
+      const int4 it = *c3p_item(queue, static_cast<unsigned int>(it_cur++));
+      const int j_it = __builtin_amdgcn_readfirstlane(it.x) * kRights;
+      other_tile = j_it != j0;
+      j0 = j_it;
+      ifirst = __builtin_amdgcn_readfirstlane(it.y);
+      i1 = __builtin_amdgcn_readfirstlane(it.z);
+      i0 = __builtin_amdgcn_readfirstlane(it.w);
+    }
+    if (!PERSIST || other_tile) {
+      int ln = lane;
+      if constexpr (PERSIST) ln = lane_again();
+#pragma unroll
+      for (int k = 0; k < (kRights + kWave - 1) / kWave; ++k) {
+        const int rl = k * kWave + ln;
+        if (rl < kRights) {
+          const int j = j0 + rl;
+          const int jcl = j < p.n_right ? j : p.n_right - 1;
+          const uint4* fp = reinterpret_cast<const uint4*>(rhist + static_cast<size_t>(jcl) * 8);
+          const uint4 f0 = fp[0], f1 = fp[1];
+          uint32_t* dst = rh_lds + rl;
+          dst[0 * kRights] = f0.x; dst[1 * kRights] = f0.y; dst[2 * kRights] = f0.z; dst[3 * kRights] = f0.w;
+          dst[4 * kRights] = f1.x; dst[5 * kRights] = f1.y; dst[6 * kRights] = f1.z; dst[7 * kRights] = f1.w;
+          rl_lds[rl] = static_cast<uint8_t>(j < p.n_right ? rlen[jcl] : 0);
+        }
+      }
+    }
 #if NSM_C3C_FP4
-  c3c_v4i bfrag[NT][2];
-  uint32_t bscales = 0u;
-  auto scale_base = [](int t) -> uint32_t { return (kOrFold && t % 2 == 0) ? 0x7fu + 9u : 0x7fu; };
-  uint32_t bscales1 = 0u;
-  if constexpr (kOrFold) {
-#pragma unroll
-    for (int t = 0; t < NT; ++t) bscales1 |= scale_base(t) << (8 * t);
-    asm volatile("" : "+v"(bscales1));
-  }
-  auto code_tile = [&](int t, const uint4& f, int k) __attribute__((always_inline)) {
-    const uint32_t ws[4] = {f.x, f.y, f.z, f.w};
-    if (k == 0) {
-#pragma unroll
-      for (int q = 0; q < 4; ++q) {
-        int m1, m2;
-        c3c_fp4_right_k0(ws[q], m1, m2);
-        bfrag[t][0][q] = m1;
-        bfrag[t][1][q] = m2;
-      }
-    } else {
-#pragma unroll
-      for (int q = 0; q < 4; ++q) {
-        int m1, m2;
-        c3c_fp4_right_scaled(ws[q], k, m1, m2);
-        bfrag[t][0][q] = m1;
-        bfrag[t][1][q] = m2;
-      }
-    }
-  };
-#pragma unroll
-  for (int t = 0; t < NT; ++t) {
-    const int j = j0 + t * kC3cBlock + col;
-    valid[t] = j < p.n_right;
-    const int jcl = valid[t] ? j : p.n_right - 1;
-    const uint4* fp = reinterpret_cast<const uint4*>(rhist + static_cast<size_t>(jcl) * 8);
-    const uint4 f0 = fp[0], f1 = fp[1];
-    const int k = c3c_fp4_scale(f0, f1);
-    bscales |= (scale_base(t) + static_cast<uint32_t>(k)) << (8 * t);
-    uint4 f = half ? f1 : f0;
-    if (!valid[t]) f = make_uint4(0u, 0u, 0u, 0u);
-    code_tile(t, f, k);
-  }
-  auto make_bfrag = [&]() __attribute__((always_inline)) {
-    const int l = lane_again();
-    const uint32_t* rp0 = rh_lds + (4 * (l >> 5)) * kRights + (l & (kC3cBlock - 1));
-#pragma unroll
-    for (int t = 0; t < NT; ++t) {
-      const uint32_t* rp = rp0 + t * kC3cBlock;
-      const int k = static_cast<int>(((bscales >> (8 * t)) & 0xffu) - scale_base(t));
-      uint4 f = make_uint4(rp[0], rp[kRights], rp[2 * kRights], rp[3 * kRights]);
-      if (!valid[t]) f = make_uint4(0u, 0u, 0u, 0u);
-      code_tile(t, f, k);
-    }
-  };
-  __builtin_amdgcn_fence(__ATOMIC_ACQ_REL, "wavefront");
-  __builtin_amdgcn_wave_barrier();
-#else
-  c3c_v4i bfrag[NT][CAP];
-  auto code_b = [&](int t, int q, uint32_t fw) {
-    const uint32_t full = c3c_ge64(fw, CAP);
-#pragma unroll
-    for (int s = 0; s < CAP - 1; ++s)
-      bfrag[t][s][q] = static_cast<int>((c3c_ge64(fw, s + 1) ^ full) >> 6);
-    bfrag[t][CAP - 1][q] = static_cast<int>(full);
-  };
-#pragma unroll
-  for (int t = 0; t < NT; ++t) {
-    const int j = j0 + t * kC3cBlock + col;
-    valid[t] = j < p.n_right;
-    const int jcl = valid[t] ? j : p.n_right - 1;
-    uint4 f = reinterpret_cast<const uint4*>(rhist + static_cast<size_t>(jcl) * 8)[half];
-    if (!valid[t]) f = make_uint4(0u, 0u, 0u, 0u);
-    code_b(t, 0, f.x); code_b(t, 1, f.y); code_b(t, 2, f.z); code_b(t, 3, f.w);
-  }
-  auto make_bfrag = [&]() {
-#pragma unroll
-    for (int t = 0; t < NT; ++t) {
-      const uint32_t* rp = rh_lds + (4 * half) * kRights + t * kC3cBlock + col;
-#pragma unroll
-      for (int q = 0; q < 4; ++q) code_b(t, q, valid[t] ? rp[q * kRights] : 0u);
-    }
-  };
-  __builtin_amdgcn_fence(__ATOMIC_ACQ_REL, "wavefront");
-  __builtin_amdgcn_wave_barrier();
-#endif
-  const int i0 = blockIdx.y * p.rows_per_chunk;
-  const int i1 = min(p.n_left, i0 + p.rows_per_chunk);
-  int q_cnt = 0;
-
-  auto need_of = [&](int la, int lb) -> int { return (la == 0 || lb == 0) ? p.zero_need : static_cast<int>(s_lcsmin[la + lb]); };
-
-  const char* chunk = reinterpret_cast<const char*>(lhist + static_cast<size_t>(i0) * 8);
-  const char* pchunk = PACKED ? lpacked + static_cast<size_t>(i0) * kC3cPackedRow : nullptr;
-
-  auto drain_pass = [&]() __attribute__((always_inline)) {
+    auto scale_base = [](int t) -> uint32_t { return (kOrFold && t % 2 == 0) ? 0x7fu + 9u : 0x7fu; };
+    uint32_t bscales1 = 0u;
+    if constexpr (kOrFold) {
+#pragma unroll
+      for (int t = 0; t < NT; ++t) bscales1 |= scale_base(t) << (8 * t);
+      asm volatile("" : "+v"(bscales1));
+    }
+    auto code_tile = [&](int t, const uint4& f, int k) __attribute__((always_inline)) {
+      const uint32_t ws[4] = {f.x, f.y, f.z, f.w};
+      if (k == 0) {
+#pragma unroll
+        for (int q = 0; q < 4; ++q) {
+          int m1, m2;
+          c3c_fp4_right_k0(ws[q], m1, m2);
+          bfrag[t][0][q] = m1;
+          bfrag[t][1][q] = m2;
+        }
+      } else {
+#pragma unroll
+        for (int q = 0; q < 4; ++q) {
+          int m1, m2;
+          c3c_fp4_right_scaled(ws[q], k, m1, m2);
+          bfrag[t][0][q] = m1;
+          bfrag[t][1][q] = m2;
+        }
+      }
+    };
+    if (!PERSIST || other_tile) {
+      bscales = 0u;
+      int col_r = col, half_r = half;
+      if constexpr (PERSIST) {
+        const int l = lane_again();
+        col_r = l & (kC3cBlock - 1);
+        half_r = l >> 5;
+      }
+#pragma unroll
+      for (int t = 0; t < NT; ++t) {
+        const int j = j0 + t * kC3cBlock + col_r;
+        valid[t] = j < p.n_right;
+        const int jcl = valid[t] ? j : p.n_right - 1;
+        const uint4* fp = reinterpret_cast<const uint4*>(rhist + static_cast<size_t>(jcl) * 8);
+        const uint4 f0 = fp[0], f1 = fp[1];
+        const int k = c3c_fp4_scale(f0, f1);
+        bscales |= (scale_base(t) + static_cast<uint32_t>(k)) << (8 * t);
+        uint4 f = half_r ? f1 : f0;
+        if (!valid[t]) f = make_uint4(0u, 0u, 0u, 0u);
+        code_tile(t, f, k);
+      }
+    }
+    auto make_bfrag = [&]() __attribute__((always_inline)) {
+      const int l = lane_again();
+      const uint32_t* rp0 = rh_lds + (4 * (l >> 5)) * kRights + (l & (kC3cBlock - 1));
+#pragma unroll
+      for (int t = 0; t < NT; ++t) {
+        const uint32_t* rp = rp0 + t * kC3cBlock;
+        const int k = static_cast<int>(((bscales >> (8 * t)) & 0xffu) - scale_base(t));
+        uint4 f = make_uint4(rp[0], rp[kRights], rp[2 * kRights], rp[3 * kRights]);
+        if (!valid[t]) f = make_uint4(0u, 0u, 0u, 0u);
+        code_tile(t, f, k);
+      }
+    };
     __builtin_amdgcn_fence(__ATOMIC_ACQ_REL, "wavefront");
     __builtin_amdgcn_wave_barrier();
-    const int n = min(q_cnt, kWave);
-    const int base = q_cnt - n;
-    q_cnt = base;
+#else
+    auto code_b = [&](int t, int q, uint32_t fw) {
+      const uint32_t full = c3c_ge64(fw, CAP);
+#pragma unroll
+      for (int s = 0; s < CAP - 1; ++s)
+        bfrag[t][s][q] = static_cast<int>((c3c_ge64(fw, s + 1) ^ full) >> 6);
+      bfrag[t][CAP - 1][q] = static_cast<int>(full);
+    };
+#pragma unroll
+    for (int t = 0; t < NT; ++t) {
+      const int j = j0 + t * kC3cBlock + col;
+      valid[t] = j < p.n_right;
+      const int jcl = valid[t] ? j : p.n_right - 1;
+      uint4 f = reinterpret_cast<const uint4*>(rhist + static_cast<size_t>(jcl) * 8)[half];
+      if (!valid[t]) f = make_uint4(0u, 0u, 0u, 0u);
+      code_b(t, 0, f.x); code_b(t, 1, f.y); code_b(t, 2, f.z); code_b(t, 3, f.w);
+    }
+    auto make_bfrag = [&]() {
+#pragma unroll
+      for (int t = 0; t < NT; ++t) {
+        const uint32_t* rp = rh_lds + (4 * half) * kRights + t * kC3cBlock + col;
+#pragma unroll
+        for (int q = 0; q < 4; ++q) code_b(t, q, valid[t] ? rp[q * kRights] : 0u);
+      }
+    };
+    __builtin_amdgcn_fence(__ATOMIC_ACQ_REL, "wavefront");
+    __builtin_amdgcn_wave_barrier();
+#endif
+    if constexpr (!PERSIST) {
+      i0 = ifirst = blockIdx.y * p.rows_per_chunk;
+      i1 = min(p.n_left, i0 + p.rows_per_chunk);
+    }
+
+    auto need_of = [&](int la, int lb) -> int { return (la == 0 || lb == 0) ? p.zero_need : static_cast<int>(s_lcsmin[la + lb]); };
+
+    const char* chunk = reinterpret_cast<const char*>(lhist + static_cast<size_t>(i0) * 8);
+    const char* pchunk = PACKED ? lpacked + static_cast<size_t>(i0) * kC3cPackedRow : nullptr;
+
+    auto drain_pass = [&]() __attribute__((always_inline)) {
+      __builtin_amdgcn_fence(__ATOMIC_ACQ_REL, "wavefront");
+      __builtin_amdgcn_wave_barrier();
+      const int n = min(q_cnt, kWave);
+      const int base = q_cnt - n;
+      q_cnt = base;
 #ifdef NSM_C3C_X_NODRAIN
-    return;
-#endif
-    const int m = lane & 3;
-    uint32_t mask = 0;
+      return;
+#endif
+      const int m = lane & 3;
+      uint32_t mask = 0;
 #pragma nounroll
-    for (int s = (n - 1) >> 4; s >= 0; --s) {
-      const int e = 16 * s + (lane >> 2);
-      const bool active = e < n;
-      const unsigned long long ent = stack[base + (active ? e : 0)];
-      const int n_rows = active ? static_cast<int>(static_cast<uint32_t>(ent)) : 0;
-      const uint32_t ehi = static_cast<uint32_t>(ent >> 32);
-      const uint32_t ib_rel = active ? ehi >> 15 : 0u;
-      const int r0 = 4 * static_cast<int>((ehi >> 5) & 1u) + m;
-      const uint32_t last_r = static_cast<uint32_t>(max(n_rows, 1) - 1);
-      uint4 w0[4], w1[4];
-#pragma unroll
-      for (int g = 0; g < 4; ++g) {
-        const uint4* lp = reinterpret_cast<const uint4*>(chunk + (ib_rel + min(static_cast<uint32_t>(r0 + 8 * g), last_r)) * 32u);
-        w0[g] = lp[0];
-        w1[g] = lp[1];
-      }
-      const int la = static_cast<int>((ehi >> 8) & 127u);
-      const int tl = static_cast<int>((ehi >> 6) & 3u) * kC3cBlock + static_cast<int>(ehi & 31u);
-      const int lb = rl_lds[tl];
-      uint32_t rq[8];
-      {
-        const uint32_t* rp = rh_lds + tl;
-#pragma unroll
-        for (int q = 0; q < 8; ++q) rq[q] = rp[q * kRights];
-      }
-      const int nd = need_of(la, lb);
-      const int budget = (active && min(la, lb) >= nd) ? la + lb - 2 * nd : -1;
-      const uint32_t sad0 = ~static_cast<uint32_t>(budget);
-#pragma unroll
-      for (int g = 3; g >= 0; --g) {
-        uint32_t l1 = sad0;
-        l1 = __builtin_amdgcn_sad_u8(w0[g].x, rq[0], l1);
-        l1 = __builtin_amdgcn_sad_u8(w0[g].y, rq[1], l1);
-        l1 = __builtin_amdgcn_sad_u8(w0[g].z, rq[2], l1);
-        l1 = __builtin_amdgcn_sad_u8(w0[g].w, rq[3], l1);
-        l1 = __builtin_amdgcn_sad_u8(w1[g].x, rq[4], l1);
-        l1 = __builtin_amdgcn_sad_u8(w1[g].y, rq[5], l1);
-        l1 = __builtin_amdgcn_sad_u8(w1[g].z, rq[6], l1);
-        l1 = __builtin_amdgcn_sad_u8(w1[g].w, rq[7], l1);
-        if (r0 + 8 * g >= n_rows) l1 = 0u;
-        mask = __builtin_amdgcn_alignbit(mask, l1, 31);
-      }
-    }
+      for (int s = (n - 1) >> 4; s >= 0; --s) {
+        const int e = 16 * s + (lane >> 2);
+        const bool active = e < n;
+        const unsigned long long ent = stack[base + (active ? e : 0)];
+        const int n_rows = active ? static_cast<int>(static_cast<uint32_t>(ent)) : 0;
+        const uint32_t ehi = static_cast<uint32_t>(ent >> 32);
+        const uint32_t ib_rel = active ? ehi >> 15 : 0u;
+        const int r0 = 4 * static_cast<int>((ehi >> 5) & 1u) + m;
+        const uint32_t last_r = static_cast<uint32_t>(max(n_rows, 1) - 1);
+        uint4 w0[4], w1[4];
+#pragma unroll
+        for (int g = 0; g < 4; ++g) {
+          const uint4* lp = reinterpret_cast<const uint4*>(chunk + (ib_rel + min(static_cast<uint32_t>(r0 + 8 * g), last_r)) * 32u);
+          w0[g] = lp[0];
+          w1[g] = lp[1];
+        }
+        const int la = static_cast<int>((ehi >> 8) & 127u);
+        const int tl = static_cast<int>((ehi >> 6) & 3u) * kC3cBlock + static_cast<int>(ehi & 31u);
+        const int lb = rl_lds[tl];
+        uint32_t rq[8];
+        {
+          const uint32_t* rp = rh_lds + tl;
+#pragma unroll
+          for (int q = 0; q < 8; ++q) rq[q] = rp[q * kRights];
+        }
+        const int nd = need_of(la, lb);
+        const int budget = (active && min(la, lb) >= nd) ? la + lb - 2 * nd : -1;
+        const uint32_t sad0 = ~static_cast<uint32_t>(budget);
+#pragma unroll
+        for (int g = 3; g >= 0; --g) {
+          uint32_t l1 = sad0;
+          l1 = __builtin_amdgcn_sad_u8(w0[g].x, rq[0], l1);
+          l1 = __builtin_amdgcn_sad_u8(w0[g].y, rq[1], l1);
+          l1 = __builtin_amdgcn_sad_u8(w0[g].z, rq[2], l1);
+          l1 = __builtin_amdgcn_sad_u8(w0[g].w, rq[3], l1);
+          l1 = __builtin_amdgcn_sad_u8(w1[g].x, rq[4], l1);
+          l1 = __builtin_amdgcn_sad_u8(w1[g].y, rq[5], l1);
+          l1 = __builtin_amdgcn_sad_u8(w1[g].z, rq[6], l1);
+          l1 = __builtin_amdgcn_sad_u8(w1[g].w, rq[7], l1);
+          if (r0 + 8 * g >= n_rows) l1 = 0u;
+          mask = __builtin_amdgcn_alignbit(mask, l1, 31);
+        }
+      }
 #ifdef NSM_C3C_X_NOLCS
-    mask = 0u;
+      mask = 0u;
 #endif
 #ifdef NSM_C3C_X_FINEONLY
-    mask = p.n_left < 0 ? mask : 0u;
-#endif
-    unsigned long long todo = __ballot(mask != 0u);
-    uint32_t cur = 0u;
-    int leader = 0, row_s = 0, j_n = 0, la_n = 0, lb_n = 0;
-    auto next_pair = [&]() -> bool {
-      if (cur == 0u) {
-        if (todo == 0ull) return false;
-        leader = __builtin_ctzll(todo);
-        todo &= todo - 1ull;
-        cur = static_cast<uint32_t>(__builtin_amdgcn_readlane(static_cast<int>(mask), leader));
-      }
-      const int pos = 31 - __builtin_clz(cur);
-      cur &= ~(1u << pos);
-      const uint32_t ehi = static_cast<uint32_t>(
-          __builtin_amdgcn_readfirstlane(static_cast<int>(stack[base + 16 * (pos >> 2) + (leader >> 2)] >> 32)));
-      const int tl = static_cast<int>((ehi >> 6) & 3u) * kC3cBlock + static_cast<int>(ehi & 31u);
-      row_s = i0 + static_cast<int>(ehi >> 15) + 8 * (pos & 3) + 4 * static_cast<int>((ehi >> 5) & 1u) + (leader & 3);
-      j_n = j0 + tl;
-      la_n = static_cast<int>((ehi >> 8) & 127u);
-      lb_n = __builtin_amdgcn_readfirstlane(static_cast<int>(rl_lds[tl]));
-      return true;
+      mask = p.n_left < 0 ? mask : 0u;
+#endif
+      unsigned long long todo = __ballot(mask != 0u);
+      uint32_t cur = 0u;
+      int leader = 0, row_s = 0, j_n = 0, la_n = 0, lb_n = 0;
+      auto next_pair = [&]() -> bool {
+        if (cur == 0u) {
+          if (todo == 0ull) return false;
+          leader = __builtin_ctzll(todo);
+          todo &= todo - 1ull;
+          cur = static_cast<uint32_t>(__builtin_amdgcn_readlane(static_cast<int>(mask), leader));
+        }
+        const int pos = 31 - __builtin_clz(cur);
+        cur &= ~(1u << pos);
+        const uint32_t ehi = static_cast<uint32_t>(
+            __builtin_amdgcn_readfirstlane(static_cast<int>(stack[base + 16 * (pos >> 2) + (leader >> 2)] >> 32)));
+        const int tl = static_cast<int>((ehi >> 6) & 3u) * kC3cBlock + static_cast<int>(ehi & 31u);
+        row_s = i0 + static_cast<int>(ehi >> 15) + 8 * (pos & 3) + 4 * static_cast<int>((ehi >> 5) & 1u) + (leader & 3);
+        j_n = j0 + tl;
+        la_n = static_cast<int>((ehi >> 8) & 127u);
+        lb_n = __builtin_amdgcn_readfirstlane(static_cast<int>(rl_lds[tl]));
+        return true;
+      };
+      auto row_units = [&](uint32_t& lc, uint32_t& rc) {
+        lc = lcodes[static_cast<size_t>(row_s) * 64 + lane];
+        rc = rcodes[static_cast<size_t>(j_n) * 64 + lane];
+      };
+      uint32_t lc_next = 0, rc_next = 0;
+      bool have = next_pair();
+      if (NSM_C3C_LCS_PREFETCH && have) row_units(lc_next, rc_next);
+      while (have) {
+        const int row_c = row_s, j_s = j_n, la_s = la_n, lb_s = lb_n;
+        const int need_s = need_of(la_s, lb_s);
+        uint32_t lc = lc_next, rc = rc_next;
+        if (!NSM_C3C_LCS_PREFETCH) row_units(lc, rc);
+        have = next_pair();
+        if (NSM_C3C_LCS_PREFETCH && have) row_units(lc_next, rc_next);
+        const int lcs = raw_lcs_units(lc, la_s, rc, lb_s, need_s, lane);
+#ifdef NSM_C3C_X_COUNTLCS
+        if (lane == 0)
+#else
+        if (lcs >= need_s && lane == 0)
+#endif
+          emit_hit(hits, p.cap, count, indel_score(la_s, lb_s, lcs), lorig[row_c], rorig[j_s]);
+      }
     };
-    auto row_units = [&](uint32_t& lc, uint32_t& rc) {
-      lc = lcodes[static_cast<size_t>(row_s) * 64 + lane];
-      rc = rcodes[static_cast<size_t>(j_n) * 64 + lane];
+    auto drain_full = [&]() __attribute__((always_inline)) {
+      while (q_cnt >= kWave) drain_pass();
+      make_bfrag();
     };
-    uint32_t lc_next = 0, rc_next = 0;
-    bool have = next_pair();
-    if (NSM_C3C_LCS_PREFETCH && have) row_units(lc_next, rc_next);
-    while (have) {
-      const int row_c = row_s, j_s = j_n, la_s = la_n, lb_s = lb_n;
-      const int need_s = need_of(la_s, lb_s);
-      uint32_t lc = lc_next, rc = rc_next;
-      if (!NSM_C3C_LCS_PREFETCH) row_units(lc, rc);
-      have = next_pair();
-      if (NSM_C3C_LCS_PREFETCH && have) row_units(lc_next, rc_next);
-      const int lcs = raw_lcs_units(lc, la_s, rc, lb_s, need_s, lane);
-#ifdef NSM_C3C_X_COUNTLCS
-      if (lane == 0)
+
+    const int c_first = 64 - llen[ifirst];
+    const int c_last = 64 - llen[i1 - 1];
+    uint32_t lane_off = static_cast<uint32_t>(col * 32 + half * 16);
+    if constexpr (PERSIST) {
+      const int l = lane_again();
+      lane_off = static_cast<uint32_t>((l & (kC3cBlock - 1)) * 32 + (l >> 5) * 16);
+    }
+    for (int c = c_first; c <= c_last; ++c) {
+      const int a = max(ifirst, lstart[c]);
+      const int b = min(i1, lstart[c + 1]);
+      if (a >= b) continue;
+      const int la = 64 - c;
+      int need2[2] = {static_cast<int>(kNever), static_cast<int>(kNever)};
+      int nm1[NT];
+      bool some = false;
+      const int l_c = lane_again();
+#pragma unroll
+      for (int t = 0; t < NT; ++t) {
+        const int lb = rl_lds[t * kC3cBlock + (l_c & (kC3cBlock - 1))];
+        const int nd = valid[t] ? need_of(la, lb) : static_cast<int>(kNever);
+        const bool fits = min(la, lb) >= nd;
+        some = some || fits;
+#if NSM_C3C_FP4
+        if constexpr (kOrFold)
+          need2[t & 1] = min(need2[t & 1], fits ? nd : static_cast<int>(kNever));
+        else
+          nm1[t] = __float_as_int(static_cast<float>(fits ? nd : static_cast<int>(kNever)) - 0.5f);
 #else
-      if (lcs >= need_s && lane == 0)
-#endif
-        emit_hit(hits, p.cap, count, indel_score(la_s, lb_s, lcs), lorig[row_c], rorig[j_s]);
-    }
-  };
-  auto drain_full = [&]() __attribute__((always_inline)) {
-    while (q_cnt >= kWave) drain_pass();
-    make_bfrag();
-  };
-
-  const int c_first = 64 - llen[i0];
-  const int c_last = 64 - llen[i1 - 1];
-  const uint32_t lane_off = static_cast<uint32_t>(col * 32 + half * 16);
-  for (int c = c_first; c <= c_last; ++c) {
-    const int a = max(i0, lstart[c]);
-    const int b = min(i1, lstart[c + 1]);
-    if (a >= b) continue;
-    const int la = 64 - c;
-    int need2[2] = {static_cast<int>(kNever), static_cast<int>(kNever)};
-    int nm1[NT];
-    bool some = false;
-    const int l_c = lane_again();
-#pragma unroll
-    for (int t = 0; t < NT; ++t) {
-      const int lb = rl_lds[t * kC3cBlock + (l_c & (kC3cBlock - 1))];
-      const int nd = valid[t] ? need_of(la, lb) : static_cast<int>(kNever);
-      const bool fits = min(la, lb) >= nd;
-      some = some || fits;
+        nm1[t] = 64 * (fits ? nd : static_cast<int>(kNever)) - 1;
+#endif
+      }
+      if (!__any(some)) continue;
+      c3c_v16f bias;
+      const float bias1 = __int_as_float(0x4b000000 | ((256 - need2[0]) << 9) | (256 - need2[1]));
+      auto make_bias = [&]() {
+#pragma unroll
+        for (int k = 0; k < 16; ++k) {
+          float x;
+          asm volatile("v_mov_b32 %0, %1" : "=v"(x) : "v"(bias1));
+          bias[k] = x;
+        }
+      };
+
+      typedef typename c3c_rows<PACKED>::type rows_t;
+      const uint32_t last_off = static_cast<uint32_t>(b - 1 - i0) * (PACKED ? 64u : 32u) + static_cast<uint32_t>((l_c >> 5) * (PACKED ? 32 : 16));
+      auto load_rows = [&](int i) -> rows_t {
+        if constexpr (PACKED) {
+          const uint32_t off = min(static_cast<uint32_t>(i - i0) * 64u + 2u * lane_off, last_off);
+          const c3c_v4i* pp = reinterpret_cast<const c3c_v4i*>(pchunk + off);
+          return c3c_packed_rows{pp[0], pp[1]};
+        } else {
+          const uint32_t off = min(static_cast<uint32_t>(i - i0) * 32u + lane_off, last_off);
+          return *reinterpret_cast<const uint4*>(chunk + off);
+        }
+      };
 #if NSM_C3C_FP4
-      if constexpr (kOrFold)
-        need2[t & 1] = min(need2[t & 1], fits ? nd : static_cast<int>(kNever));
-      else
-        nm1[t] = __float_as_int(static_cast<float>(fits ? nd : static_cast<int>(kNever)) - 0.5f);
+      typedef c3c_v16f acc_t;
+      c3c_v4i afrag[2];
+      auto make_afrag = [&](const rows_t& w) {
+        if constexpr (!PACKED) {
+          const uint32_t ws[4] = {w.x, w.y, w.z, w.w};
+#pragma unroll
+          for (int q = 0; q < 4; ++q) {
+            int m1, m2;
+            c3c_fp4_left(ws[q], m1, m2);
+            afrag[0][q] = m1;
+            afrag[1][q] = m2;
+          }
+        }
+      };
+      constexpr int NU = kOrFold ? NT / 2 : NT;
+      auto chain = [&](int u, const rows_t& w) -> acc_t {
+        if constexpr (kOrFold) {
+          acc_t acc = c3c_fp4_mfma2(w.m1, bfrag[2 * u][0], bias, static_cast<int>(bscales1), 2 * u);
+          acc = c3c_fp4_mfma2(w.m2, bfrag[2 * u][1], acc, static_cast<int>(bscales), 2 * u);
+          acc = c3c_fp4_mfma2(w.m1, bfrag[2 * u + 1][0], acc, static_cast<int>(bscales1), 2 * u + 1);
+          return c3c_fp4_mfma2(w.m2, bfrag[2 * u + 1][1], acc, static_cast<int>(bscales), 2 * u + 1);
+        } else if constexpr (PACKED) {
+          return c3c_fp4_mfma2(w.m2, bfrag[u][1], c3c_fp4_mfma1(w.m1, bfrag[u][0]), static_cast<int>(bscales), u);
+        } else {
+          return c3c_fp4_mfma2(afrag[1], bfrag[u][1], c3c_fp4_mfma1(afrag[0], bfrag[u][0]), static_cast<int>(bscales), u);
+        }
+      };
+      auto fold = [&](const acc_t& acc) -> int {
+        const c3c_v16i bits = __builtin_bit_cast(c3c_v16i, acc);
+        if constexpr (kOrFold) {
+          int top = bits[0] | bits[1] | bits[2];
+#pragma unroll
+          for (int k = 3; k < 15; k += 2) top = top | bits[k] | bits[k + 1];
+          return (top | bits[15]) & (kFlagHi | kFlagLo);
+        } else {
+          int top = max(max(bits[0], bits[1]), bits[2]);
+#pragma unroll
+          for (int k = 3; k < 15; k += 2) top = max(max(top, bits[k]), bits[k + 1]);
+          return max(top, bits[15]);
+        }
+      };
 #else
-      nm1[t] = 64 * (fits ? nd : static_cast<int>(kNever)) - 1;
-#endif
-    }
-    if (!__any(some)) continue;
-    c3c_v16f bias;
-    const float bias1 = __int_as_float(0x4b000000 | ((256 - need2[0]) << 9) | (256 - need2[1]));
-    auto make_bias = [&]() {
-#pragma unroll
-      for (int k = 0; k < 16; ++k) {
-        float x;
-        asm volatile("v_mov_b32 %0, %1" : "=v"(x) : "v"(bias1));
-        bias[k] = x;
-      }
-    };
-
-    typedef typename c3c_rows<PACKED>::type rows_t;
-    const uint32_t last_off = static_cast<uint32_t>(b - 1 - i0) * (PACKED ? 64u : 32u) + static_cast<uint32_t>((l_c >> 5) * (PACKED ? 32 : 16));
-    auto load_rows = [&](int i) -> rows_t {
-      if constexpr (PACKED) {
-        const uint32_t off = min(static_cast<uint32_t>(i - i0) * 64u + 2u * lane_off, last_off);
-        const c3c_v4i* pp = reinterpret_cast<const c3c_v4i*>(pchunk + off);
-        return c3c_packed_rows{pp[0], pp[1]};
-      } else {
-        const uint32_t off = min(static_cast<uint32_t>(i - i0) * 32u + lane_off, last_off);
-        return *reinterpret_cast<const uint4*>(chunk + off);
-      }
-    };
+      typedef c3c_v16i acc_t;
+      constexpr int NU = NT;
+      c3c_v4i afrag[CAP - 1];
+      auto make_afrag = [&](const uint4& w) {
+#pragma unroll
+        for (int s = 0; s < CAP - 1; ++s) {
+          afrag[s].x = static_cast<int>(c3c_ge64(w.x, s + 1)); afrag[s].y = static_cast<int>(c3c_ge64(w.y, s + 1));
+          afrag[s].z = static_cast<int>(c3c_ge64(w.z, s + 1)); afrag[s].w = static_cast<int>(c3c_ge64(w.w, s + 1));
+        }
+      };
+      auto chain = [&](int t, const uint4& w) -> c3c_v16i {
+        c3c_v16i acc = {0, 0, 0, 0, 0, 0, 0, 0, 0, 0, 0, 0, 0, 0, 0, 0};
+#pragma unroll
+        for (int s = 0; s < CAP - 1; ++s) acc = __builtin_amdgcn_mfma_i32_32x32x32_i8(afrag[s], bfrag[t][s], acc, 0, 0, 0);
+        const c3c_v4i last = {static_cast<int>(w.x), static_cast<int>(w.y), static_cast<int>(w.z), static_cast<int>(w.w)};
+        return __builtin_amdgcn_mfma_i32_32x32x32_i8(last, bfrag[t][CAP - 1], acc, 0, 0, 0);
+      };
+      auto fold = [&](const c3c_v16i& acc) -> int {
+        int top = max(max(acc[0], acc[1]), acc[2]);
+#pragma unroll
+        for (int k = 3; k < 15; k += 2) top = max(max(top, acc[k]), acc[k + 1]);
+        return max(top, acc[15]);
+      };
+#endif
+      auto push = [&](bool ps, unsigned long long m, int t, int i) {
+        if (m == 0ull) return;
+#ifdef NSM_C3C_X_COUNTPUSH
+        if (lane == 0) atomicAdd(count, static_cast<unsigned long long>(__popcll(m)));
+#endif
+        if (ps) {
+          const int slot = __builtin_amdgcn_mbcnt_hi(static_cast<uint32_t>(m >> 32), __builtin_amdgcn_mbcnt_lo(static_cast<uint32_t>(m), static_cast<uint32_t>(q_cnt)));
+          const uint32_t hi = (static_cast<uint32_t>(i - i0) << 15) | (static_cast<uint32_t>(la) << 8) | (static_cast<uint32_t>(t) << 6);
+          uint32_t el = static_cast<uint32_t>(lane);
+          asm volatile("" : "+v"(el));
+          const uint32_t n_rows = static_cast<uint32_t>(min(kC3cBlock, b - i));
+          stack[slot] = (static_cast<unsigned long long>(hi | el) << 32) | n_rows;
+        }
+        q_cnt += __popcll(m);
+      };
+      auto finish = [&](int top, int u, int i) {
+        if constexpr (kOrFold) {
+          if (__ballot(top != 0) == 0ull) return;
+          const bool hi = (top & kFlagHi) != 0 && valid[2 * u], lo = (top & kFlagLo) != 0 && valid[2 * u + 1];
+          push(hi, __ballot(hi), 2 * u, i);
+          push(lo, __ballot(lo), 2 * u + 1, i);
+        } else {
+          const bool ps = top > nm1[u];
+          push(ps, __ballot(ps), u, i);
+        }
+      };
+#if NSM_C3C_PIPE
+      static_assert(NU % 2 == 0, "unit 0 of the next block takes the accumulator of unit NU: NU must be even (or NSM_C3C_PIPE=0)");
+      acc_t acc[2];
+      auto block = [&](int i, rows_t& wc, rows_t& wn) __attribute__((always_inline)) -> bool {
+        const bool more = i + kC3cBlock < b;
+        bool flush = false;
+#pragma unroll
+        for (int t = 0; t < NU; ++t) {
+          if (t + 1 < NU) {
+            acc[(t + 1) & 1] = chain(t + 1, wc);
+          } else {
+            flush = q_cnt > kC3cDrainAt;
+            if (kOrFold || (more && !flush)) {
+              make_afrag(wn);
+              if constexpr (PACKED) asm volatile("" : "+v"(wn.m1), "+v"(wn.m2));
+              if (i + 2 * kC3cBlock < b) wc = load_rows(i + 2 * kC3cBlock);
+              acc[0] = chain(0, wn);
+            }
+          }
+          const int top = fold(acc[t & 1]);
 #if NSM_C3C_FP4
-    typedef c3c_v16f acc_t;
-    c3c_v4i afrag[2];
-    auto make_afrag = [&](const rows_t& w) {
-      if constexpr (!PACKED) {
-        const uint32_t ws[4] = {w.x, w.y, w.z, w.w};
-#pragma unroll
-        for (int q = 0; q < 4; ++q) {
-          int m1, m2;
-          c3c_fp4_left(ws[q], m1, m2);
-          afrag[0][q] = m1;
-          afrag[1][q] = m2;
-        }
-      }
-    };
-    constexpr int NU = kOrFold ? NT / 2 : NT;
-    auto chain = [&](int u, const rows_t& w) -> acc_t {
-      if constexpr (kOrFold) {
-        acc_t acc = c3c_fp4_mfma2(w.m1, bfrag[2 * u][0], bias, static_cast<int>(bscales1), 2 * u);
-        acc = c3c_fp4_mfma2(w.m2, bfrag[2 * u][1], acc, static_cast<int>(bscales), 2 * u);
-        acc = c3c_fp4_mfma2(w.m1, bfrag[2 * u + 1][0], acc, static_cast<int>(bscales1), 2 * u + 1);
-        return c3c_fp4_mfma2(w.m2, bfrag[2 * u + 1][1], acc, static_cast<int>(bscales), 2 * u + 1);
-      } else if constexpr (PACKED) {
-        return c3c_fp4_mfma2(w.m2, bfrag[u][1], c3c_fp4_mfma1(w.m1, bfrag[u][0]), static_cast<int>(bscales), u);
-      } else {
-        return c3c_fp4_mfma2(afrag[1], bfrag[u][1], c3c_fp4_mfma1(afrag[0], bfrag[u][0]), static_cast<int>(bscales), u);
-      }
-    };
-    auto fold = [&](const acc_t& acc) -> int {
-      const c3c_v16i bits = __builtin_bit_cast(c3c_v16i, acc);
-      if constexpr (kOrFold) {
-        int top = bits[0] | bits[1] | bits[2];
-#pragma unroll
-        for (int k = 3; k < 15; k += 2) top = top | bits[k] | bits[k + 1];
-        return (top | bits[15]) & (kFlagHi | kFlagLo);
-      } else {
-        int top = max(max(bits[0], bits[1]), bits[2]);
-#pragma unroll
-        for (int k = 3; k < 15; k += 2) top = max(max(top, bits[k]), bits[k + 1]);
-        return max(top, bits[15]);
-      }
-    };
+          if constexpr (kOrFold) {
+            __builtin_amdgcn_sched_group_barrier(0x008, 1, 0);
+            __builtin_amdgcn_sched_group_barrier(0x002, NSM_C3C_OR_SPLIT, 0);
+            __builtin_amdgcn_sched_group_barrier(0x008, 1, 0);
+            __builtin_amdgcn_sched_group_barrier(0x002, NSM_C3C_OR_SPLIT, 0);
+            __builtin_amdgcn_sched_group_barrier(0x008, 1, 0);
+            __builtin_amdgcn_sched_group_barrier(0x002, NSM_C3C_OR_SPLIT, 0);
+            __builtin_amdgcn_sched_group_barrier(0x008, 1, 0);
+            __builtin_amdgcn_sched_group_barrier(0x002, 8 - 3 * NSM_C3C_OR_SPLIT, 0);
+          } else {
+            __builtin_amdgcn_sched_group_barrier(0x008, 1, 0);
+            __builtin_amdgcn_sched_group_barrier(0x002, NSM_C3C_FP4_SPLIT, 0);
+            __builtin_amdgcn_sched_group_barrier(0x008, 1, 0);
+            __builtin_amdgcn_sched_group_barrier(0x002, 8 - NSM_C3C_FP4_SPLIT, 0);
+          }
+          if (t + 1 < NU || kOrFold || (more && !flush)) asm volatile("" : "+v"(acc[(t + 1) & 1]));
 #else
-    typedef c3c_v16i acc_t;
-    constexpr int NU = NT;
-    c3c_v4i afrag[CAP - 1];
-    auto make_afrag = [&](const uint4& w) {
-#pragma unroll
-      for (int s = 0; s < CAP - 1; ++s) {
-        afrag[s].x = static_cast<int>(c3c_ge64(w.x, s + 1)); afrag[s].y = static_cast<int>(c3c_ge64(w.y, s + 1));
-        afrag[s].z = static_cast<int>(c3c_ge64(w.z, s + 1)); afrag[s].w = static_cast<int>(c3c_ge64(w.w, s + 1));
-      }
-    };
-    auto chain = [&](int t, const uint4& w) -> c3c_v16i {
-      c3c_v16i acc = {0, 0, 0, 0, 0, 0, 0, 0, 0, 0, 0, 0, 0, 0, 0, 0};
-#pragma unroll
-      for (int s = 0; s < CAP - 1; ++s) acc = __builtin_amdgcn_mfma_i32_32x32x32_i8(afrag[s], bfrag[t][s], acc, 0, 0, 0);
-      const c3c_v4i last = {static_cast<int>(w.x), static_cast<int>(w.y), static_cast<int>(w.z), static_cast<int>(w.w)};
-      return __builtin_amdgcn_mfma_i32_32x32x32_i8(last, bfrag[t][CAP - 1], acc, 0, 0, 0);
-    };
-    auto fold = [&](const c3c_v16i& acc) -> int {
-      int top = max(max(acc[0], acc[1]), acc[2]);
-#pragma unroll
-      for (int k = 3; k < 15; k += 2) top = max(max(top, acc[k]), acc[k + 1]);
-      return max(top, acc[15]);
-    };
-#endif
-    auto push = [&](bool ps, unsigned long long m, int t, int i) {
-      if (m == 0ull) return;
-#ifdef NSM_C3C_X_COUNTPUSH
-      if (lane == 0) atomicAdd(count, static_cast<unsigned long long>(__popcll(m)));
-#endif
-      if (ps) {
-        const int slot = __builtin_amdgcn_mbcnt_hi(static_cast<uint32_t>(m >> 32), __builtin_amdgcn_mbcnt_lo(static_cast<uint32_t>(m), static_cast<uint32_t>(q_cnt)));
-        const uint32_t hi = (static_cast<uint32_t>(i - i0) << 15) | (static_cast<uint32_t>(la) << 8) | (static_cast<uint32_t>(t) << 6);
-        uint32_t el = static_cast<uint32_t>(lane);
-        asm volatile("" : "+v"(el));
-        const uint32_t n_rows = static_cast<uint32_t>(min(kC3cBlock, b - i));
-        stack[slot] = (static_cast<unsigned long long>(hi | el) << 32) | n_rows;
-      }
-      q_cnt += __popcll(m);
-    };
-    auto finish = [&](int top, int u, int i) {
-      if constexpr (kOrFold) {
-        if (__ballot(top != 0) == 0ull) return;
-        const bool hi = (top & kFlagHi) != 0 && valid[2 * u], lo = (top & kFlagLo) != 0 && valid[2 * u + 1];
-        push(hi, __ballot(hi), 2 * u, i);
-        push(lo, __ballot(lo), 2 * u + 1, i);
-      } else {
-        const bool ps = top > nm1[u];
-        push(ps, __ballot(ps), u, i);
-      }
-    };
-#if NSM_C3C_PIPE
-    static_assert(NU % 2 == 0, "unit 0 of the next block takes the accumulator of unit NU: NU must be even (or NSM_C3C_PIPE=0)");
-    acc_t acc[2];
-    auto block = [&](int i, rows_t& wc, rows_t& wn) __attribute__((always_inline)) -> bool {
-      const bool more = i + kC3cBlock < b;
-      bool flush = false;
-#pragma unroll
-      for (int t = 0; t < NU; ++t) {
-        if (t + 1 < NU) {
-          acc[(t + 1) & 1] = chain(t + 1, wc);
+          __builtin_amdgcn_sched_group_barrier(0x008, 1, 0);
+          __builtin_amdgcn_sched_group_barrier(0x002, 4, 0);
+          __builtin_amdgcn_sched_group_barrier(0x008, 1, 0);
+          __builtin_amdgcn_sched_group_barrier(0x002, 4, 0);
+          __builtin_amdgcn_sched_group_barrier(0x008, 1, 0);
+#endif
+          finish(top, t, i);
+        }
+        return flush;
+      };
+      for (int i = a; i < b;) {
+        if (q_cnt > kC3cDrainAt)
+          drain_full();
+        if constexpr (kOrFold) make_bias();
+        rows_t w0 = load_rows(i);
+        make_afrag(w0);
+        rows_t w1;
+        if constexpr (PACKED) {
+          w1 = load_rows(i + kC3cBlock);
         } else {
-          flush = q_cnt > kC3cDrainAt;
-          if (kOrFold || (more && !flush)) {
-            make_afrag(wn);
-            if constexpr (PACKED) asm volatile("" : "+v"(wn.m1), "+v"(wn.m2));
-            if (i + 2 * kC3cBlock < b) wc = load_rows(i + 2 * kC3cBlock);
-            acc[0] = chain(0, wn);
-          }
-        }
-        const int top = fold(acc[t & 1]);
-#if NSM_C3C_FP4
-        if constexpr (kOrFold) {
-          __builtin_amdgcn_sched_group_barrier(0x008, 1, 0);
-          __builtin_amdgcn_sched_group_barrier(0x002, NSM_C3C_OR_SPLIT, 0);
-          __builtin_amdgcn_sched_group_barrier(0x008, 1, 0);
-          __builtin_amdgcn_sched_group_barrier(0x002, NSM_C3C_OR_SPLIT, 0);
-          __builtin_amdgcn_sched_group_barrier(0x008, 1, 0);
-          __builtin_amdgcn_sched_group_barrier(0x002, NSM_C3C_OR_SPLIT, 0);
-          __builtin_amdgcn_sched_group_barrier(0x008, 1, 0);
-          __builtin_amdgcn_sched_group_barrier(0x002, 8 - 3 * NSM_C3C_OR_SPLIT, 0);
-        } else {
-          __builtin_amdgcn_sched_group_barrier(0x008, 1, 0);
-          __builtin_amdgcn_sched_group_barrier(0x002, NSM_C3C_FP4_SPLIT, 0);
-          __builtin_amdgcn_sched_group_barrier(0x008, 1, 0);
-          __builtin_amdgcn_sched_group_barrier(0x002, 8 - NSM_C3C_FP4_SPLIT, 0);
-        }
-        if (t + 1 < NU || kOrFold || (more && !flush)) asm volatile("" : "+v"(acc[(t + 1) & 1]));
+          w1 = w0;
+          if (i + kC3cBlock < b) w1 = load_rows(i + kC3cBlock);
+        }
+        acc[0] = chain(0, w0);
+        for (;;) {
+          const bool f0 = block(i, w0, w1);
+          if ((i += kC3cBlock) >= b || f0) break;
+          const bool f1 = block(i, w1, w0);
+          if ((i += kC3cBlock) >= b || f1) break;
+        }
+      }
 #else
-        __builtin_amdgcn_sched_group_barrier(0x008, 1, 0);
-        __builtin_amdgcn_sched_group_barrier(0x002, 4, 0);
-        __builtin_amdgcn_sched_group_barrier(0x008, 1, 0);
-        __builtin_amdgcn_sched_group_barrier(0x002, 4, 0);
-        __builtin_amdgcn_sched_group_barrier(0x008, 1, 0);
-#endif
-        finish(top, t, i);
-      }
-      return flush;
-    };
-    for (int i = a; i < b;) {
-      if (q_cnt > kC3cDrainAt)
-        drain_full();
       if constexpr (kOrFold) make_bias();
-      rows_t w0 = load_rows(i);
-      make_afrag(w0);
-      rows_t w1;
-      if constexpr (PACKED) {
-        w1 = load_rows(i + kC3cBlock);
-      } else {
-        w1 = w0;
-        if (i + kC3cBlock < b) w1 = load_rows(i + kC3cBlock);
-      }
-      acc[0] = chain(0, w0);
-      for (;;) {
-        const bool f0 = block(i, w0, w1);
-        if ((i += kC3cBlock) >= b || f0) break;
-        const bool f1 = block(i, w1, w0);
-        if ((i += kC3cBlock) >= b || f1) break;
-      }
-    }
-#else
-    if constexpr (kOrFold) make_bias();
-    rows_t w_next = load_rows(a);
-    for (int i = a; i < b; i += kC3cBlock) {
-      const rows_t w = w_next;
-      if (i + kC3cBlock < b) w_next = load_rows(i + kC3cBlock);
-      if (q_cnt > kC3cDrainAt)
-        drain_full();
-      make_afrag(w);
-#pragma unroll
-      for (int t = 0; t < NU; ++t) {
-        const acc_t acc = chain(t, w);
-        finish(fold(acc), t, i);
-      }
-    }
-#endif
-  }
-  while (q_cnt > 0) drain_pass();
-}
-
-}
+      rows_t w_next = load_rows(a);
+      for (int i = a; i < b; i += kC3cBlock) {
+        const rows_t w = w_next;
+        if (i + kC3cBlock < b) w_next = load_rows(i + kC3cBlock);
+        if (q_cnt > kC3cDrainAt)
+          drain_full();
+        make_afrag(w);
+#pragma unroll
+        for (int t = 0; t < NU; ++t) {
+          const acc_t acc = chain(t, w);
+          finish(fold(acc), t, i);
+        }
+      }
+#endif
+    }
+    bool keep = false;
+    if constexpr (PERSIST) {
+      if (it_cur < it_end) {
+        const int4 nx = *c3p_item(c3p_queue(lpacked), static_cast<unsigned int>(it_cur));
+        keep = __builtin_amdgcn_readfirstlane(nx.x) * kRights == j0 && __builtin_amdgcn_readfirstlane(nx.w) == i0;
+      }
+    }
+    if (!keep) {
+      while (q_cnt > 0) drain_pass();
+    }
+  } while (PERSIST);
+}
+
+}
diff --git a/napkon-string-matching_amd/napkon_string_matching_amd/_lib.py b/napkon-string-matching_amd/napkon_string_matching_amd/_lib.py
--- a/napkon-string-matching_amd/napkon_string_matching_amd/_lib.py
+++ b/napkon-string-matching_amd/napkon_string_matching_amd/_lib.py
@@ -13,6 +13,7 @@
 FLAG_RAW_SCORE = 32
 FLAG_ONE_STAGE = 1024
 FLAG_PACK, FLAG_NO_PACK = 2048, 4096
+FLAG_ONE_GROUP = 8192
 FLAG_SPLIT, FLAG_TILE, FLAG_PROBE = 128, 256, 512
 FLAG_PARK = 16
 BUILD_PARTITION, BUILD_VALIDATE, BUILD_SORT = 1, 2, 4
diff --git a/napkon-string-matching_amd/napkon_string_matching_amd/grid.py b/napkon-string-matching_amd/napkon_string_matching_amd/grid.py
--- a/napkon-string-matching_amd/napkon_string_matching_amd/grid.py
+++ b/napkon-string-matching_amd/napkon_string_matching_amd/grid.py
@@ -133,12 +133,13 @@
 
 def indel_raw_grid(
     left: StrTable, right: StrTable, threshold: float, prune: bool = True, capacity: Optional[int] = None,
-    two_stage: bool = True, pack: Optional[bool] = None, defer: bool = False,
+    two_stage: bool = True, pack: Optional[bool] = None, defer: bool = False, one_group: bool = False,
 ) -> Hits:
     lib = _lib.load()
     ls, rs = left.struct(), right.struct()
     flags = ((_lib.FLAG_PRUNE if prune else 0) | (0 if two_stage else _lib.FLAG_ONE_STAGE)
-             | (0 if pack is None else (_lib.FLAG_PACK if pack else _lib.FLAG_NO_PACK)))
+             | (0 if pack is None else (_lib.FLAG_PACK if pack else _lib.FLAG_NO_PACK))
+             | (_lib.FLAG_ONE_GROUP if one_group else 0))
 
     def launch(buf: HitBuffer, stream: int) -> int:
         return lib.nsm_indel_raw_grid(
```

Result: faster. 44100 billion pair-comparisons/s (median of 6 runs) (+1.6%).
